# dakom/awsm-renderer

Measured on AMD Instinct MI355X. Metric: frames/sec + shaded Mpix/s, 4K Sponza glTF, 1/2/4/8 MI355X, higher is better.
Workload: dtype f32; 1 GPU; Sponza-class procedural atrium (configs[3]): 262144 triangles, 25 materials, 69 textures, 3840x2160, geometry pass + opaque pass, single-sample, MipmapMode::None; triangles=262144, width=3840, height=2160, draws=92, frame_overlap=True, stream_handoff=device flags (k_handoff_signal / k_handoff_wait), camera=orbit, one turn per 240 frames, environment=uniform cubes (builder default), opaque_route=lean (k_shade_lean + k_shade_todo), library=awsm-renderer_amd/libawsm_hip.so

## Files before the change

### awsm-renderer_amd/csrc/awsm_hip.cpp

```cpp
#include <hip/hip_runtime.h>
#include <algorithm>
#include <cmath>
#include <cstdarg>
#include <cstdio>
#include <cstdlib>
#include <cstring>
#include <ctime>
#include <string>
#include <vector>

#include "ctx.hpp"
#include "launch.hpp"

using namespace awsm;

namespace {

constexpr int kLeanWgsPerCu = 0;

inline FrameBufs* pass_slots(AwsmHipCtx* c, PassKind kind) {
    FrameBufs* const sets[kPassKinds] = {c->fb, c->tr, c->hud, c->htr, c->shadow};
    return sets[kind];
}
inline FrameBufs& pass_bufs(AwsmHipCtx* c, PassKind kind) { return pass_slots(c, kind)[c->slot]; }
inline FrameBufs& FB(AwsmHipCtx* c) { return c->fb[c->slot]; }
inline uint32_t samples_of(const AwsmHipCtx* c) { return c->msaa == 4 ? 4u : 1u; }
inline bool is_sharded(const AwsmHipCtx* c) { return c->band_n > 1 || (c->y1 != 0 && !(c->y0 == 0 && c->y1 >= c->height)); }
inline hipStream_t shade_stream_of(AwsmHipCtx* c) { return c->overlap ? c->shade_streams[c->slot] : c->stream; }
inline int n_slots(const AwsmHipCtx* c) { return c->overlap ? kSlots : 1; }
inline int prev_slot(const AwsmHipCtx* c) { return (c->slot + kSlots - 1) % kSlots; }
inline uint32_t* handoff_timeouts(AwsmHipCtx* c) { return c->counters_host + 16 + 2 * kSlots; }
inline unsigned long long* trace_slot(AwsmHipCtx* c, int which) { return c->trace_dev ? c->trace_dev + (size_t)which * c->trace_cap + c->frame_serial % c->trace_cap : nullptr; }
inline hipError_t mark_shade_done(AwsmHipCtx* c, hipStream_t ss) {
    if (c->handoff) awsm_launch_handoff_signal(c->handoff_flags + kSlots + c->slot, ++c->shade_sig[c->slot], trace_slot(c, 2), ss);
    else if (c->trace_dev) awsm_launch_handoff_signal(nullptr, 0u, trace_slot(c, 2), ss);
    const hipError_t e = hipEventRecord(c->ev_shade_done[c->slot], ss);
    c->shade_pending[c->slot] = true; c->shade_recorded[c->slot] = true;
    return e;
}
inline hipError_t wait_prev_slot(AwsmHipCtx* c, hipStream_t ss, bool main_kernel_only = false) {
    const int p = prev_slot(c);
    if (c->handoff && c->shade_sig[p]) {
        const bool lean = main_kernel_only && c->lean_flagged[p];
        awsm_launch_handoff_wait(c->handoff_flags + (lean ? 2 * kSlots : kSlots) + p, lean ? c->lean_sig[p] : c->shade_sig[p], c->handoff_budget_ticks, handoff_timeouts(c), c->handoff_timeouts_seen,
                                 c->handoff_poison + c->slot, c->frame_serial, ss);
        return hipSuccess;
    }
    return hipStreamWaitEvent(ss, c->ev_shade_done[p], 0);
}
inline hipError_t wait_slot_free(AwsmHipCtx* c) {
    if (c->handoff) { awsm_launch_handoff_wait(c->handoff_flags + kSlots + c->slot, c->shade_sig[c->slot], c->handoff_budget_ticks, handoff_timeouts(c), c->handoff_timeouts_seen,
                                               c->handoff_poison + c->slot, c->frame_serial, c->stream); return hipSuccess; }
    return hipStreamWaitEvent(c->stream, c->ev_shade_done[c->slot], 0);
}

struct HostTrace {
    static long threshold() { static long t = [] { const char* e = getenv("AWSM_HOST_TRACE"); return e ? atol(e) : 0L; }(); return t; }
    timespec last{};
    uint32_t serial;
    explicit HostTrace(uint32_t frame_serial) : serial(frame_serial) { if (threshold()) clock_gettime(CLOCK_MONOTONIC, &last); }
    void mark(const char* what) {
        if (!threshold()) return;
        timespec now; clock_gettime(CLOCK_MONOTONIC, &now);
        const long us = (now.tv_sec - last.tv_sec) * 1000000L + (now.tv_nsec - last.tv_nsec) / 1000L;
        if (us >= threshold()) fprintf(stderr, "awsm_hip host trace: frame %u: %s took %ld us\n", serial, what, us);
        last = now;
    }
};

int handoff_check(AwsmHipCtx* c) {
    if (!c->overlap) return AWSM_OK;
    const uint32_t now = *(volatile uint32_t*)handoff_timeouts(c);
    if (now != c->handoff_timeouts_seen) {
        c->handoff_dropped_frames += now - c->handoff_timeouts_seen;
        c->handoff_timeouts_seen = now;
        c->handoff = false;
        c->handoff_error_pending = true;
        for (FrameBufs& b : c->fb) b.cache_valid = false;
        c->taa_have = false; c->taa_serial = 0;
    }
    if (!c->handoff_error_pending) return AWSM_OK;
    c->handoff_error_pending = false;
    return fail(c, AWSM_ERR_DEVICE, "a device-side stream hand-off timed out (kernels serialised by a profiler, the streams folded onto one hardware queue, or a stall longer than "
                                    "AWSM_HANDOFF_TIMEOUT_MS): %u gate(s) so far, each dropped the frame it guarded whole — that frame's image was not written; this context orders "
                                    "its streams with events from here on (AWSM_DEVICE_HANDOFF=0 selects them from the start)", c->handoff_dropped_frames);
}

}

namespace awsm {

int fail(AwsmHipCtx* c, int code, const char* fmt, ...) {
    char buf[512];
    va_list ap;
    va_start(ap, fmt);
    vsnprintf(buf, sizeof buf, fmt, ap);
    va_end(ap);
    if (c) c->last_error = buf;
    return code;
}

hipError_t sync_shade_streams(AwsmHipCtx* c) {
    for (hipStream_t s : c->shade_streams) if (s) { const hipError_t e = hipStreamSynchronize(s); if (e != hipSuccess) return e; }
    for (bool& b : c->shade_recorded) b = false;
    return hipSuccess;
}

int dev_realloc(AwsmHipCtx* c, DevBuf& b, size_t bytes, bool zero) {
    if (b.ptr && b.size == bytes) {
        if (zero) HIPCHK(c, hipMemsetAsync(b.ptr, 0, bytes, c->stream));
        return AWSM_OK;
    }
    if (b.ptr) {
        HIPCHK(c, hipStreamSynchronize(c->stream));
        HIPCHK(c, sync_shade_streams(c));
        HIPCHK(c, hipFree(b.ptr));
        b.ptr = nullptr; b.size = 0;
    }
    if (bytes == 0) return AWSM_OK;
    HIPCHK(c, hipMalloc(&b.ptr, bytes));
    b.size = bytes;
    if (zero) HIPCHK(c, hipMemsetAsync(b.ptr, 0, bytes, c->stream));
    return AWSM_OK;
}

int dev_reserve(AwsmHipCtx* c, DevBuf& b, size_t bytes) {
    if (b.size >= bytes && b.ptr) return AWSM_OK;
    size_t want = std::max(bytes, b.size + b.size / 2);
    return dev_realloc(c, b, want, false);
}

constexpr size_t kKernelUploadMax = 256u << 10;

int stage_alloc(AwsmHipCtx* c, size_t len, uint8_t** out) {
    len = (len + 255) & ~size_t(255);
    if (len > c->stage_cap) {
        HIPCHK(c, hipStreamSynchronize(c->stream));
        if (c->stage) HIPCHK(c, hipHostFree(c->stage));
        c->stage = nullptr;
        size_t cap = std::max<size_t>(len * 2, 8u << 20);
        HIPCHK(c, hipHostMalloc((void**)&c->stage, cap, hipHostMallocDefault));
        c->stage_cap = cap; c->stage_head = 0;
    }
    if (c->stage_head + len > c->stage_cap) {
        HIPCHK(c, hipStreamSynchronize(c->stream));
        c->stage_head = 0;
    }
    *out = c->stage + c->stage_head;
    c->stage_head += len;
    return AWSM_OK;
}

int upload_small(AwsmHipCtx* c, void* dst, const void* src, size_t len) {
    uint8_t* st;
    int rc = stage_alloc(c, len, &st);
    if (rc) return rc;
    memcpy(st, src, len);
    if (len <= kKernelUploadMax && (len & 3u) == 0 && ((uintptr_t)dst & 3u) == 0 && ((uintptr_t)st & 3u) == 0) {
        awsm_launch_upload_words(dst, st, (uint32_t)(len >> 2), c->stream);
        HIPCHK(c, hipGetLastError());
    } else {
        HIPCHK(c, hipMemcpyAsync(dst, st, len, hipMemcpyHostToDevice, c->stream));
    }
    return AWSM_OK;
// ... 55 lines not shown
    f.tile_count = (uint32_t*)b.tile_count.ptr; f.tile_offset = (uint32_t*)b.tile_offset.ptr;
    f.tile_cursor = (uint32_t*)b.tile_cursor.ptr; f.bin_list = (uint32_t*)b.bin_list.ptr;
    f.tile_order = (uint32_t*)b.tile_order.ptr;
    f.scan_tmp = (uint32_t*)b.scan_tmp.ptr;
    f.tile_split = (uint32_t*)b.tile_split.ptr; f.raster_scratch = (unsigned long long*)b.raster_scratch.ptr;
    f.raster_extra_cap = b.raster_extra_cap; f.raster_slot_cap = b.raster_slot_cap;
    f.big_list = (uint32_t*)b.big_list.ptr;
    f.counters = (uint32_t*)b.counters.ptr;
    f.vis = (unsigned long long*)b.vis.ptr;
}

struct FrameView { bool hud_keys, merged; };
inline FrameView world_view() { return {false, false}; }
inline FrameView frame_view(const AwsmHipCtx* c) { return {c->hud_geometry_done, c->hud_merged}; }

void fill_frame(AwsmHipCtx* c, FrameDev* f, FrameView view) {
    memset(f, 0, sizeof *f);
    const PassList& world = c->lists[kPassWorld];
    const PassList& hud = c->lists[kPassHud];
    uint32_t y0, y1;
    shard(c, &y0, &y1);
    f->width = c->width; f->height = c->height; f->y0 = y0; f->y1 = y1; f->sy0 = y0; f->sy1 = y1;
    if (c->msaa && (y0 > 0 || y1 < c->height)) {
        f->y0 = y0 > 0 ? y0 - 1 : 0; f->y1 = std::min(c->height, y1 + 1);
    }
    f->tiles_x = (c->width + kTile - 1) / kTile;
    f->band_n = 1; f->band_r = 0; f->out_compact = 0;
    f->tile_row0 = f->y0 >> kTileShift;
    f->tiles_y = (f->y1 > f->y0) ? ((f->y1 + kTile - 1) / kTile - f->tile_row0) : 0;
    if (c->band_n > 1) {
        const uint32_t rows_full = (c->height + kTile - 1) / kTile;
        f->band_n = c->band_n; f->band_r = c->band_r; f->out_compact = c->band_compact;
        f->tile_row0 = c->band_r;
        f->tiles_y = c->band_r < rows_full ? (rows_full - c->band_r + c->band_n - 1) / c->band_n : 0;
    }
    f->n_draws = (uint32_t)world.draws.size();
    f->total_tris = world.total_tris; f->total_verts = 3u * world.total_tris;
    bind_pass(*f, FB(c));
    f->draw_shade = (DrawShadeDev*)FB(c).draw_shade.ptr;
    f->tex_slots = (TexSlotDev*)FB(c).tex_slots.ptr;
    f->draw_mat = (DrawMatDev*)FB(c).draw_mat.ptr;
    const bool lean_ok = !(c->flags & AWSM_CFG_GENERAL_SHADE_ONLY) && (uint64_t)c->width * c->height * (c->msaa == 4 ? 32u : 8u) < (1ull << 32) && (c->msaa == 0 || (c->msaa_edge_bits[c->slot].ptr && c->msaa_cells[c->slot].ptr)) && FB(c).tri_shade.ptr && FB(c).draw_lean.ptr && c->shade_todo[c->slot].ptr && ((uint64_t)world.total_tris + (view.merged ? hud.total_tris : 0u)) * kTriRecBytes < (1ull << 32) &&
                         c->bufs[AWSM_BUF_ATTR_DATA].size < (1ull << 32) - 64;
    f->tri_shade = lean_ok ? (uint4*)FB(c).tri_shade.ptr : nullptr;
    f->attr_data_bytes = (uint32_t)std::min<size_t>(c->bufs[AWSM_BUF_ATTR_DATA].size, 0xFFFFFFFFu);
    f->draw_lean = lean_ok ? (LeanDrawDev*)FB(c).draw_lean.ptr : nullptr;
    f->shade_todo = (uint32_t*)c->shade_todo[c->slot].ptr;
    f->shade_todo_cap = f->shade_todo ? (uint32_t)(c->shade_todo[c->slot].size / 4 - 4 - 1024) : 0u;
    f->lean_next = f->shade_todo ? f->shade_todo + 4 + f->shade_todo_cap : nullptr;
    f->lean_grid = c->lean_grid;
#ifdef AWSM_STAMP
    {
        static unsigned long long* stamps = nullptr;
        if (!stamps && hipMalloc((void**)&stamps, 4ull * 16384 * 8 * 8) == hipSuccess) (void)hipMemset(stamps, 0, 4ull * 16384 * 8 * 8);
        f->stamps = stamps;
        static bool told = false;
        if (!told) { told = true; FILE* fp = fopen("/tmp/awsm_stamps_ptr", "w"); if (fp) { fprintf(fp, "%llu\n", (unsigned long long)(uintptr_t)stamps); fclose(fp); } }
    }
#endif
    f->poison = c->handoff_poison ? c->handoff_poison + c->slot : nullptr;
    f->host_bin_status = c->counters_host + 16 + 2 * c->slot;
    f->frame_serial = c->frame_serial;
    f->camera = (const uint8_t*)FB(c).camera.ptr;
    f->camera_snap = nullptr; f->camera_snap_words = 0;
    memcpy(f->pix2view, FB(c).pix2view, sizeof f->pix2view); memcpy(f->view_rot, FB(c).view_rot, sizeof f->view_rot); memcpy(f->cam_pos, FB(c).cam_pos, sizeof f->cam_pos);
    memcpy(f->ortho_view_dir, FB(c).ortho_view_dir, sizeof f->ortho_view_dir); f->cam_ortho = FB(c).cam_ortho;
    f->msaa = c->msaa;
    f->msaa_color0 = (float4*)c->msaa_color0[c->slot].ptr;
    f->msaa_edges = (uint32_t*)c->msaa_edges[c->slot].ptr;
    f->msaa_edge_bits = (lean_ok && c->msaa == 4) ? (unsigned long long*)c->msaa_edge_bits[c->slot].ptr : nullptr;
    f->msaa_cells = (uint2*)c->msaa_cells[c->slot].ptr;
    f->hud_vis = view.hud_keys ? (const unsigned long long*)c->hud[c->slot].vis.ptr : nullptr;
    f->hud_draws = (const DrawDev*)c->hud[c->slot].draws_dev.ptr; f->hud_tri_info = (const uint32_t*)c->hud[c->slot].tri_flags.ptr;
    if (view.hud_keys && view.merged) {
        f->n_draws = (uint32_t)c->hud_combined.size();
        f->total_tris = world.total_tris + hud.total_tris; f->total_verts = 3u * f->total_tris;
        f->vis = (unsigned long long*)c->merged_vis[c->slot].ptr;
        f->hud_draws = f->draws; f->hud_tri_info = f->tri_info;
    }
    f->hud_pass = 0;
    f->msaa_halo = (const unsigned long long*)c->msaa_halo;
    f->halo_bands = c->band_n > 1 ? ((c->height + kTile - 1) / kTile + c->band_n - 1) / c->band_n : 0u;
    f->out_rgba16f = (uint16_t*)(c->bound_out ? (uint8_t*)c->bound_out - (size_t)c->out_first_row * c->width * 8 : c->out16[c->slot].ptr);
    f->out_rgba32f = (float*)c->out32[c->slot].ptr;
    f->lights_pre = (float4*)c->lights_pre[c->slot].ptr;
    f->lights_cap = (uint32_t)(c->lights_pre[c->slot].size / 32);
}

void compose_pixel_to_view(AwsmHipCtx* c, FrameBufs& b) {
    float cam[128];
    memcpy(cam, c->camera_host, 512);
    const float* proj = cam + 16; const float* inv_proj = cam + 64; const float* inv_view = cam + 80;
    const double W = (double)c->width, H = (double)c->height;
    const double A[16] = {2.0 / W, 0, 0, 0,   0, -2.0 / H, 0, 0,   0, 0, 1, 0,   1.0 / W - 1.0, 1.0 - 1.0 / H, 0, 1};
    for (int col = 0; col < 4; col++) for (int row = 0; row < 4; row++) {
        double s = 0.0;
        for (int k = 0; k < 4; k++) s += (double)inv_proj[k * 4 + row] * A[col * 4 + k];
        b.pix2view[col * 4 + row] = (float)s;
    }
    for (int col = 0; col < 3; col++) for (int row = 0; row < 3; row++) b.view_rot[col * 3 + row] = inv_view[col * 4 + row];
    for (int i = 0; i < 3; i++) b.cam_pos[i] = cam[96 + i];
    b.cam_ortho = proj[15] > 0.9f ? 1u : 0u;
    const double vx = inv_view[8], vy = inv_view[9], vz = inv_view[10], l = std::sqrt(vx * vx + vy * vy + vz * vz);
    b.ortho_view_dir[0] = l > 0.0 ? (float)(vx / l) : 0.0f; b.ortho_view_dir[1] = l > 0.0 ? (float)(vy / l) : 0.0f; b.ortho_view_dir[2] = l > 0.0 ? (float)(vz / l) : 1.0f;
}

int record(AwsmHipCtx* c, int which, hipStream_t s = nullptr) {
    if (!c->stage_timers) { c->ev_valid[which] = false; return AWSM_OK; }
    HIPCHK(c, hipEventRecord(c->ev[which], s ? s : c->stream));
    c->ev_valid[which] = true;
    return AWSM_OK;
}

AwsmHipCtx::ResolveKey resolve_key(AwsmHipCtx* c, const FrameDev& f) {
    AwsmHipCtx::ResolveKey k;
    memset(&k, 0, sizeof k);
    k.write_seq = c->write_seq + (c->scene_dirty ? 1u : 0u); k.draws_version = FB(c).draws_version;
    k.ptrs[0] = f.draw_shade; k.ptrs[1] = f.draw_mat; k.ptrs[2] = f.tex_slots; k.ptrs[3] = f.draw_lean; k.ptrs[4] = f.lights_pre;
    k.n_draws = f.n_draws; k.mipmap = c->last_opaque.mipmap; k.has_opaque = c->last_opaque.has_opaque; k.lights_cap = f.lights_cap;
    return k;
}
bool resolve_stale(AwsmHipCtx* c, const FrameDev& f) {
    const AwsmHipCtx::ResolveKey k = resolve_key(c, f);
    return memcmp(&k, &c->resolved[c->slot], sizeof k) != 0;
}

void fill_geometry_cache(AwsmHipCtx* c, FrameDev* f, bool replay) {
    FrameBufs& b = FB(c);
    f->wcache = (float4*)b.wcache.ptr;
    f->cache_on = 0; f->prev_draws = nullptr; f->prev_n_draws = 0; f->n_dirty = 0; f->cache_serial = b.cache_serial;
    if (!c->geometry_cache || replay || !b.cache_valid || !b.wcache.ptr || b.cache_had_tri_shade != (f->tri_shade != nullptr)) return;
    std::vector<DirtyRange> r;
    if (!c->dirty_log.ranges_since(b.cache_seq, kMaxDirtyRanges, r)) return;
    for (size_t i = 0; i < r.size(); i++) { f->dirty[i][0] = r[i].buf; f->dirty[i][1] = r[i].lo; f->dirty[i][2] = r[i].hi; }
    f->n_dirty = (uint32_t)r.size();
    f->prev_draws = (const DrawDev*)(b.cached_is_prev ? b.draws_prev.ptr : b.draws_dev.ptr);
    f->prev_n_draws = b.cached_n_draws;
    f->cache_on = f->prev_draws ? 1u : 0u;
}


inline void enqueue_binning(const FrameDev& f, bool has_tris, hipStream_t s) {
    if (has_tris) { awsm_launch_bin_count(&f, s); awsm_launch_bin_big(&f, 0, s); }
    awsm_launch_bin_scan(&f, s);
    if (has_tris) { awsm_launch_bin_fill(&f, s); awsm_launch_bin_big(&f, 1, s); }
}
int clear_empty_pass(AwsmHipCtx* c, const FrameBufs& b, uint32_t* counters, uint32_t n_tiles, hipStream_t s) {
    HIPCHK(c, hipMemsetAsync(counters, 0, kCtrWords * sizeof(uint32_t), s));
    HIPCHK(c, hipMemsetAsync(counters + 12, 0, 2 * sizeof(uint32_t), s));
    if (n_tiles) HIPCHK(c, hipMemsetAsync(b.tile_count.ptr, 0, n_tiles * sizeof(uint32_t), s));
    return AWSM_OK;
}

int enqueue_geometry(AwsmHipCtx* c, bool replay = false) {
    HostTrace ht(c->frame_serial);
    const PassList& world = c->lists[kPassWorld];
    FrameDev f;
    fill_frame(c, &f, world_view());
    fill_geometry_cache(c, &f, replay);
    f.block_draw = FB(c).block_map_valid ? (const uint32_t*)FB(c).block_map.ptr : nullptr;
    f.cache_mark = (c->stage_timers && FB(c).cache_mark.size >= (size_t)world.n_blocks * 4) ? (uint32_t*)FB(c).cache_mark.ptr : nullptr;
    const uint32_t n_tiles = f.tiles_x * f.tiles_y;
    int rc = sync_scene(c);
    if (rc) return rc;
    ht.mark("geometry: sync_scene");
    if (c->overlap && c->shade_pending[c->slot]) { HIPCHK(c, wait_slot_free(c)); c->shade_pending[c->slot] = false; }
    if (c->bufs[AWSM_BUF_CAMERA].ptr && !replay) {
        const size_t cam_bytes = std::min<size_t>(512, c->bufs[AWSM_BUF_CAMERA].size);
        if (world.total_tris && n_tiles) { f.camera_snap = (uint32_t*)FB(c).camera.ptr; f.camera_snap_words = (uint32_t)(cam_bytes / 4); }
        else HIPCHK(c, hipMemcpyAsync(FB(c).camera.ptr, c->bufs[AWSM_BUF_CAMERA].ptr, cam_bytes, hipMemcpyDeviceToDevice, c->stream));
    }
    if (c->overlap) {
        c->uploads_recorded[c->slot] = false;
        if (resolve_stale(c, f)) { HIPCHK(c, hipEventRecord(c->ev_uploads[c->slot], c->stream)); c->uploads_recorded[c->slot] = true; }
        c->geom_write_seq[c->slot] = c->write_seq;
    }
    ht.mark("geometry: slot wait + upload event");
    const bool has_geometry = world.total_tris && n_tiles;
    if (!has_geometry && (rc = clear_empty_pass(c, FB(c), (uint32_t*)FB(c).counters.ptr, n_tiles, c->stream))) return rc;
    if (c->trace_dev) awsm_launch_handoff_signal(nullptr, 0u, trace_slot(c, 0), c->stream);
    if ((rc = record(c, EV_START))) return rc;
#ifdef AWSM_DEBUG_SWITCHES
    static const int knockout_env = getenv("AWSM_DEBUG_KNOCKOUT") ? atoi(getenv("AWSM_DEBUG_KNOCKOUT")) : 0;
    const int knockout = c->frame_serial > 8 ? knockout_env : 0;
#else
    const int knockout = 0;
#endif
    if (has_geometry && !(knockout & 1)) awsm_launch_transform(c->scene_dev, &f, world.n_blocks, c->stream);
    if ((rc = record(c, EV_TRANSFORM))) return rc;
    ht.mark("geometry: transform launch");
    if (n_tiles && !(knockout & 2)) enqueue_binning(f, world.total_tris != 0, c->stream);
    if ((rc = record(c, EV_BIN))) return rc;
    ht.mark("geometry: bin launches");
    if (n_tiles && !(knockout & 4)) awsm_launch_raster(&f, c->stream);
    if ((rc = record(c, EV_RASTER))) return rc;
    ht.mark("geometry: raster launch");
    HIPCHK(c, hipGetLastError());
    {
        FrameBufs& b = FB(c);
        b.cache_valid = has_geometry && !(knockout & 1) && b.wcache.ptr != nullptr;
        b.cached_n_draws = (uint32_t)world.draws.size(); b.cached_is_prev = false;
        b.cache_had_tri_shade = f.tri_shade != nullptr;
        b.cache_seq = c->write_seq; b.cache_serial = c->frame_serial;
        uint64_t oldest = ~0ull;
        for (int sl = 0; sl < n_slots(c); sl++) oldest = std::min(oldest, c->fb[sl].cache_valid ? c->fb[sl].cache_seq : c->write_seq);
        c->dirty_log.prune(oldest);
    }
    return AWSM_OK;
}

int enqueue_opaque(AwsmHipCtx* c) {
    HostTrace ht(c->frame_serial);
    FrameDev f;
    fill_frame(c, &f, frame_view(c));
    f.has_opaque = c->last_opaque.has_opaque;
    f.mipmap = c->last_opaque.mipmap;
    f.aniso = (c->flags & AWSM_CFG_ANISOTROPIC) ? 1u : 0u;
    if (c->bound_out) {
        if (c->out_rows_mode) {
            if (f.out_compact || f.sy0 < c->out_first_row || (size_t)(f.sy1 - c->out_first_row) * c->width * 8 > c->bound_out_bytes)
                return fail(c, AWSM_ERR_INVALID_ARGUMENT, "opaque_pass: bound output starts at row %u and holds %zu bytes, the shard shades rows [%u, %u)", c->out_first_row, c->bound_out_bytes, f.sy0, f.sy1);
        } else {
            const size_t need = (f.out_compact ? (size_t)f.tiles_y * kTile : (size_t)c->height) * c->width * 8;
            if (c->bound_out_bytes < need) return fail(c, AWSM_ERR_INVALID_ARGUMENT, "opaque_pass: bound output holds %zu bytes, this shard layout writes %zu", c->bound_out_bytes, need);
        }
    }
    int rc = sync_scene(c);
    if (rc) return rc;
    hipStream_t ss = shade_stream_of(c);
    const bool want_resolve = f.sy1 > f.sy0 && f.has_opaque && (resolve_stale(c, f) || c->stage_timers);
    if (want_resolve) c->resolved[c->slot] = resolve_key(c, f);
    const bool early = c->uploads_recorded[c->slot] && c->overlap && !c->stage_timers && want_resolve && c->geometry_done && c->geom_write_seq[c->slot] == c->write_seq;
    if (early) {
        HIPCHK(c, hipStreamWaitEvent(ss, c->ev_uploads[c->slot], 0));
        awsm_launch_resolve_draws(c->scene_dev, &f, ss);
    }
    ht.mark("opaque: sync_scene + early resolve");
    if (c->overlap) {
        if (c->handoff) {
            ++c->geom_sig[c->slot];
            if (c->handoff_test_drop) c->handoff_test_drop--;
            else awsm_launch_handoff_signal(c->handoff_flags + c->slot, c->geom_sig[c->slot], trace_slot(c, 1), c->stream);
            awsm_launch_handoff_wait(c->handoff_flags + c->slot, c->geom_sig[c->slot], c->handoff_budget_ticks, handoff_timeouts(c), c->handoff_timeouts_seen, c->handoff_poison + c->slot, c->frame_serial, ss);
        } else {
            if (c->trace_dev) awsm_launch_handoff_signal(nullptr, 0u, trace_slot(c, 1), c->stream);
            HIPCHK(c, hipEventRecord(c->ev_geom_done[c->slot], c->stream));
            HIPCHK(c, hipStreamWaitEvent(ss, c->ev_geom_done[c->slot], 0));
        }
        const uint8_t* lo = (const uint8_t*)c->bound_out; const uint8_t* hi = lo ? lo + c->bound_out_bytes : nullptr;
        const int p = prev_slot(c);
        const bool same_image = lo && c->slot_out_lo[p] && lo < c->slot_out_hi[p] && c->slot_out_lo[p] < hi;
        if (c->shade_recorded[p]) HIPCHK(c, wait_prev_slot(c, ss, !(same_image || (c->msaa != 0 && c->msaa_halo))));
        c->slot_out_lo[c->slot] = lo; c->slot_out_hi[c->slot] = hi;
    }
    ht.mark("opaque: hand-off launches");
    if (want_resolve && !early) awsm_launch_resolve_draws(c->scene_dev, &f, ss);
    if ((rc = record(c, EV_SHADE_BEGIN, ss))) return rc;
    c->ev_valid[EV_SHADE_LEAN] = false;
    c->lean_flagged[c->slot] = false;
    if (c->overlap && c->handoff && f.sy1 > f.sy0 && awsm_shade_is_lean(&f)) {
        f.lean_done_flag = c->handoff_flags + 2 * kSlots + c->slot; f.lean_done_serial = ++c->lean_sig[c->slot];
        c->lean_flagged[c->slot] = true;
    }
    if (f.sy1 > f.sy0) {
        awsm_launch_shade(c->scene_dev, &f, ss);
        if (c->stage_timers && awsm_shade_is_lean(&f) && (rc = record(c, EV_SHADE_LEAN, ss))) return rc;
        (void)awsm_launch_shade_todo(c->scene_dev, &f, ss);
    }
    const AwsmHipCtx::ShadowState& sh = c->shadow_pass[c->slot];
    if (sh.on && c->shadow_px[c->slot] && f.has_opaque && f.sy1 > f.sy0) {
        const size_t px = (size_t)c->width * c->height;
        ShadowViewsArgs av{};
        ShadowArgs& a = av.base;
        const AwsmHipCtx::ShadowViews& views = c->shadow_views[c->slot];
        av.n_views = views.n; av.view = (unsigned char*)c->shadow_view_layers[c->slot].ptr;
        memcpy(av.view_proj, views.view_proj, sizeof av.view_proj);
        a.width = c->width; a.height = c->height;
        a.vis = (const unsigned long long*)FB(c).vis.ptr;
        a.camera = (const float*)f.camera;
        a.map = (const uint32_t*)c->shadow[c->slot].vis.ptr; a.map_size = sh.p.map_size; a.pcf_radius = (int32_t)sh.p.pcf_radius;
        memcpy(a.light_view_proj, sh.light_view_proj, sizeof a.light_view_proj); memcpy(a.light, sh.p.light, sizeof a.light);
        a.bias = sh.p.bias; a.slope_bias = sh.p.slope_bias; a.max_slope = sh.p.max_slope; a.strength = sh.p.strength; a.facing_fade = sh.p.facing_fade;
        a.visibility = (float*)c->shadow_layers[c->slot].ptr; a.multiplier = a.visibility + px;
        a.out16 = (uint2*)f.out_rgba16f; a.out32 = (float4*)f.out_rgba32f;
        a.poison = f.poison; a.frame_serial = f.frame_serial;
        awsm_launch_shadow_resolve(&a, samples_of(c), ss);
    }
    const AwsmHipCtx::SsaoState& so = c->ssao_pass[c->slot];
    if (so.on && f.has_opaque && f.sy1 > f.sy0) {
        const size_t px = (size_t)c->width * c->height;
        SsaoArgs sa{};
        sa.width = c->width; sa.height = c->height;
        sa.vis = (const unsigned long long*)FB(c).vis.ptr;
        sa.camera = (const float*)f.camera;
        sa.radius = so.p[0]; sa.intensity = so.p[1]; sa.bias = so.p[2]; sa.strength = so.p[3];
        sa.ao_raw = (float*)c->ssao_layers[c->slot].ptr; sa.ao_smoothed = sa.ao_raw + px; sa.view_z = sa.ao_raw + 2 * px;
        sa.out16 = (uint2*)f.out_rgba16f; sa.out32 = (float4*)f.out_rgba32f;
        sa.poison = f.poison; sa.frame_serial = f.frame_serial;
        awsm_launch_ssao(&sa, samples_of(c), ss);
    }
    if ((rc = record(c, EV_SHADE, ss))) return rc;
    ht.mark("opaque: shade launches");
    if (c->overlap) HIPCHK(c, mark_shade_done(c, ss));
    else if (c->trace_dev) awsm_launch_handoff_signal(nullptr, 0u, trace_slot(c, 2), ss);
    ht.mark("opaque: shade-done signal + event");
    HIPCHK(c, hipGetLastError());
    return AWSM_OK;
}

void fill_frame_forward(AwsmHipCtx* c, FrameDev* f, PassKind kind) {
    fill_frame(c, f, frame_view(c));
    const FrameBufs& t = pass_bufs(c, kind);
    const PassList& list = c->lists[kind];
    bind_pass(*f, t);
    f->vis = (unsigned long long*)FB(c).vis.ptr;
    f->n_draws = (uint32_t)list.draws.size();
    f->total_tris = list.total_tris; f->total_verts = 3u * list.total_tris;
    f->draw_shade = (DrawShadeDev*)t.draw_shade.ptr;
    f->tex_slots = (TexSlotDev*)t.tex_slots.ptr;
    f->draw_mat = (DrawMatDev*)t.draw_mat.ptr;
    f->wpos = (float4*)t.wpos.ptr;
    f->tri_shade = nullptr; f->draw_lean = nullptr; f->shade_todo = nullptr; f->shade_todo_cap = 0; f->lean_next = nullptr; f->lean_grid = 0;
    f->raster_scratch = nullptr;
    f->raster_extra_cap = 0; f->raster_slot_cap = 0;
    f->opaque_rgba16f = c->opaque_src ? (const uint16_t*)c->opaque_src : f->out_rgba16f;
    f->out_compact = 0;
    f->frag_rec = (uint4*)t.frag_rec.ptr; f->frag_color = (float4*)t.frag_color.ptr; f->frag_first = (uint32_t*)t.frag_first.ptr; f->frag_cap = t.frag_cap;
    f->out_rgba16f = (uint16_t*)(c->bound_comp ? c->bound_comp : c->comp16.ptr);
    f->out_rgba32f = (float*)c->comp32.ptr;
    f->has_opaque = c->last_opaque.has_opaque;
    f->mipmap = c->last_opaque.mipmap;
    f->aniso = (c->flags & AWSM_CFG_ANISOTROPIC) ? 1u : 0u;
    if (kind == kPassHudTransparent) {
        f->hud_pass = 1;
        f->opaque_rgba16f = f->out_rgba16f;
    }
}

void fill_selection(AwsmHipCtx* c, const AwsmHipCtx::SelectionState& st, SelectionDev* a) {
    memset(a, 0, sizeof *a);
    a->width = c->width; a->height = c->height; a->msaa = samples_of(c);
    a->n_draws = (uint32_t)c->lists[kPassWorld].draws.size(); a->total_tris = c->lists[kPassWorld].total_tris;
    a->n_keys = (uint32_t)(st.keys.size() / 2); a->n_boxes = (uint32_t)(st.boxes.size() / 6);
    a->flags = st.flags; a->radius = st.radius;
    memcpy(a->outline_color, st.outline_color, sizeof a->outline_color); memcpy(a->box_color, st.box_color, sizeof a->box_color);
    a->half_width = st.half_width; a->hidden_alpha = st.hidden_alpha; a->depth_epsilon = st.depth_epsilon;
    a->scene = c->scene_dev;
    a->material_meta_bytes = (uint32_t)std::min<size_t>(c->bufs[AWSM_BUF_MATERIAL_META].size, 0xFFFFFFFFu);
    a->draws = (const DrawDev*)FB(c).draws_dev.ptr;
    a->tri_info = (const uint32_t*)FB(c).tri_flags.ptr;
    a->vis = (const unsigned long long*)FB(c).vis.ptr;
    a->camera = (const uint8_t*)FB(c).camera.ptr;
    a->edges = (float*)c->sel_tables[c->slot].ptr;
    a->draw_selected = (uint8_t*)c->sel_tables[c->slot].ptr + (size_t)selection::kMaxEdges * selection::kEdgeFloats * 4;
    if (a->n_keys) memcpy(a->keys, st.keys.data(), st.keys.size() * 4);
    if (a->n_boxes) memcpy(a->boxes, st.boxes.data(), st.boxes.size() * 4);
}

int enqueue_transparent(AwsmHipCtx* c, PassKind kind) {
    const bool hud = kind == kPassHudTransparent;
    FrameDev f;
    fill_frame_forward(c, &f, kind);
    const uint32_t n_tiles = f.tiles_x * f.tiles_y;
    int rc = sync_scene(c);
    if (rc) return rc;
    hipStream_t ss = shade_stream_of(c);
    if (c->overlap && c->shade_recorded[prev_slot(c)]) HIPCHK(c, wait_prev_slot(c, ss));
    if ((rc = record(c, EV_FWD_BEGIN, ss))) return rc;
    const bool has_geometry = f.total_tris && n_tiles;
    if (!has_geometry) {
        if ((rc = clear_empty_pass(c, pass_bufs(c, kind), (uint32_t*)pass_bufs(c, kind).counters.ptr, n_tiles, ss))) return rc;
    } else {
        awsm_launch_resolve_draws(c->scene_dev, &f, ss);
        awsm_launch_transform_forward(c->scene_dev, &f, c->lists[kind].n_blocks, ss);
    }
    if (n_tiles) {
        enqueue_binning(f, f.total_tris != 0, ss);
        EditorGridDev grid;
        const AwsmHipCtx::GridState& gs = c->grid_pass[c->slot];
        const bool with_grid = gs.on && !hud;
        if (with_grid) { grid.camera = f.camera; memcpy(grid.p, gs.p, sizeof grid.p); }
        awsm_launch_forward(c->scene_dev, &f, with_grid ? &grid : nullptr, ss);
        const AwsmHipCtx::SelectionState& sl = c->sel_pass[c->slot];
        if (sl.on && !hud) {
            SelectionDev sd;
            fill_selection(c, sl, &sd);
            sd.out16 = (uint2*)f.out_rgba16f; sd.out32 = (float4*)f.out_rgba32f;
            sd.poison = f.poison; sd.frame_serial = f.frame_serial;
            awsm_launch_selection(&sd, ss);
        }
    }
    if ((rc = record(c, EV_FWD, ss))) return rc;
    if (c->overlap) HIPCHK(c, mark_shade_done(c, ss));
    HIPCHK(c, hipGetLastError());
    return AWSM_OK;
}

int ensure_bin_capacity_of(AwsmHipCtx* c, FrameBufs& b, uint32_t entries) {
    if (entries <= b.bin_capacity && b.bin_list.ptr) return AWSM_OK;
    uint32_t cap = std::max(entries, b.bin_capacity + b.bin_capacity / 2);
    int rc = dev_realloc(c, b.bin_list, (size_t)cap * 4, false);
    if (rc) return rc;
    b.bin_capacity = cap;
    return AWSM_OK;
}

int ensure_fragment_capacity(AwsmHipCtx* c, FrameBufs& b, uint32_t fragments) {
    if (fragments <= b.frag_cap && b.frag_rec.ptr) return AWSM_OK;
    const uint32_t cap = std::max(fragments, b.frag_cap + b.frag_cap / 2);
    int rc = dev_realloc(c, b.frag_rec, (size_t)cap * 16, false);
    if (!rc) rc = dev_realloc(c, b.frag_color, (size_t)cap * 16, false);
    if (rc) return rc;
    b.frag_cap = cap;
    return AWSM_OK;
}

int build_draw_list(AwsmHipCtx* c, const char* pass, const AwsmDraw* draws, uint32_t n, AwsmBuf data, uint32_t bytes_per_tri,
                    std::vector<DrawDev>& out, uint64_t* tris_out, uint64_t* blocks_out) {
    out.clear();
    uint64_t tris = 0, blocks = 0;
    for (uint32_t i = 0; i < n; i++) {
        const AwsmDraw& d = draws[i];
        if (d.inst_count != 0) {
            const DevBuf& ib = c->bufs[AWSM_BUF_INSTANCES];
            if (!ib.ptr) return fail(c, AWSM_ERR_NOT_READY, "%s: draw %u: instanced, but the instance-transform buffer was never created", pass, i);
            if ((d.inst_off & 15u) || (uint64_t)d.inst_off + 64ull * d.inst_count > ib.size)
                return fail(c, AWSM_ERR_OUT_OF_RANGE, "%s: draw %u: %u instances at %u exceed the instance-transform buffer", pass, i, d.inst_count, d.inst_off);
        }
        if (d.vis_data_off & (bytes_per_tri ? 15u : 3u)) return fail(c, AWSM_ERR_INVALID_ARGUMENT, "%s: draw %u: vertex data offset %u misaligned", pass, i, d.vis_data_off);
        if ((uint64_t)d.vis_data_off + (uint64_t)bytes_per_tri * d.tri_count > c->bufs[data].size || (!bytes_per_tri && d.tri_count && (uint64_t)d.vis_data_off + 40 > c->bufs[data].size))
            return fail(c, AWSM_ERR_OUT_OF_RANGE, "%s: draw %u: %u triangles at %u exceed the vertex buffer", pass, i, d.tri_count, d.vis_data_off);
        if ((uint64_t)d.geom_meta_off + 40 > c->bufs[AWSM_BUF_GEOM_META].size || (d.geom_meta_off & 3u))
            return fail(c, AWSM_ERR_OUT_OF_RANGE, "%s: draw %u: geometry meta offset %u out of range", pass, i, d.geom_meta_off);
        if (d.tri_count == 0) continue;
        const uint32_t copies = d.inst_count ? d.inst_count : 1u;
        for (uint32_t k = 0; k < copies; k++) {
            DrawDev dd{};
            dd.geom_meta_off = d.geom_meta_off; dd.vis_data_off = d.vis_data_off; dd.tri_count = d.tri_count; dd.flags = d.flags & 0x7Fu;
            if (d.inst_count) { dd.flags |= kDrawInstanced; dd.inst_off = d.inst_off + 64u * k; }
            dd.first_tri = (uint32_t)tris; dd.first_block = (uint32_t)blocks;
            out.push_back(dd);
            tris += d.tri_count;
            blocks += (3ull * d.tri_count + 255) / 256;
            if (tris > 0x55555555ull) return fail(c, AWSM_ERR_UNSUPPORTED, "%s: more than 2^32/3 triangles in one pass", pass);
            if (out.size() >= (1u << 24)) return fail(c, AWSM_ERR_UNSUPPORTED, "%s: more than 2^24 non-empty draws (instances included) in one pass", pass);
        }
    }
    *tris_out = tris; *blocks_out = blocks;
    return AWSM_OK;
}

struct PassDims { uint32_t w, h, samples; };
inline PassDims dims_of(const AwsmHipCtx* c, const FrameBufs& b) {
    if (b.kind == kPassShadow) { const uint32_t S = c->shadow_pass[b.slot].p.map_size; return {S, S, 1u}; }
    return {c->width, c->height, samples_of(c)};
}

int reserve_raster_items(AwsmHipCtx* c, FrameBufs& b, bool forward, PassDims dm) {
    const uint32_t tiles_x = (dm.w + kTile - 1) / kTile, tiles_y_full = (dm.h + kTile - 1) / kTile;
    const size_t n_tiles_full = (size_t)tiles_x * tiles_y_full;
    const uint32_t extra_cap = forward ? 0u : b.bin_capacity / 256u + 1u, slot_cap = forward ? 0u : b.bin_capacity / 128u + 2u;
    int rc;
    if ((rc = dev_reserve(c, b.tile_order, (n_tiles_full + extra_cap) * 4))) return rc;
    if (!forward && (rc = dev_reserve(c, b.raster_scratch, (size_t)slot_cap * kTile * kTile * 8 * dm.samples))) return rc;
    b.raster_extra_cap = extra_cap; b.raster_slot_cap = slot_cap;
    return AWSM_OK;
}

int size_pass_buffers(AwsmHipCtx* c, FrameBufs& b, size_t tri_cap, size_t draw_cap, bool forward, PassDims dm) {
    int rc;
    const size_t nd = std::max<size_t>(draw_cap, 1), nv = std::max<size_t>(3 * tri_cap, 1), nt = std::max<size_t>(tri_cap, 1);
    if ((rc = dev_reserve(c, b.draws_dev, nd * sizeof(DrawDev)))) return rc;
    const bool world_pass = b.kind == kPassWorld, shadow = b.kind == kPassShadow;
    if (world_pass && c->geometry_cache) {
        if ((rc = dev_reserve(c, b.draws_prev, nd * sizeof(DrawDev)))) return rc;
        if ((rc = dev_reserve(c, b.wcache, nv * 16))) return rc;
        const size_t blocks_bound = nv / 256 + nd + 1;
        if ((rc = dev_reserve(c, b.block_map, blocks_bound * 4))) return rc;
        b.block_map_valid = false;
        if (b.cache_mark.size < blocks_bound * 4) { if ((rc = dev_realloc(c, b.cache_mark, (blocks_bound + blocks_bound / 2) * 4, true))) return rc; }
    }
    b.cache_valid = false;
    if (!shadow && (rc = dev_reserve(c, b.draw_shade, nd * sizeof(DrawShadeDev)))) return rc;
    if (!shadow && (rc = dev_reserve(c, b.tex_slots, nd * kCoreTextures * sizeof(TexSlotDev)))) return rc;
    if (!shadow && (rc = dev_reserve(c, b.draw_mat, nd * sizeof(DrawMatDev)))) return rc;
    if ((rc = dev_reserve(c, b.clip, nv * 16))) return rc;
    if ((rc = dev_reserve(c, b.nrm, nv * 16))) return rc;
    if ((rc = dev_reserve(c, b.tan, nv * 16))) return rc;
    if (forward && (rc = dev_reserve(c, b.wpos, nv * 16))) return rc;
    if ((rc = dev_reserve(c, b.tri_flags, nt * 4))) return rc;
    if (!forward && !shadow && (rc = dev_reserve(c, b.tri_shade, nt * 32))) return rc;
    if (!forward && !shadow && (rc = dev_reserve(c, b.draw_lean, nd * sizeof(LeanDrawDev)))) return rc;
    if ((rc = dev_reserve(c, b.big_list, nt * 4))) return rc;
    if ((rc = dev_reserve(c, b.tri_rec, nt * kTriRecBytes))) return rc;
    const uint32_t tiles_x = (dm.w + kTile - 1) / kTile, tiles_y_full = (dm.h + kTile - 1) / kTile;
    const size_t n_tiles_full = (size_t)tiles_x * tiles_y_full;
    if ((rc = dev_reserve(c, b.tile_count, n_tiles_full * 4))) return rc;
    if ((rc = dev_reserve(c, b.tile_offset, (n_tiles_full + 1) * 4))) return rc;
    if ((rc = dev_reserve(c, b.tile_cursor, n_tiles_full * 4))) return rc;
    if ((rc = dev_reserve(c, b.tile_split, n_tiles_full * 8))) return rc;
    if ((rc = dev_reserve(c, b.scan_tmp, (((n_tiles_full + 255) / 256) * 2 + 1) * 40 * 4))) return rc;
    if ((rc = ensure_bin_capacity_of(c, b, (c->flags & AWSM_CFG_SMALL_BIN_LIST) ? 4096u : (uint32_t)std::min<size_t>(std::max<size_t>(4 * tri_cap + 65536u, 1u << 18), 0xFFFFFFF0u)))) return rc;
    if ((rc = reserve_raster_items(c, b, forward, dm))) return rc;
    b.tri_cap = tri_cap; b.draw_cap = draw_cap; b.sized_w = dm.w; b.sized_h = dm.h;
    return AWSM_OK;
}

int ensure_pass_capacity(AwsmHipCtx* c, FrameBufs& b, const std::vector<DrawDev>& draws_host, uint32_t total_tris, bool forward) {
    int rc;
    const PassDims dm = dims_of(c, b);
    if (total_tris > b.tri_cap || draws_host.size() > b.draw_cap || b.sized_w != dm.w || b.sized_h != dm.h || !b.bin_list.ptr) {
        bool instanced = false;
        for (const DrawDev& d : draws_host) instanced |= (d.flags & kDrawInstanced) != 0;
        const size_t tri_bound = forward || instanced ? ~size_t(0) : c->bufs[AWSM_BUF_VIS_GEOM_DATA].size / 168u;
        const size_t tri_cap = std::max<size_t>(std::min<size_t>((size_t)total_tris + total_tris / 4 + 4096, std::max<size_t>(tri_bound, total_tris)), b.tri_cap);
        const size_t draw_cap = std::max<size_t>(draws_host.size() + draws_host.size() / 4 + 64, b.draw_cap);
        const bool shadow = b.kind == kPassShadow;
        FrameBufs* const set = pass_slots(c, b.kind);
        for (int sl = 0; sl < (shadow ? 1 : n_slots(c)); sl++) {
            FrameBufs& t = set[(c->slot + sl) % kSlots];
            if ((rc = size_pass_buffers(c, t, std::max(tri_cap, t.tri_cap), std::max(draw_cap, t.draw_cap), forward, dm))) return rc;
        }
    }
    return AWSM_OK;
}

int upload_draws_at(AwsmHipCtx* c, FrameBufs& b, size_t at, const std::vector<DrawDev>& list) {
    const size_t bytes = list.size() * sizeof(DrawDev);
    uint8_t* dst = (uint8_t*)b.draws_dev.ptr + at * sizeof(DrawDev);
    if (bytes <= (1u << 20)) return upload_small(c, dst, list.data(), bytes);
    HIPCHK(c, hipMemcpyAsync(dst, list.data(), bytes, hipMemcpyHostToDevice, c->stream));
    HIPCHK(c, hipStreamSynchronize(c->stream));
    return AWSM_OK;
}

int upload_draw_list(AwsmHipCtx* c, FrameBufs& b, const std::vector<DrawDev>& draws_host, bool keep_prev) {
    const bool same_draws = b.draws_uploaded_valid && b.draws_uploaded_ptr == b.draws_dev.ptr && b.draws_uploaded.size() == draws_host.size() &&
                            (draws_host.empty() || memcmp(b.draws_uploaded.data(), draws_host.data(), draws_host.size() * sizeof(DrawDev)) == 0);
    auto upload_block_map = [&]() -> int {
        b.block_map_valid = false;
        if (!keep_prev || !b.block_map.ptr) return AWSM_OK;
        std::vector<uint32_t> map;
        for (size_t i = 0; i < draws_host.size(); i++) map.insert(map.end(), (3ull * draws_host[i].tri_count + 255) / 256, (uint32_t)i);
        if (map.size() * 4 > b.block_map.size || map.size() * 4 > (1u << 20)) return AWSM_OK;
        const int rc = upload_small(c, b.block_map.ptr, map.data(), map.size() * 4);
        if (!rc) b.block_map_valid = true;
        return rc;
    };
    if (draws_host.empty()) return AWSM_OK;
    if (same_draws) return (keep_prev && !b.block_map_valid) ? upload_block_map() : AWSM_OK;
    if (keep_prev && b.cache_valid && !b.cached_is_prev && b.draws_prev.ptr && b.draws_prev.size == b.draws_dev.size) {
        std::swap(b.draws_dev, b.draws_prev);
        b.cached_is_prev = true;
    } else if (keep_prev && !b.cached_is_prev) b.cache_valid = false;
    b.draws_uploaded = draws_host; b.draws_uploaded_ptr = b.draws_dev.ptr; b.draws_uploaded_valid = true; b.draws_version++;
    b.tail_uploaded_valid = false;
    { const int rc = upload_block_map(); if (rc) return rc; }
    return upload_draws_at(c, b, 0, draws_host);
}

int reserve_pass_buffers(AwsmHipCtx* c, FrameBufs& b, const std::vector<DrawDev>& draws_host, uint32_t total_tris, bool forward) {
    int rc = ensure_pass_capacity(c, b, draws_host, total_tris, forward);
    if (rc) return rc;
    return upload_draw_list(c, b, draws_host, b.kind == kPassWorld);
}

inline uint32_t with_headroom(uint32_t need) { return need + need / 4 + 1024; }
int grow_after_overflow(AwsmHipCtx* c, FrameBufs& b, const uint32_t* counters) {
    const int rc = ensure_bin_capacity_of(c, b, with_headroom(counters[kCtrEntries]));
    return rc ? rc : reserve_raster_items(c, b, false, dims_of(c, b));
}

int merge_record(AwsmHipCtx* c, const char* entry, const char* type, const void* src, void* dst, size_t size) {
    const uint32_t given = *(const uint32_t*)src;
    if (given < 4u || given > 4096u) return fail(c, AWSM_ERR_INVALID_ARGUMENT, "%s: %s.struct_size = %u (set it to sizeof(%s))", entry, type, given, type);
    memcpy((uint8_t*)dst + 4, (const uint8_t*)src + 4, (std::min<size_t>(given, size) & ~(size_t)3) - 4);
    return AWSM_OK;
}
int check_finite(AwsmHipCtx* c, const char* entry, const float* p, size_t n) {
    for (size_t i = 0; i < n; i++)
        if (!std::isfinite(p[i])) return fail(c, AWSM_ERR_INVALID_ARGUMENT, "%s: value %zu of the record is not finite", entry, i);
    return AWSM_OK;
}

}

extern "C" {

uint32_t awsm_hip_abi_version(void) { return AWSM_HIP_ABI_VERSION; }

const char* awsm_hip_last_error(const AwsmHipCtx* ctx) { return ctx ? ctx->last_error.c_str() : "null context"; }

int awsm_hip_create(const AwsmConfig* cfg, AwsmHipCtx** out) {
    if (!cfg || !out || cfg->struct_size < sizeof(AwsmConfig) || cfg->abi_version != AWSM_HIP_ABI_VERSION)
        return AWSM_ERR_INVALID_ARGUMENT;
    *out = nullptr;
    int n_dev = 0;
    if (hipGetDeviceCount(&n_dev) != hipSuccess || n_dev <= 0 || cfg->device < 0 || cfg->device >= n_dev) return AWSM_ERR_NO_DEVICE;
    AwsmHipCtx* c = new (std::nothrow) AwsmHipCtx();
    if (!c) return AWSM_ERR_OUT_OF_MEMORY;
    c->device = cfg->device;
    c->flags = cfg->flags;
    for (int k = 0; k < kPassKinds; k++)
        for (int s = 0; s < kSlots; s++) { FrameBufs& b = pass_slots(c, (PassKind)k)[s]; b.kind = (PassKind)k; b.slot = (uint8_t)s; }
    auto bail = [&](int code) { awsm_hip_destroy(c); return code; };
    if (hipSetDevice(c->device) != hipSuccess) return bail(AWSM_ERR_DEVICE);
    hipDeviceProp_t prop;
    if (hipGetDeviceProperties(&prop, c->device) != hipSuccess) return bail(AWSM_ERR_DEVICE);
    if (strncmp(prop.gcnArchName, "gfx950", 6) != 0) {
        fprintf(stderr, "awsm_hip: device %d is %s; this library carries gfx950 code objects only\n", c->device, prop.gcnArchName);
        return bail(AWSM_ERR_NO_DEVICE);
    }
    if (cfg->stream) { c->stream = (hipStream_t)cfg->stream; c->own_stream = false; }
    else { if (hipStreamCreateWithFlags(&c->stream, hipStreamNonBlocking) != hipSuccess) return bail(AWSM_ERR_DEVICE); c->own_stream = true; }
    for (int i = 0; i < EV_COUNT; i++) if (hipEventCreate(&c->ev[i]) != hipSuccess) return bail(AWSM_ERR_DEVICE);
    if (hipMalloc((void**)&c->scene_dev, sizeof(DevScene)) != hipSuccess) return bail(AWSM_ERR_OUT_OF_MEMORY);
    c->overlap = (cfg->flags & AWSM_CFG_OVERLAP_FRAMES) != 0;
    { const char* e = getenv("AWSM_GEOMETRY_CACHE"); c->geometry_cache = !(e && e[0] == '0'); }
    {
        const char* e = getenv("AWSM_LEAN_WGS_PER_CU");
        const int per_cu = e ? atoi(e) : (c->overlap ? kLeanWgsPerCu : 0);
        c->lean_grid = per_cu > 0 ? (uint32_t)(per_cu * prop.multiProcessorCount) & ~7u : 0u;
    }
    for (int s = 0; s < n_slots(c); s++) {
        for (PassKind k : {kPassWorld, kPassTransparent, kPassHudTransparent, kPassHud}) {
            DevBuf& ctr = pass_slots(c, k)[s].counters;
            if (hipMalloc(&ctr.ptr, 16 * sizeof(uint32_t)) != hipSuccess || (k == kPassWorld && hipMemset(ctr.ptr, 0, 16 * sizeof(uint32_t)) != hipSuccess)) return bail(AWSM_ERR_OUT_OF_MEMORY);
            ctr.size = 16 * sizeof(uint32_t);
        }
        if (hipMalloc(&c->fb[s].camera.ptr, 512) != hipSuccess || hipMemset(c->fb[s].camera.ptr, 0, 512) != hipSuccess) return bail(AWSM_ERR_OUT_OF_MEMORY);
        c->fb[s].camera.size = 512;
    }

    if (c->overlap) {
        for (int s = 0; s < kSlots; s++) {
#ifdef AWSM_DEBUG_SWITCHES
            if (const char* m = getenv("AWSM_SHADE_CU_MASK")) {
                std::vector<uint32_t> words;
                for (const char* p = m; *p; ) { char* end = nullptr; words.push_back((uint32_t)strtoul(p, &end, 16)); p = (*end == ',') ? end + 1 : end; if (end == p && *p) break; }
                if (words.empty() || hipExtStreamCreateWithCUMask(&c->shade_streams[s], (uint32_t)words.size(), words.data()) != hipSuccess) return bail(AWSM_ERR_DEVICE);
            } else
#endif
            if (hipStreamCreateWithFlags(&c->shade_streams[s], hipStreamNonBlocking) != hipSuccess) return bail(AWSM_ERR_DEVICE);
            const unsigned ev_flags = hipEventDisableTiming | hipEventReleaseToDevice;
            if (hipEventCreateWithFlags(&c->ev_geom_done[s], ev_flags) != hipSuccess || hipEventCreateWithFlags(&c->ev_shade_done[s], ev_flags) != hipSuccess ||
                hipEventCreateWithFlags(&c->ev_uploads[s], ev_flags) != hipSuccess) return bail(AWSM_ERR_DEVICE);
            if (s == 0 && hipEventCreateWithFlags(&c->ev_flush, hipEventDisableTiming) != hipSuccess) return bail(AWSM_ERR_DEVICE);
        }
    }
    if (hipHostMalloc((void**)&c->counters_host, (16 + 2 * kSlots + 1) * sizeof(uint32_t), hipHostMallocDefault) != hipSuccess) return bail(AWSM_ERR_OUT_OF_MEMORY);
    memset(c->counters_host, 0, (16 + 2 * kSlots + 1) * sizeof(uint32_t));
    if (c->overlap) {
        const char* e = getenv("AWSM_DEVICE_HANDOFF");
        c->handoff = !(e && e[0] == '0');
        { int khz = 0; if (hipDeviceGetAttribute(&khz, hipDeviceAttributeWallClockRate, c->device) == hipSuccess && khz > 0) c->clock_khz = (uint32_t)khz; }
        double budget_ms = 4000.0;
        if (const char* p = getenv("AWSM_HANDOFF_TIMEOUT_MS")) { const double v = atof(p); if (v > 0.0) budget_ms = v; }
        c->handoff_budget_ticks = (unsigned long long)(budget_ms * (double)c->clock_khz) + 1ull;
        if (hipMalloc((void**)&c->handoff_flags, 3 * kSlots * sizeof(uint32_t)) != hipSuccess || hipMalloc((void**)&c->handoff_poison, kSlots * sizeof(uint32_t)) != hipSuccess) return bail(AWSM_ERR_OUT_OF_MEMORY);
        if (hipMemset(c->handoff_flags, 0, 3 * kSlots * sizeof(uint32_t)) != hipSuccess || hipMemset(c->handoff_poison, 0xFF, kSlots * sizeof(uint32_t)) != hipSuccess ||
            hipDeviceSynchronize() != hipSuccess) return bail(AWSM_ERR_DEVICE);
        if (const char* d = getenv("AWSM_TEST_HANDOFF_DROP")) c->handoff_test_drop = (uint32_t)atoi(d);
        for (int k = 0; c->handoff && k < 2 * kSlots; k++) {
            hipStream_t ss = c->shade_streams[k % kSlots], waiter = k < kSlots ? ss : c->stream, setter = k < kSlots ? c->stream : ss;
            const uint32_t serial = ++c->geom_sig[0];
            awsm_launch_handoff_wait(c->handoff_flags, serial, 10ull * c->clock_khz , handoff_timeouts(c), 0u, nullptr, 0u, waiter);
            awsm_launch_handoff_signal(c->handoff_flags, serial, nullptr, setter);
            if (hipStreamSynchronize(waiter) != hipSuccess || hipStreamSynchronize(setter) != hipSuccess) return bail(AWSM_ERR_DEVICE);
            if (*(volatile uint32_t*)handoff_timeouts(c) != 0u) { c->handoff = false; c->handoff_timeouts_seen = *(volatile uint32_t*)handoff_timeouts(c); }
        }
    }
    memset(&c->scene, 0, sizeof c->scene);
    c->scene.skybox_rgba[3] = 1.0f;
    for (int i = 0; i < 3; i++) { c->scene.prefiltered_rgb[i] = 1.0f; c->scene.irradiance_rgb[i] = 1.0f; }
    *out = c;
    return AWSM_OK;
}

int awsm_hip_destroy(AwsmHipCtx* c) {
    if (!c) return AWSM_ERR_INVALID_ARGUMENT;
    (void)hipSetDevice(c->device);
    if (c->stream) (void)hipStreamSynchronize(c->stream);
    (void)sync_shade_streams(c);
    auto fr = [](DevBuf& b) { if (b.ptr) (void)hipFree(b.ptr); b.ptr = nullptr; b.size = 0; };
    for (auto& b : c->bufs) fr(b);
    for (auto& b : c->tex) fr(b);
    for (auto& b : c->tex_kinds) fr(b);
    for (auto& b : c->merged_vis) fr(b);
    fr(c->pose_records);
    fr(c->env_stage); fr(c->env_tables); fr(c->env_rows); fr(c->env_filter_tab); if (c->ev_env_copy) (void)hipEventDestroy(c->ev_env_copy);
    fr(c->lut); for (auto& b : c->cube_tex) fr(b); for (auto& b : c->cube_bordered) fr(b); fr(c->digest); for (auto& b : c->shade_todo) fr(b); for (int sl = 0; sl < kSlots; sl++) { fr(c->msaa_color0[sl]); fr(c->msaa_edges[sl]); fr(c->msaa_edge_bits[sl]); fr(c->msaa_cells[sl]); } fr(c->mip_kinds); for (auto& b : c->out16) fr(b); for (auto& b : c->out32) fr(b); fr(c->comp16); fr(c->comp32); fr(c->grid_layer); for (auto& b : c->lights_pre) fr(b);
    for (auto& b : c->ssao_layers) fr(b);
    for (auto& b : c->taa_img) fr(b); fr(c->taa_layers);
    for (auto& b : c->sel_tables) fr(b);
    fr(c->sel_layers);
    for (auto& b : c->shadow_layers) fr(b); for (auto& b : c->shadow_cam) fr(b); for (auto& b : c->shadow_view_ctr) fr(b); for (auto& b : c->shadow_view_layers) fr(b); for (DevScene* sc : c->shadow_scene) if (sc) (void)hipFree(sc);
    for (auto& b : c->display8) fr(b); fr(c->effects16); fr(c->bloom_a); fr(c->bloom_b); fr(c->dof_lc); fr(c->dof_blur);
    for (int k = 0; k < kPassKinds * kSlots; k++) {
        FrameBufs& b = pass_slots(c, (PassKind)(k / kSlots))[k % kSlots];
        fr(b.vis); fr(b.wpos); fr(b.frag_rec); fr(b.frag_color); fr(b.frag_first); fr(b.tex_slots); fr(b.draw_mat); fr(b.clip); fr(b.nrm); fr(b.tan); fr(b.tri_rec); fr(b.tri_flags); fr(b.tri_shade); fr(b.draw_lean); fr(b.draws_dev); fr(b.draw_shade); fr(b.tile_count); fr(b.tile_offset);
        fr(b.wcache); fr(b.draws_prev); fr(b.cache_mark); fr(b.block_map); fr(b.tile_cursor); fr(b.tile_order); fr(b.scan_tmp); fr(b.tile_split); fr(b.raster_scratch); fr(b.bin_list); fr(b.big_list); fr(b.counters); fr(b.camera);
    }
    for (hipStream_t st : c->shade_streams) if (st) (void)hipStreamDestroy(st);
    for (int i = 0; i < kSlots; i++) { if (c->ev_geom_done[i]) (void)hipEventDestroy(c->ev_geom_done[i]); if (c->ev_shade_done[i]) (void)hipEventDestroy(c->ev_shade_done[i]); if (c->ev_uploads[i]) (void)hipEventDestroy(c->ev_uploads[i]); }
    if (c->ev_flush) (void)hipEventDestroy(c->ev_flush);
    if (c->scene_dev) (void)hipFree(c->scene_dev);
    if (c->stage) (void)hipHostFree(c->stage);
    if (c->counters_host) (void)hipHostFree(c->counters_host);
    if (c->handoff_flags) (void)hipFree(c->handoff_flags);
    if (c->handoff_poison) (void)hipFree(c->handoff_poison);
    if (c->trace_dev) (void)hipFree(c->trace_dev);
    for (int i = 0; i < EV_COUNT; i++) if (c->ev[i]) (void)hipEventDestroy(c->ev[i]);
    if (c->own_stream && c->stream) (void)hipStreamDestroy(c->stream);
    delete c;
    return AWSM_OK;
}

int awsm_hip_device_info(AwsmHipCtx* c, char* name_out, size_t name_cap, uint32_t* cu_count, uint64_t* hbm_bytes) {
    if (!c) return AWSM_ERR_INVALID_ARGUMENT;
    hipDeviceProp_t prop;
    HIPCHK(c, hipGetDeviceProperties(&prop, c->device));
    if (name_out && name_cap) snprintf(name_out, name_cap, "%s (%s)", prop.name, prop.gcnArchName);
    if (cu_count) *cu_count = (uint32_t)prop.multiProcessorCount;
    if (hbm_bytes) *hbm_bytes = (uint64_t)prop.totalGlobalMem;
    return AWSM_OK;
}

int awsm_hip_buffer_create(AwsmHipCtx* c, AwsmBuf which, size_t bytes) {
    if (!c || (int)which < 0 || which >= AWSM_BUF_COUNT) return fail(c, AWSM_ERR_INVALID_ARGUMENT, "buffer_create: bad buffer id %d", (int)which);
    HIPCHK(c, hipSetDevice(c->device));
    { int rcb = scene_write_barrier(c); if (rcb) return rcb; }
    log_dirty(c, which, 0, ~size_t(0));
    if (bytes && c->bufs[which].ptr && c->bufs[which].size == bytes) {
        if (which == AWSM_BUF_CAMERA) memset(c->camera_host, 0, sizeof c->camera_host);
        HIPCHK(c, hipMemsetAsync(c->bufs[which].ptr, 0, bytes + 16, c->stream));
        return AWSM_OK;
    }
    int rc = dev_realloc(c, c->bufs[which], bytes ? bytes + 16 : 0, true);
    if (rc) return rc;
    if (bytes) c->bufs[which].size = bytes;
    if (which == AWSM_BUF_CAMERA) memset(c->camera_host, 0, sizeof c->camera_host);
    if (which == AWSM_BUF_LIGHTS) for (int sl = 0; sl < n_slots(c); sl++) if ((rc = dev_realloc(c, c->lights_pre[sl], std::max<size_t>(bytes / 64, 1) * 32, true))) return rc;
    c->scene_dirty = true;
    return AWSM_OK;
}

int awsm_hip_buffer_write(AwsmHipCtx* c, AwsmBuf which, size_t dst_off, const void* src, size_t len) {
    if (!c || (int)which < 0 || which >= AWSM_BUF_COUNT || (!src && len)) return fail(c, AWSM_ERR_INVALID_ARGUMENT, "buffer_write: bad argument");
    if ((dst_off & 3) || (len & 3)) return fail(c, AWSM_ERR_INVALID_ARGUMENT, "buffer_write: offset %zu / size %zu not 4-byte aligned", dst_off, len);
    DevBuf& b = c->bufs[which];
    if (!b.ptr) return fail(c, AWSM_ERR_NOT_READY, "buffer_write: buffer %d was never created", (int)which);
    if (dst_off > b.size || len > b.size - dst_off) return fail(c, AWSM_ERR_OUT_OF_RANGE, "buffer_write: [%zu,+%zu) outside buffer %d of %zu bytes", dst_off, len, (int)which, b.size);
    if (len == 0) return AWSM_OK;
    HIPCHK(c, hipSetDevice(c->device));
    if (which != AWSM_BUF_CAMERA) { int rcb = scene_write_barrier(c); if (rcb) return rcb; log_dirty(c, which, dst_off, dst_off + len); }
    else { if (dst_off < 512) memcpy(c->camera_host + dst_off, src, std::min<size_t>(len, 512 - dst_off)); c->camera_written_since_snapshot = true; }
    uint8_t* dst = (uint8_t*)b.ptr + dst_off;
    if (len <= (1u << 20)) return upload_small(c, dst, src, len);
    HIPCHK(c, hipMemcpyAsync(dst, src, len, hipMemcpyHostToDevice, c->stream));
    HIPCHK(c, hipStreamSynchronize(c->stream));
    return AWSM_OK;
}

int awsm_hip_skin_pose_records_write(AwsmHipCtx* c, uint32_t first, uint32_t n, const AwsmSkinPoseRecord* records) {
    if (!c || (!records && n)) return fail(c, AWSM_ERR_INVALID_ARGUMENT, "skin_pose_records_write: bad argument");
    static_assert(sizeof(AwsmSkinPoseRecord) == 72, "k_skin_pose reads 72-byte records");
    std::vector<AwsmSkinPoseRecord>& host = c->pose_records_host;
    if (first > host.size() || n > 0x03000000u - first) return fail(c, AWSM_ERR_OUT_OF_RANGE, "skin_pose_records_write: [%u,+%u) with %zu records resident", first, n, host.size());
    if (n == 0) return AWSM_OK;
    for (uint32_t i = 0; i < n; i++)
        if ((records[i].transform_offset & 3u) || (records[i].matrix_offset & 3u)) return fail(c, AWSM_ERR_INVALID_ARGUMENT, "skin_pose_records_write: record %u has an offset that is not a multiple of 4", first + i);
// ... 405 lines not shown
    }
    if (!c->shadow_scene[c->slot]) { HIPCHK(c, hipMalloc((void**)&c->shadow_scene[c->slot], sizeof(DevScene))); c->shadow_scene_seq[c->slot] = 0; }
    return dev_reserve(c, c->shadow_cam[c->slot], (size_t)cam_blocks * 512);
}

int awsm_hip_shadow_pass(AwsmHipCtx* c, const AwsmShadow* s, const void* light_camera, size_t camera_bytes, const AwsmDraw* casters, uint32_t n) {
    if (!c || !s || (!casters && n)) return AWSM_ERR_INVALID_ARGUMENT;
    if (!c->geometry_done || c->opaque_done) return fail(c, AWSM_ERR_NOT_READY, "shadow_pass goes between the geometry pass and the opaque pass of a frame");
    if (is_sharded(c))
        return fail(c, AWSM_ERR_UNSUPPORTED, "shadow_pass on a sharded context: the resolve's neighbours need rows the shard never rasterised (no halo exchange)");
    AwsmShadow full;
    float lvp[16];
    int rc;
    if ((rc = check_shadow_record(c, "shadow_pass", "spot", s, full))) return rc;
    if ((rc = check_light_block(c, "shadow_pass", light_camera, camera_bytes, lvp))) return rc;
    if (n && (rc = check_caster_buffers(c, "shadow_pass"))) return rc;
    HIPCHK(c, hipSetDevice(c->device));
    std::vector<DrawDev> list;
    uint64_t tris = 0, blocks = 0;
    if ((rc = build_draw_list(c, "shadow_pass", casters, n, AWSM_BUF_VIS_GEOM_DATA, 168u, list, &tris, &blocks))) return rc;
    FrameBufs& sb = pass_bufs(c, kPassShadow);
    PassList& cast = c->lists[kPassShadow];
    AwsmHipCtx::ShadowState& st = c->shadow_pass[c->slot];
    c->shadow_done = false; st.on = false;
    st.p = full; memcpy(st.light_view_proj, lvp, sizeof lvp);
    cast.draws.swap(list);
    cast.total_tris = (uint32_t)tris; cast.n_blocks = (uint32_t)blocks;
    if ((rc = reserve_shadow_slot(c, 0u, 1u))) return rc;
    if ((rc = dev_reserve(c, sb.vis, (size_t)full.map_size * full.map_size * 8))) return rc;
    if ((rc = reserve_pass_buffers(c, sb, cast.draws, cast.total_tris, false))) return rc;
    if ((rc = upload_small(c, c->shadow_cam[c->slot].ptr, light_camera, 512))) return rc;
    c->shadow_views[c->slot].n = 0;
    if ((rc = enqueue_shadow(c))) return rc;
    st.on = true; c->shadow_done = true;
    return AWSM_OK;
}

int awsm_hip_shadow_pass_views(AwsmHipCtx* c, const AwsmShadow* s, const AwsmShadowView* views, uint32_t n_views) {
    if (!c || !s) return AWSM_ERR_INVALID_ARGUMENT;
    if (!views || n_views < 1u || n_views > (uint32_t)AWSM_SHADOW_MAX_VIEWS)
        return fail(c, AWSM_ERR_INVALID_ARGUMENT, "shadow_pass_views: %u views at %p (1 .. %d views)", n_views, (const void*)views, AWSM_SHADOW_MAX_VIEWS);
    if (!c->geometry_done || c->opaque_done) return fail(c, AWSM_ERR_NOT_READY, "shadow_pass_views goes between the geometry pass and the opaque pass of a frame");
    if (is_sharded(c))
        return fail(c, AWSM_ERR_UNSUPPORTED, "shadow_pass_views on a sharded context: the resolve's neighbours need rows the shard never rasterised (no halo exchange)");
    AwsmShadow full;
    int rc;
    if ((rc = check_shadow_record(c, "shadow_pass_views", "positional", s, full))) return rc;
    float lvp[AWSM_SHADOW_MAX_VIEWS][16];
    uint8_t blocks_host[AWSM_SHADOW_MAX_VIEWS * 512];
    char label[AWSM_SHADOW_MAX_VIEWS][40];
    bool any_casters = false;
    for (uint32_t i = 0; i < n_views; i++) {
        const AwsmShadowView& v = views[i];
        snprintf(label[i], sizeof label[i], "shadow_pass_views: view %u", i);
        if (!v.casters && v.n_casters) return fail(c, AWSM_ERR_INVALID_ARGUMENT, "shadow_pass_views: view %u has %u casters at a null pointer", i, v.n_casters);
        if ((rc = check_light_block(c, label[i], v.light_camera, v.camera_bytes, lvp[i]))) return rc;
        memcpy(blocks_host + (size_t)i * 512, v.light_camera, 512);
        any_casters |= v.n_casters != 0;
    }
    if (any_casters && (rc = check_caster_buffers(c, "shadow_pass_views"))) return rc;
    HIPCHK(c, hipSetDevice(c->device));
    PassList lists[AWSM_SHADOW_MAX_VIEWS];
    for (uint32_t i = 0; i < n_views; i++) {
        uint64_t tris = 0, blocks = 0;
        if ((rc = build_draw_list(c, label[i], views[i].casters, views[i].n_casters, AWSM_BUF_VIS_GEOM_DATA, 168u, lists[i].draws, &tris, &blocks))) return rc;
        lists[i].total_tris = (uint32_t)tris; lists[i].n_blocks = (uint32_t)blocks;
    }
    FrameBufs& sb = pass_bufs(c, kPassShadow);
    AwsmHipCtx::ShadowState& st = c->shadow_pass[c->slot];
    AwsmHipCtx::ShadowViews& vs = c->shadow_views[c->slot];
    c->shadow_done = false; st.on = false;
    st.p = full; memcpy(st.light_view_proj, lvp[0], sizeof st.light_view_proj);
    vs.n = n_views; memcpy(vs.view_proj, lvp, sizeof vs.view_proj);
    for (uint32_t i = 0; i < n_views; i++) { vs.lists[i].draws.swap(lists[i].draws); vs.lists[i].total_tris = lists[i].total_tris; vs.lists[i].n_blocks = lists[i].n_blocks; }
    c->lists[kPassShadow] = PassList();
    if ((rc = reserve_shadow_slot(c, AWSM_SHADOW_MAX_VIEWS, AWSM_SHADOW_MAX_VIEWS))) return rc;
    if ((rc = dev_reserve(c, sb.vis, (size_t)n_views * full.map_size * full.map_size * 8))) return rc;
    for (uint32_t i = 0; i < n_views; i++)
        if ((rc = ensure_pass_capacity(c, sb, vs.lists[i].draws, vs.lists[i].total_tris, false))) return rc;
    if ((rc = upload_small(c, c->shadow_cam[c->slot].ptr, blocks_host, (size_t)n_views * 512))) return rc;
    if ((rc = enqueue_shadow_views(c))) return rc;
    st.on = true; c->shadow_done = true;
    return AWSM_OK;
}

static int read_shadow_layer(AwsmHipCtx* c, const char* entry, uint32_t view, uint64_t* keys) {
    if (!c || !keys) return AWSM_ERR_INVALID_ARGUMENT;
    if (!c->shadow_done || !c->shadow[c->slot].vis.ptr) return fail(c, AWSM_ERR_NOT_READY, "%s: the last submitted frame had no shadow pass", entry);
    const uint32_t n = std::max(c->shadow_views[c->slot].n, 1u);
    if (view >= n) return fail(c, AWSM_ERR_INVALID_ARGUMENT, "%s: view %u of a pass with %u", entry, view, n);
    HIPCHK(c, hipSetDevice(c->device));
    { int rcs = sync_all(c); if (rcs) return rcs; }
    const size_t S = c->shadow_pass[c->slot].p.map_size;
    HIPCHK(c, hipMemcpy(keys, (const uint64_t*)c->shadow[c->slot].vis.ptr + (size_t)view * S * S, S * S * 8, hipMemcpyDeviceToHost));
    return AWSM_OK;
}
int awsm_hip_read_shadow_map(AwsmHipCtx* c, uint64_t* keys) { return read_shadow_layer(c, "read_shadow_map", 0u, keys); }
int awsm_hip_read_shadow_map_view(AwsmHipCtx* c, uint32_t view, uint64_t* keys) { return read_shadow_layer(c, "read_shadow_map_view", view, keys); }

int awsm_hip_read_shadow_view(AwsmHipCtx* c, uint8_t* view_out) {
    if (!c || !view_out) return AWSM_ERR_INVALID_ARGUMENT;
    const size_t px = (size_t)c->width * c->height;
    if (!px || !c->shadow_done || !c->opaque_done || c->shadow_px[c->slot] != px || !c->shadow_views[c->slot].n || c->shadow_view_layers[c->slot].size < px)
        return fail(c, AWSM_ERR_NOT_READY, "read_shadow_view: the last submitted frame had no shadow_pass_views with an opaque pass (has_opaque) behind it");
    HIPCHK(c, hipSetDevice(c->device));
    { int rcs = sync_all(c); if (rcs) return rcs; }
    HIPCHK(c, hipMemcpy(view_out, c->shadow_view_layers[c->slot].ptr, px, hipMemcpyDeviceToHost));
    return AWSM_OK;
}

int awsm_hip_read_shadow(AwsmHipCtx* c, float* visibility, float* multiplier) {
    if (!c) return AWSM_ERR_INVALID_ARGUMENT;
    const size_t px = (size_t)c->width * c->height;
    if (!px || !c->shadow_done || !c->opaque_done || c->shadow_px[c->slot] != px || !c->shadow_layers[c->slot].ptr)
        return fail(c, AWSM_ERR_NOT_READY, "read_shadow: the last submitted frame had no shadow pass with an opaque pass (has_opaque) behind it");
    HIPCHK(c, hipSetDevice(c->device));
    { int rcs = sync_all(c); if (rcs) return rcs; }
    const float* d = (const float*)c->shadow_layers[c->slot].ptr;
    if (visibility) HIPCHK(c, hipMemcpy(visibility, d, px * 4, hipMemcpyDeviceToHost));
    if (multiplier) HIPCHK(c, hipMemcpy(multiplier, d + px, px * 4, hipMemcpyDeviceToHost));
    return AWSM_OK;
}

int awsm_hip_opaque_pass(AwsmHipCtx* c, const AwsmOpaqueParams* p) {
    if (!c || !p) return AWSM_ERR_INVALID_ARGUMENT;
    if (p->mipmap > 1) return fail(c, AWSM_ERR_INVALID_ARGUMENT, "opaque_pass: mipmap must be 0 (MipmapMode::None) or 1 (MipmapMode::Gradient)");
    if (c->width == 0) return fail(c, AWSM_ERR_NOT_READY, "opaque_pass before resize");
    if (p->has_opaque) {
        if (!c->geometry_done) return fail(c, AWSM_ERR_NOT_READY, "opaque_pass before geometry_pass");
        static const AwsmBuf need[] = {AWSM_BUF_CAMERA, AWSM_BUF_GEOM_META, AWSM_BUF_MATERIAL_META, AWSM_BUF_MATERIALS, AWSM_BUF_ATTR_INDEX,
                                       AWSM_BUF_ATTR_DATA, AWSM_BUF_TEXTURE_TRANSFORMS, AWSM_BUF_LIGHTS_INFO, AWSM_BUF_LIGHTS};
        for (AwsmBuf b : need) if (!c->bufs[b].ptr) return fail(c, AWSM_ERR_NOT_READY, "opaque_pass: buffer %d missing", (int)b);
        if (!c->lut.ptr) return fail(c, AWSM_ERR_NOT_READY, "opaque_pass: no BRDF LUT (env_upload or brdf_lut_generate)");
    }
    if (c->msaa == 4 && c->band_n > 1 && p->has_opaque) {
        const size_t need = (size_t)c->band_n * awsm_hip_msaa_halo_bands(c) * 2 * c->width * 8;
        if (!c->msaa_halo || c->msaa_halo_bytes < need)
            return fail(c, AWSM_ERR_NOT_READY, "opaque_pass: MSAA with band sharding needs the gathered halo keys (awsm_hip_msaa_halo_export -> all-gather -> awsm_hip_msaa_halo_bind, %zu bytes)", need);
    }
    const bool ssao_on = c->ssao.on && p->has_opaque;
    if (ssao_on && is_sharded(c))
        return fail(c, AWSM_ERR_UNSUPPORTED, "opaque_pass with SSAO on a sharded context: its taps and its smoothing read depth in rows the shard never rasterised (no halo exchange)");
    HIPCHK(c, hipSetDevice(c->device));
    if (ssao_on) { const int rcs = dev_reserve(c, c->ssao_layers[c->slot], (size_t)c->width * c->height * 12); if (rcs) return rcs; }
    c->ssao_pass[c->slot] = c->ssao;
    c->ssao_pass[c->slot].on = ssao_on;
    c->ssao_px[c->slot] = ssao_on ? (size_t)c->width * c->height : 0;
    const bool shadow_on = c->shadow_done && c->shadow_pass[c->slot].on && p->has_opaque;
    if (shadow_on) { const int rcs = dev_reserve(c, c->shadow_layers[c->slot], (size_t)c->width * c->height * 8); if (rcs) return rcs; }
    if (shadow_on && c->shadow_views[c->slot].n) { const int rcs = dev_reserve(c, c->shadow_view_layers[c->slot], (size_t)c->width * c->height); if (rcs) return rcs; }
    c->shadow_px[c->slot] = shadow_on ? (size_t)c->width * c->height : 0;
    c->last_opaque = *p;
    if (!p->has_opaque && c->camera_written_since_snapshot && c->bufs[AWSM_BUF_CAMERA].ptr) {
        int rcs = sync_all(c);
        if (rcs) return rcs;
        compose_pixel_to_view(c, FB(c));
        HIPCHK(c, hipMemcpy(FB(c).camera.ptr, c->bufs[AWSM_BUF_CAMERA].ptr, std::min<size_t>(512, c->bufs[AWSM_BUF_CAMERA].size), hipMemcpyDeviceToDevice));
        c->camera_written_since_snapshot = false;
    }
    int rc = enqueue_opaque(c);
    if (rc) return rc;
    c->opaque_done = true; c->transparent_done = false; c->hud_transparent_done = false;
    return AWSM_OK;
}

static int transparent_pass_body(AwsmHipCtx* c, const AwsmDraw* draws, uint32_t n, PassKind kind) {
    const bool hud = kind == kPassHudTransparent;
    if (!c || (!draws && n)) return AWSM_ERR_INVALID_ARGUMENT;
    if (!c->geometry_done || !c->opaque_done) return fail(c, AWSM_ERR_NOT_READY, "transparent_pass needs the geometry and opaque passes of the same frame first");
    if (hud && !c->transparent_done) return fail(c, AWSM_ERR_NOT_READY, "hud_transparent_pass draws over the composite: call transparent_pass first (n_draws = 0 is valid)");
    const bool sharded = is_sharded(c);
    if (sharded && !c->opaque_src)
        return fail(c, AWSM_ERR_UNSUPPORTED, "transparent_pass on a sharded context: screen-space transmission reads the whole opaque image — gather it and bind it with awsm_hip_bind_opaque_source first");
    if (!hud && c->sel.on && sharded)
        return fail(c, AWSM_ERR_UNSUPPORTED, "transparent_pass with a selection on a sharded context: the outline's ring reads keys in rows the shard never rasterised (no halo exchange)");
    if (!hud && c->sel.on && !c->lists[kPassWorld].draws.empty() && (!c->bufs[AWSM_BUF_GEOM_META].ptr || !c->bufs[AWSM_BUF_MATERIAL_META].ptr))
        return fail(c, AWSM_ERR_NOT_READY, "transparent_pass with a selection: the geometry or material meta buffer is missing");
    if (c->opaque_src && c->opaque_src_bytes < (size_t)c->width * c->height * 8)
        return fail(c, AWSM_ERR_INVALID_ARGUMENT, "transparent_pass: the bound opaque source holds %zu bytes, the frame needs %zu", c->opaque_src_bytes, (size_t)c->width * c->height * 8);
    static const AwsmBuf need[] = {AWSM_BUF_TRANSFORMS, AWSM_BUF_CAMERA, AWSM_BUF_GEOM_META, AWSM_BUF_MATERIAL_META, AWSM_BUF_MATERIALS, AWSM_BUF_ATTR_INDEX,
                                   AWSM_BUF_ATTR_DATA, AWSM_BUF_TEXTURE_TRANSFORMS, AWSM_BUF_LIGHTS_INFO, AWSM_BUF_LIGHTS, AWSM_BUF_TRANSPARENCY_GEOM_DATA};
    if (n) {
        for (AwsmBuf b : need) if (!c->bufs[b].ptr) return fail(c, AWSM_ERR_NOT_READY, "transparent_pass: buffer %d missing", (int)b);
        if (!c->lut.ptr) return fail(c, AWSM_ERR_NOT_READY, "transparent_pass: no BRDF LUT (env_upload or brdf_lut_generate)");
    }
    HIPCHK(c, hipSetDevice(c->device));
    uint64_t tris = 0, blocks = 0;
    PassList& list = c->lists[kind];
    FrameBufs& t = pass_bufs(c, kind);
    int rc = build_draw_list(c, hud ? "hud_transparent_pass" : "transparent_pass", draws, n, AWSM_BUF_TRANSPARENCY_GEOM_DATA, 0u, list.draws, &tris, &blocks);
    if (rc) return rc;
    list.total_tris = (uint32_t)tris; list.n_blocks = (uint32_t)blocks;
    const size_t px = (size_t)c->width * c->height;
    if (!c->bound_comp && (rc = dev_reserve(c, c->comp16, px * 8))) return rc;
    if (c->bound_comp && c->bound_comp_bytes < px * 8) return fail(c, AWSM_ERR_INVALID_ARGUMENT, "transparent_pass: bound composite holds %zu bytes, the frame needs %zu", c->bound_comp_bytes, px * 8);
    if ((c->flags & AWSM_CFG_PARITY_TAP) && (rc = dev_reserve(c, c->comp32, px * 16))) return rc;
    if ((rc = reserve_pass_buffers(c, t, list.draws, list.total_tris, true))) return rc;
    if ((rc = dev_reserve(c, t.frag_first, px * 4))) return rc;
    if ((rc = ensure_fragment_capacity(c, t, (c->flags & AWSM_CFG_SMALL_BIN_LIST) ? 4096u : (uint32_t)std::max<size_t>(px / 2, 1u << 20)))) return rc;
    if (c->overlap) {
        HIPCHK(c, hipEventRecord(c->ev_geom_done[c->slot], c->stream));
        HIPCHK(c, hipStreamWaitEvent(shade_stream_of(c), c->ev_geom_done[c->slot], 0));
    }
    if (!hud) c->grid_pass[c->slot] = c->grid;
    if (!hud) {
        if (c->sel.on && (rc = dev_reserve(c, c->sel_tables[c->slot], (size_t)selection::kMaxEdges * selection::kEdgeFloats * 4 + std::max<size_t>(c->lists[kPassWorld].draws.size(), 1)))) return rc;
        c->sel_pass[c->slot] = c->sel;
    }
    if ((rc = enqueue_transparent(c, kind))) return rc;
    if (hud) c->hud_transparent_done = true; else { c->transparent_done = true; c->hud_transparent_done = false; }
    return AWSM_OK;
}
int awsm_hip_transparent_pass(AwsmHipCtx* c, const AwsmDraw* draws, uint32_t n) { return transparent_pass_body(c, draws, n, kPassTransparent); }
int awsm_hip_hud_transparent_pass(AwsmHipCtx* c, const AwsmDraw* draws, uint32_t n) { return transparent_pass_body(c, draws, n, kPassHudTransparent); }

int awsm_hip_set_stage_timers(AwsmHipCtx* c, int enabled) {
    if (!c) return AWSM_ERR_INVALID_ARGUMENT;
    c->stage_timers = enabled != 0;
    return AWSM_OK;
}

int awsm_hip_frame_trace(AwsmHipCtx* c, uint32_t capacity) {
    if (!c || capacity > (1u << 20)) return AWSM_ERR_INVALID_ARGUMENT;
    HIPCHK(c, hipSetDevice(c->device));
    { int rcs = sync_all(c); if (rcs) return rcs; }
    if (c->trace_dev) { HIPCHK(c, hipFree(c->trace_dev)); c->trace_dev = nullptr; c->trace_cap = 0; }
    if (!capacity) return AWSM_OK;
    HIPCHK(c, hipMalloc((void**)&c->trace_dev, (size_t)3 * capacity * 8));
    HIPCHK(c, hipMemset(c->trace_dev, 0, (size_t)3 * capacity * 8));
    c->trace_cap = capacity;
    return AWSM_OK;
}

int awsm_hip_read_frame_trace(AwsmHipCtx* c, uint64_t* ticks_out, uint32_t n_frames, uint32_t* last_serial_out, uint32_t* ticks_per_ms_out) {
    if (!c || !ticks_out) return AWSM_ERR_INVALID_ARGUMENT;
    if (!c->trace_dev) return fail(c, AWSM_ERR_NOT_READY, "read_frame_trace: tracing is off (awsm_hip_frame_trace)");
    if (n_frames == 0 || n_frames > c->trace_cap) return fail(c, AWSM_ERR_OUT_OF_RANGE, "read_frame_trace: %u frames asked, the ring holds %u", n_frames, c->trace_cap);
    HIPCHK(c, hipSetDevice(c->device));
    { int rcs = sync_all(c); if (rcs) return rcs; }
    std::vector<uint64_t> ring((size_t)3 * c->trace_cap);
    HIPCHK(c, hipMemcpy(ring.data(), c->trace_dev, ring.size() * 8, hipMemcpyDeviceToHost));
    for (uint32_t i = 0; i < n_frames; i++) {
        const uint32_t serial = c->frame_serial - (n_frames - 1u - i);
        for (int w = 0; w < 3; w++) ticks_out[(size_t)i * 3 + w] = ring[(size_t)w * c->trace_cap + serial % c->trace_cap];
    }
    if (last_serial_out) *last_serial_out = c->frame_serial;
    if (ticks_per_ms_out) { int khz = 0; *ticks_per_ms_out = hipDeviceGetAttribute(&khz, hipDeviceAttributeWallClockRate, c->device) == hipSuccess && khz > 0 ? (uint32_t)khz : 100000u; }
    return AWSM_OK;
}

int awsm_hip_frame_flush(AwsmHipCtx* c) {
    if (!c) return AWSM_ERR_INVALID_ARGUMENT;
    { int rch = handoff_check(c); if (rch) return rch; }
    int rc = scene_write_barrier(c, false);
    if (rc || !c->overlap) return rc;
    HIPCHK(c, hipEventRecord(c->ev_flush, c->stream));
    return AWSM_OK;
}

static int enqueue_post(AwsmHipCtx* c, const AwsmPostParams& p);
int awsm_hip_frame_end(AwsmHipCtx* c, AwsmFrameStats* out) {
    if (!c) return AWSM_ERR_INVALID_ARGUMENT;
    HIPCHK(c, hipSetDevice(c->device));
    const PassList& world_list = c->lists[kPassWorld];
    const uint32_t* const world = c->counters_host;
    const uint32_t* const fwd = c->counters_host + 8;
    bool still_over = false;
    for (int attempt = 0;; attempt++) {
        if (out && c->geometry_done && c->has_opaque_for_stats()) {
            FrameDev f;
            fill_frame(c, &f, frame_view(c));
            HIPCHK(c, hipMemsetAsync((uint32_t*)FB(c).counters.ptr + kCtrCovered, 0, sizeof(uint32_t), c->stream));
            awsm_launch_count_covered(&f, c->stream);
        }
        HIPCHK(c, hipMemcpyAsync(c->counters_host, FB(c).counters.ptr, 8 * sizeof(uint32_t), hipMemcpyDeviceToHost, c->stream));
        HIPCHK(c, hipStreamSynchronize(c->stream));
        c->cache_blocks_last = 0;
        if (out && c->geometry_done && c->stage_timers && world_list.n_blocks && FB(c).cache_mark.size >= (size_t)world_list.n_blocks * 4) {
            std::vector<uint32_t> marks(world_list.n_blocks);
            HIPCHK(c, hipMemcpy(marks.data(), FB(c).cache_mark.ptr, marks.size() * 4, hipMemcpyDeviceToHost));
            for (uint32_t m : marks) c->cache_blocks_last += m == c->frame_serial ? 1u : 0u;
        }
        if (c->overlap) { HIPCHK(c, sync_shade_streams(c)); for (bool& b : c->shade_pending) b = false; }
        { int rch = handoff_check(c); if (rch) return rch; }
        memset(c->counters_host + 8, 0, 8 * sizeof(uint32_t));
        uint32_t hud_fwd[kCtrWords] = {}, hud_geo[kCtrWords] = {}, shadow_geo[kCtrWords] = {};
        if (c->shadow_done) { const int rcs = read_shadow_counters(c, shadow_geo); if (rcs) return rcs; }
        if (c->transparent_done) HIPCHK(c, hipMemcpy(c->counters_host + 8, pass_bufs(c, kPassTransparent).counters.ptr, kCtrWords * sizeof(uint32_t), hipMemcpyDeviceToHost));
        if (c->hud_transparent_done) HIPCHK(c, hipMemcpy(hud_fwd, pass_bufs(c, kPassHudTransparent).counters.ptr, sizeof hud_fwd, hipMemcpyDeviceToHost));
        if (c->hud_geometry_done) HIPCHK(c, hipMemcpy(hud_geo, pass_bufs(c, kPassHud).counters.ptr, sizeof hud_geo, hipMemcpyDeviceToHost));
        const bool geom_over = c->geometry_done && world[kCtrOverflow] != 0, fwd_over = c->transparent_done && fwd[kCtrOverflow] != 0;
        const bool frag_over = c->transparent_done && fwd[kCtrFragOverflow] != 0;
        const bool hud_geo_over = c->hud_geometry_done && hud_geo[kCtrOverflow] != 0, hud_fwd_over = c->hud_transparent_done && hud_fwd[kCtrOverflow] != 0, hud_frag_over = c->hud_transparent_done && hud_fwd[kCtrFragOverflow] != 0;
        const bool shadow_over = c->shadow_done && shadow_geo[kCtrOverflow] != 0;
        still_over = geom_over || fwd_over || frag_over || hud_geo_over || hud_fwd_over || hud_frag_over || shadow_over;
        if (!still_over || attempt >= 4) break;
        int rc;
        c->overflow_retries++;
        if (geom_over) {
            if ((rc = grow_after_overflow(c, FB(c), world))) return rc;
            if ((rc = enqueue_geometry(c, true))) return rc;
        }
        if (hud_geo_over || (geom_over && c->hud_geometry_done && c->hud_merged)) {
            if (hud_geo_over && (rc = grow_after_overflow(c, pass_bufs(c, kPassHud), hud_geo))) return rc;
            if ((rc = enqueue_hud_geometry(c))) return rc;
        }
        if (shadow_over) {
            if ((rc = grow_after_overflow(c, pass_bufs(c, kPassShadow), shadow_geo))) return rc;
// ... 380 lines not shown
    if (full.flags & ~AWSM_TAA_RESET) return fail(c, AWSM_ERR_INVALID_ARGUMENT, "set_taa: unknown flags 0x%x", full.flags);
    for (int i = 0; i < 2; i++) if (!std::isfinite(full.jitter_ndc[i])) return fail(c, AWSM_ERR_INVALID_ARGUMENT, "set_taa: jitter_ndc[%d] is not finite", i);
    for (int i = 0; i < 16; i++) if (!std::isfinite(full.reproject[i])) return fail(c, AWSM_ERR_INVALID_ARGUMENT, "set_taa: reproject[%d] is not finite", i);
    AwsmHipCtx::TaaState& st = c->taa;
    st.on = true;
    st.feedback = full.feedback;
    st.flags |= full.flags;
    memcpy(st.jitter, full.jitter_ndc, sizeof st.jitter); memcpy(st.reproject, full.reproject, sizeof st.reproject);
    return AWSM_OK;
}
int awsm_hip_read_taa(AwsmHipCtx* c, uint16_t* resolved, float* lookup_xy, uint8_t* used) {
    if (!c) return AWSM_ERR_INVALID_ARGUMENT;
    const size_t px = (size_t)c->width * c->height;
    if (!px || !c->taa_resolved || !c->post_done || c->taa_serial != c->frame_serial) return fail(c, AWSM_ERR_NOT_READY, "read_taa: the last post pass did not resolve (awsm_hip_set_taa, then awsm_hip_post_pass)");
    HIPCHK(c, hipSetDevice(c->device));
    { int rcs = sync_all(c); if (rcs) return rcs; }
    if (resolved) HIPCHK(c, hipMemcpy(resolved, c->taa_args.out, px * 8, hipMemcpyDeviceToHost));
    if (lookup_xy || used) {
        const int rc = dev_reserve(c, c->taa_layers, px * 9);
        if (rc) return rc;
        TaaArgs t = c->taa_args;
        t.layer_xy = (float*)c->taa_layers.ptr; t.layer_used = (uint8_t*)(t.layer_xy + 2 * px);
        t.poison = nullptr;
        awsm_launch_taa_layers(&t, samples_of(c), c->stream);
        HIPCHK(c, hipGetLastError());
        HIPCHK(c, hipStreamSynchronize(c->stream));
        if (lookup_xy) HIPCHK(c, hipMemcpy(lookup_xy, t.layer_xy, px * 8, hipMemcpyDeviceToHost));
        if (used) HIPCHK(c, hipMemcpy(used, t.layer_used, px, hipMemcpyDeviceToHost));
    }
    return AWSM_OK;
}

int awsm_hip_post_pass(AwsmHipCtx* c, const AwsmPostParams* p) {
    if (!c || !p) return AWSM_ERR_INVALID_ARGUMENT;
    if (p->struct_size != sizeof(AwsmPostParams)) return fail(c, AWSM_ERR_INVALID_ARGUMENT, "post_pass: struct_size %u, this library's AwsmPostParams is %zu bytes", p->struct_size, sizeof(AwsmPostParams));
    if (p->tonemapping > 2u) return fail(c, AWSM_ERR_INVALID_ARGUMENT, "post_pass: tonemapping %u (0 None, 1 KhronosNeutralPbr, 2 Aces)", p->tonemapping);
    if (p->flags & ~(AWSM_POST_SMAA | AWSM_POST_BLOOM | AWSM_POST_DOF)) return fail(c, AWSM_ERR_INVALID_ARGUMENT, "post_pass: unknown flags 0x%x", p->flags);
    if (is_sharded(c)) return fail(c, AWSM_ERR_UNSUPPORTED, "post_pass on a sharded context: the SMAA / bloom / DoF stencils read neighbouring rows (no halo exchange)");
    if (c->width == 0 || !c->geometry_done || !c->opaque_done) return fail(c, AWSM_ERR_NOT_READY, "post_pass needs the frame's opaque pass first");
    if (c->taa.on && (c->taa.flags & AWSM_TAA_RESET)) { c->taa_have = false; c->taa_serial = 0; c->taa.flags &= ~AWSM_TAA_RESET; }
    c->taa_pass = c->taa;
    if (!c->taa.on) c->taa_resolved = false;
    return enqueue_post(c, *p);
}

static int enqueue_post(AwsmHipCtx* c, const AwsmPostParams& pp) {
    const AwsmPostParams* p = &pp;
    const size_t px = (size_t)c->width * c->height;
    if (c->bound_display && c->bound_display_bytes < px * 4) return fail(c, AWSM_ERR_INVALID_ARGUMENT, "post_pass: bound display image holds %zu bytes, the frame needs %zu", c->bound_display_bytes, px * 4);
    HIPCHK(c, hipSetDevice(c->device));
    int rc = AWSM_OK;
    if (!c->bound_display && (rc = dev_reserve(c, c->display8[c->slot], px * 4))) return rc;
    const bool bloom = p->flags & AWSM_POST_BLOOM, dof = p->flags & AWSM_POST_DOF, tap = c->flags & AWSM_CFG_PARITY_TAP;
    if (tap && (rc = dev_reserve(c, c->effects16, px * 8))) return rc;
    if (bloom && ((rc = dev_reserve(c, c->bloom_a, px * 8)) || (rc = dev_reserve(c, c->bloom_b, px * 8)))) return rc;
    if (dof && ((rc = dev_reserve(c, c->dof_lc, px * 8)) || (rc = dev_reserve(c, c->dof_blur, px * 16)))) return rc;
    PostArgs a{};
    a.width = c->width; a.height = c->height;
    if (c->transparent_done) a.src = (const uint2*)(c->bound_comp ? c->bound_comp : c->comp16.ptr);
    else a.src = (const uint2*)(c->bound_out ? (const uint8_t*)c->bound_out - (size_t)c->out_first_row * c->width * 8 : (const uint8_t*)c->out16[c->slot].ptr);
    a.vis = (const unsigned long long*)FB(c).vis.ptr;
    const FrameBufs& t = pass_bufs(c, kPassTransparent);
    if (dof && c->transparent_done && c->lists[kPassTransparent].total_tris && t.frag_first.ptr) {
        a.frag_first = (const uint32_t*)t.frag_first.ptr; a.frag_rec = (const uint4*)t.frag_rec.ptr; a.frag_cap = t.frag_cap; a.tri_rec = (const TriRec*)t.tri_rec.ptr;
    }
    a.camera = (const float*)FB(c).camera.ptr;
    a.dof_lc = (float2*)c->dof_lc.ptr; a.dof_blur = (float4*)c->dof_blur.ptr;
    a.effects = tap ? (uint2*)c->effects16.ptr : nullptr;
    a.display = (uint32_t*)(c->bound_display ? c->bound_display : c->display8[c->slot].ptr);
    a.tonemap = p->tonemapping; a.dof = dof ? 1u : 0u;
    a.poison = c->handoff_poison ? c->handoff_poison + c->slot : nullptr; a.frame_serial = c->frame_serial;
    if (!a.src || !a.vis || !a.camera) return fail(c, AWSM_ERR_NOT_READY, "post_pass: the frame's images are missing");
    hipStream_t ss = shade_stream_of(c);
    if (c->overlap && c->shade_recorded[prev_slot(c)]) HIPCHK(c, wait_prev_slot(c, ss));
    if (c->taa_pass.on) {
        if ((rc = dev_reserve(c, c->taa_img[0], px * 8)) || (rc = dev_reserve(c, c->taa_img[1], px * 8))) return rc;
        if (c->taa_serial != c->frame_serial) {
            c->taa_frame_hist = c->taa_have;
            c->taa_cur ^= 1;
            c->taa_serial = c->frame_serial;
        }
        const AwsmHipCtx::TaaState& ts = c->taa_pass;
        TaaArgs t{};
        t.width = c->width; t.height = c->height;
        t.cur = a.src; t.vis = a.vis;
        t.history = c->taa_frame_hist ? (const uint2*)c->taa_img[c->taa_cur ^ 1].ptr : nullptr;
        t.out = (uint2*)c->taa_img[c->taa_cur].ptr;
        memcpy(t.reproject, ts.reproject, sizeof t.reproject); t.jitter[0] = ts.jitter[0]; t.jitter[1] = ts.jitter[1]; t.feedback = ts.feedback;
        t.poison = a.poison; t.frame_serial = a.frame_serial;
        awsm_launch_taa(&t, samples_of(c), ss);
        a.src = t.out;
        c->taa_args = t; c->taa_have = true; c->taa_resolved = true;
    }
    awsm_launch_post(&a, p->flags, samples_of(c), c->bloom_a.ptr, c->bloom_b.ptr, ss);
    HIPCHK(c, hipGetLastError());
    if (c->overlap) HIPCHK(c, mark_shade_done(c, ss));
    c->last_display = a.display;
    c->post_params = pp;
    c->post_done = true;
    return AWSM_OK;
}

int awsm_hip_read_display(AwsmHipCtx* c, uint8_t* out) {
    if (!c || !out) return AWSM_ERR_INVALID_ARGUMENT;
    if (!c->last_display) return fail(c, AWSM_ERR_NOT_READY, "read_display before post_pass");
    HIPCHK(c, hipSetDevice(c->device));
    { int rcs = sync_all(c); if (rcs) return rcs; }
    HIPCHK(c, hipMemcpy(out, c->last_display, (size_t)c->width * c->height * 4, hipMemcpyDeviceToHost));
    return AWSM_OK;
}

int awsm_hip_read_effects(AwsmHipCtx* c, uint16_t* out) {
    if (!c || !out) return AWSM_ERR_INVALID_ARGUMENT;
    if (!(c->flags & AWSM_CFG_PARITY_TAP) || !c->effects16.ptr || !c->last_display) return fail(c, AWSM_ERR_NOT_READY, "read_effects needs AWSM_CFG_PARITY_TAP and a post_pass");
    HIPCHK(c, hipSetDevice(c->device));
    { int rcs = sync_all(c); if (rcs) return rcs; }
    HIPCHK(c, hipMemcpy(out, c->effects16.ptr, (size_t)c->width * c->height * 8, hipMemcpyDeviceToHost));
    return AWSM_OK;
}

int awsm_hip_bind_display(AwsmHipCtx* c, void* device_ptr, size_t bytes) {
    if (!c) return AWSM_ERR_INVALID_ARGUMENT;
    if (device_ptr && bytes == 0) return fail(c, AWSM_ERR_INVALID_ARGUMENT, "bind_display: zero-sized image");
    c->bound_display = device_ptr; c->bound_display_bytes = bytes;
    return AWSM_OK;
}

void* awsm_hip_display_device_ptr(AwsmHipCtx* c) { return c ? c->last_display : nullptr; }

static int read_pass_vertices(AwsmHipCtx* c, const FrameBufs& b, uint32_t n, float* clip_out, float* nt_out, float* wpos_out) {
    HIPCHK(c, hipSetDevice(c->device));
    { int rcs = sync_all(c); if (rcs) return rcs; }
    if (n == 0) return AWSM_OK;
    if (clip_out) HIPCHK(c, hipMemcpy(clip_out, b.clip.ptr, (size_t)n * 16, hipMemcpyDeviceToHost));
    if (wpos_out) HIPCHK(c, hipMemcpy(wpos_out, b.wpos.ptr, (size_t)n * 16, hipMemcpyDeviceToHost));
    if (nt_out) {
        std::vector<float> nn((size_t)n * 4), tt((size_t)n * 4);
        HIPCHK(c, hipMemcpy(nn.data(), b.nrm.ptr, (size_t)n * 16, hipMemcpyDeviceToHost));
        HIPCHK(c, hipMemcpy(tt.data(), b.tan.ptr, (size_t)n * 16, hipMemcpyDeviceToHost));
        for (size_t i = 0; i < n; i++) { memcpy(nt_out + i * 8, &nn[i * 4], 16); memcpy(nt_out + i * 8 + 4, &tt[i * 4], 16); }
    }
    return AWSM_OK;
}

int awsm_hip_read_transformed_forward(AwsmHipCtx* c, float* clip_out, float* nt_out, float* wpos_out, uint32_t max_vertices) {
    if (!c) return AWSM_ERR_INVALID_ARGUMENT;
    if (!c->transparent_done) return fail(c, AWSM_ERR_NOT_READY, "read_transformed_forward before transparent_pass");
    return read_pass_vertices(c, pass_bufs(c, kPassTransparent), std::min(max_vertices, 3u * c->lists[kPassTransparent].total_tris), clip_out, nt_out, wpos_out);
}

int awsm_hip_read_transformed(AwsmHipCtx* c, float* clip_out, float* nt_out, uint32_t max_vertices) {
    if (!c) return AWSM_ERR_INVALID_ARGUMENT;
    if (!c->geometry_done) return fail(c, AWSM_ERR_NOT_READY, "read_transformed before geometry_pass");
    return read_pass_vertices(c, FB(c), std::min(max_vertices, 3u * c->lists[kPassWorld].total_tris), clip_out, nt_out, nullptr);
}

}
```

### awsm-renderer_amd/csrc/ctx.hpp

```cpp
#pragma once
#include <hip/hip_runtime.h>
#include <stddef.h>
#include <stdint.h>
#include <string>
#include <vector>

#include "frame_params.hpp"
#include "dirty_log.hpp"

namespace awsm {

#ifndef AWSM_SLOTS
#define AWSM_SLOTS 2
#endif
constexpr int kSlots = AWSM_SLOTS;
struct DevBuf {
    void* ptr = nullptr;
    size_t size = 0;
};

enum { EV_START = 0, EV_TRANSFORM, EV_BIN, EV_RASTER, EV_SHADE_BEGIN, EV_SHADE_LEAN, EV_SHADE, EV_FWD_BEGIN, EV_FWD, EV_COUNT };

enum PassKind : uint8_t { kPassWorld = 0, kPassTransparent, kPassHud, kPassHudTransparent, kPassShadow };
constexpr int kPassKinds = 5;

struct PassList {
    std::vector<DrawDev> draws;
    uint32_t total_tris = 0, n_blocks = 0;
};

struct FrameBufs {
    DevBuf wpos;
    DevBuf frag_rec, frag_color, frag_first;
    uint32_t frag_cap = 0;
    DevBuf tex_slots;
    DevBuf draw_mat;
    DevBuf tri_shade, draw_lean;
    DevBuf clip, nrm, tan, tri_rec, tri_flags, draws_dev, draw_shade, tile_count, tile_offset, tile_cursor, tile_order, bin_list, big_list, counters, vis;
    DevBuf camera;
    DevBuf scan_tmp;
    DevBuf tile_split, raster_scratch;
    uint32_t raster_extra_cap = 0, raster_slot_cap = 0;
    uint32_t bin_capacity = 0;
    float pix2view[16] = {}, view_rot[9] = {}, cam_pos[3] = {}, ortho_view_dir[3] = {};
    uint32_t cam_ortho = 0;
    size_t tri_cap = 0, draw_cap = 0;
    uint32_t sized_w = 0, sized_h = 0;
    std::vector<DrawDev> draws_uploaded;
    void* draws_uploaded_ptr = nullptr;
    bool draws_uploaded_valid = false;
    uint64_t draws_version = 0;
    std::vector<DrawDev> tail_uploaded;
    void* tail_uploaded_ptr = nullptr;
    size_t tail_uploaded_at = 0;
    bool tail_uploaded_valid = false;
    DevBuf wcache, draws_prev;
    DevBuf block_map;
    bool block_map_valid = false;
    DevBuf cache_mark;
    uint32_t cached_n_draws = 0;
    bool cache_valid = false;
    bool cached_is_prev = false;
    bool cache_had_tri_shade = false;
    uint64_t cache_seq = 0;
    uint32_t cache_serial = 0;
    PassKind kind = kPassWorld;
    uint8_t slot = 0;
};

}

using namespace awsm;

struct AwsmHipCtx {
    int device = 0;
    uint32_t flags = 0;
    hipStream_t stream = nullptr;
    bool own_stream = false;
    bool stage_timers = true;
    std::string last_error;

    DevBuf bufs[AWSM_BUF_COUNT];
    bool camera_written_since_snapshot = false;
    uint8_t camera_host[512] = {};
    DevScene scene{};
    DevScene* scene_dev = nullptr;
    bool scene_dirty = true;
    DevBuf tex[kMaxTexArrays];
    DevBuf lut;
    DevBuf cube_tex[3], cube_bordered[3];
    DevBuf env_stage, env_tables, env_rows, env_filter_tab;
    hipEvent_t ev_env_copy = nullptr;
    DevBuf tex_kinds[kMaxTexArrays];
    uint32_t tex_srgb[64] = {};
    bool tex_srgb_made = false;

    DevBuf pose_records;
    std::vector<AwsmSkinPoseRecord> pose_records_host;

    uint32_t width = 0, height = 0;
    uint32_t y0 = 0, y1 = 0;
    uint32_t band_n = 1, band_r = 0, band_compact = 0;
    uint32_t msaa = 0;
    DevBuf mip_kinds;
    DevBuf msaa_color0[kSlots], msaa_edges[kSlots];
    DevBuf msaa_edge_bits[kSlots];
    DevBuf msaa_cells[kSlots];
    DevBuf out16[kSlots], out32[kSlots];
    DevBuf digest;
    uint32_t lean_grid = 0;
    DevBuf shade_todo[kSlots];
    void* bound_out = nullptr;
    size_t bound_out_bytes = 0;
    const uint8_t* slot_out_lo[kSlots] = {}; const uint8_t* slot_out_hi[kSlots] = {};

    bool overlap = false;
    hipStream_t shade_streams[kSlots] = {};
    bool shade_recorded[kSlots] = {};
    bool uploads_recorded[kSlots] = {};
    struct ResolveKey { uint64_t write_seq, draws_version; const void* ptrs[5]; uint32_t n_draws, mipmap, has_opaque, lights_cap; } resolved[kSlots] = {};
    hipEvent_t ev_geom_done[kSlots] = {}, ev_shade_done[kSlots] = {}, ev_uploads[kSlots] = {} ;
    hipEvent_t ev_flush = nullptr;
    uint64_t write_seq = 0, geom_write_seq[kSlots] = {};
    DirtyLog dirty_log;
    bool geometry_cache = true;
    uint32_t cache_blocks_last = 0;
    bool shade_pending[kSlots] = {};
    bool handoff = false;
    uint32_t* handoff_flags = nullptr;
    uint32_t geom_sig[kSlots] = {}, shade_sig[kSlots] = {}, lean_sig[kSlots] = {};
    bool lean_flagged[kSlots] = {};
    unsigned long long handoff_budget_ticks = 400000000ull;
    uint32_t clock_khz = 100000;
    uint32_t* handoff_poison = nullptr;
    uint32_t handoff_timeouts_seen = 0;
    uint32_t handoff_dropped_frames = 0;
    bool handoff_error_pending = false;
    uint32_t handoff_test_drop = 0;
    FrameBufs fb[kSlots];
    FrameBufs tr[kSlots];
    FrameBufs hud[kSlots];
    bool hud_geometry_done = false;
    bool hud_merged = false;
    DevBuf merged_vis[kSlots];
    std::vector<DrawDev> hud_combined;
    bool transparent_done = false, hud_transparent_done = false;
    FrameBufs htr[kSlots];
    struct GridState { bool on = false; float p[20] = {}; } grid, grid_pass[kSlots];
    DevBuf grid_layer;
    struct SelectionState {
        bool on = false;
        uint32_t flags = 0, radius = 0;
        float outline_color[4] = {}, box_color[4] = {}, half_width = 0, hidden_alpha = 0, depth_epsilon = 0;
        std::vector<uint32_t> keys;
        std::vector<float> boxes;
    } sel, sel_pass[kSlots];
    DevBuf sel_tables[kSlots], sel_layers;
    DevBuf comp16, comp32;
    DevBuf display8[kSlots], effects16, bloom_a, bloom_b, dof_lc, dof_blur;
    void* bound_display = nullptr;
    size_t bound_display_bytes = 0;
    void* last_display = nullptr;
    bool post_done = false;
    AwsmPostParams post_params{};
    DevBuf lights_pre[kSlots];
    void* bound_comp = nullptr;
    size_t bound_comp_bytes = 0;
    const void* msaa_halo = nullptr;
    size_t msaa_halo_bytes = 0;
    const void* opaque_src = nullptr;
    size_t opaque_src_bytes = 0;
    int slot = 0;
    PassList lists[kPassKinds];
    std::vector<AwsmDraw> draws_api;
    bool geometry_done = false, opaque_done = false;
    AwsmOpaqueParams last_opaque{};
    uint32_t overflow_retries = 0;
    bool has_opaque_for_stats() const { return !opaque_done || last_opaque.has_opaque != 0; }

    uint8_t* stage = nullptr;
    size_t stage_cap = 0, stage_head = 0;
    uint32_t* counters_host = nullptr;
    uint32_t frame_serial = 0, status_seen[kSlots] = {};
    uint32_t dropped_frames = 0;
    uint32_t out_first_row = 0;
    bool out_rows_mode = false;

    hipEvent_t ev[EV_COUNT] = {};
    bool ev_valid[EV_COUNT] = {};

    unsigned long long* trace_dev = nullptr;
    uint32_t trace_cap = 0;

    struct SsaoState { bool on = false; float p[4] = {}; } ssao, ssao_pass[kSlots];
    DevBuf ssao_layers[kSlots];
    size_t ssao_px[kSlots] = {};

    FrameBufs shadow[kSlots];
    DevScene* shadow_scene[kSlots] = {};
    uint64_t shadow_scene_seq[kSlots] = {}, scene_uploads = 0;
    DevBuf shadow_cam[kSlots];
    bool shadow_done = false;
    struct ShadowState { bool on = false; AwsmShadow p{}; float light_view_proj[16] = {}; } shadow_pass[kSlots];
    DevBuf shadow_layers[kSlots];
    size_t shadow_px[kSlots] = {};

    struct TaaState {
        bool on = false;
        float feedback = 0.1f;
        uint32_t flags = 0;
        float jitter[2] = {};
        float reproject[16] = {1, 0, 0, 0, 0, 1, 0, 0, 0, 0, 1, 0, 0, 0, 0, 1};
    } taa, taa_pass;
    DevBuf taa_img[2], taa_layers;
    int taa_cur = 0;
    bool taa_have = false;
    bool taa_frame_hist = false;
    uint32_t taa_serial = 0;
    bool taa_resolved = false;
    TaaArgs taa_args{};

    struct ShadowViews {
        uint32_t n = 0;
        float view_proj[AWSM_SHADOW_MAX_VIEWS][16] = {};
        PassList lists[AWSM_SHADOW_MAX_VIEWS];
    } shadow_views[kSlots];
    DevBuf shadow_view_ctr[kSlots], shadow_view_layers[kSlots];
};

#define HIPCHK(c, call)                                                                            \
    do {                                                                                           \
        hipError_t e_ = (call);                                                                    \
        if (e_ != hipSuccess)                                                                      \
            return fail((c), e_ == hipErrorOutOfMemory ? AWSM_ERR_OUT_OF_MEMORY : AWSM_ERR_DEVICE, \
                        "%s failed: %s (%s:%d)", #call, hipGetErrorString(e_), __FILE__, __LINE__); \
    } while (0)

#define AWSM_HIDDEN __attribute__((visibility("hidden")))

namespace awsm {

AWSM_HIDDEN int fail(AwsmHipCtx* c, int code, const char* fmt, ...);
AWSM_HIDDEN hipError_t sync_shade_streams(AwsmHipCtx* c);
AWSM_HIDDEN int dev_realloc(AwsmHipCtx* c, DevBuf& b, size_t bytes, bool zero);
AWSM_HIDDEN int dev_reserve(AwsmHipCtx* c, DevBuf& b, size_t bytes);
AWSM_HIDDEN int stage_alloc(AwsmHipCtx* c, size_t len, uint8_t** out);
AWSM_HIDDEN int upload_small(AwsmHipCtx* c, void* dst, const void* src, size_t len);
AWSM_HIDDEN int scene_write_barrier(AwsmHipCtx* c, bool is_write = true);
AWSM_HIDDEN int sync_all(AwsmHipCtx* c);
AWSM_HIDDEN uint32_t mip_levels_full(uint32_t w, uint32_t h);

}
```

### awsm-renderer_amd/csrc/frame_params.hpp

```cpp
#pragma once
#include <hip/hip_runtime.h>
#include <stdint.h>
#include "../../include/awsm_hip.h"

namespace awsm {

constexpr int kTile = 32;
constexpr int kTileShift = 5;
constexpr int kMaxTexArrays = 64;
constexpr int kMaxSamplers = 32;

constexpr uint32_t kDrawInstanced = 0x80u;

struct DrawDev {
    uint32_t geom_meta_off;
    uint32_t vis_data_off;
    uint32_t tri_count;
    uint32_t flags;
    uint32_t first_tri;
    uint32_t first_block;
    uint32_t inst_off;
    uint32_t pad1;
};

struct DrawShadeDev {
    uint32_t first_tri;
    uint32_t material_word;
    uint32_t attr_indices_word;
    uint32_t attr_data_word;
    uint32_t stride_words;
    uint32_t uv_sets_index;
    uint32_t flags;
    uint32_t color_sets;
};

struct TexSlotDev {
    const uint32_t* base;
    uint32_t width, height;
    uint32_t flags;
    float tt[6];
    uint32_t layer_levels;
    const uint32_t* level_off;
    const uint32_t* array_base;
};
static_assert(sizeof(TexSlotDev) == 64, "TexSlotDev must be 64 bytes");
constexpr int kCoreTextures = 5;

struct DrawMatDev {
    float base_color[4];
    float metallic, roughness, normal_scale, occlusion_strength;
    float emissive[3];
    float ior;
    uint32_t shader_alpha;
    uint32_t debug_bitmask;
    uint32_t ext_mask;
    float alpha_cutoff;
};
static_assert(sizeof(DrawMatDev) == 64, "DrawMatDev must be 64 bytes");

struct LeanDrawDev {
    uint32_t flags;
    float metallic, roughness, normal_scale;
    float base_color[3]; float occlusion_strength;
    float emissive[3];
    float normal_bias;
    uint32_t tex[kCoreTextures][2];
    float occlusion_bias;
    uint32_t pad1;
    uint32_t gtex[kCoreTextures][4];
    float tt[6];
    uint32_t pad2[2];
};
static_assert(sizeof(LeanDrawDev) == 208, "LeanDrawDev must be 208 bytes");

constexpr int kMaxMipLevels = 16;
struct TexArrayDev {
    const uint8_t* texels;
    uint32_t width, height, layers;
    uint32_t mips;
    uint32_t level_off[kMaxMipLevels];
};

struct CubeDev {
    const uint2* texels;
    uint32_t size, mips;
    uint32_t level_off[kMaxMipLevels];
    const uint2* bordered;
    uint32_t b_level_off[kMaxMipLevels];
};
enum { kCubeSkybox = 0, kCubePrefiltered = 1, kCubeIrradiance = 2 };

struct DevScene {
    const uint8_t* buf[AWSM_BUF_COUNT];
    TexArrayDev tex[kMaxTexArrays];
    AwsmSampler samplers[kMaxSamplers];
    uint32_t n_tex, n_samplers;
    float skybox_rgba[4];
    float prefiltered_rgb[4];
    float irradiance_rgb[4];
    const uint16_t* lut_rg16f;
    uint32_t lut_w, lut_h;
    CubeDev cube[3];
};

struct TriRec;
constexpr size_t kTriRecBytes = 80;
constexpr uint32_t kMaxDirtyRanges = 12;

enum CounterWord : uint32_t { kCtrBinned = 0, kCtrEntries, kCtrOverflow, kCtrCovered, kCtrBig, kCtrFragments, kCtrFragOverflow, kCtrExtraItems, kCtrWords };

struct FrameDev {
    uint32_t width, height;
    uint32_t y0, y1;
    uint32_t sy0, sy1;
    uint32_t tiles_x, tiles_y;
    uint32_t tile_row0;
    uint32_t band_n, band_r;
    uint32_t out_compact;
    uint32_t n_draws;
    uint32_t total_tris;
    uint32_t total_verts;
    uint32_t rank0, block0;
    uint32_t bin_capacity;
    uint32_t has_opaque;
    uint32_t mipmap;
    uint32_t aniso;
    uint32_t msaa;
    const uint8_t* camera;
    float pix2view[16];
    float view_rot[9];
    float cam_pos[3];
    float ortho_view_dir[3];
    uint32_t cam_ortho;
    const DrawDev* draws;
    DrawShadeDev* draw_shade;
    TexSlotDev* tex_slots;
    DrawMatDev* draw_mat;
    float4* lights_pre;
    uint32_t lights_cap;
    float4* clip;
    float4* nrm;
    float4* tan;
    float4* wpos;
    const uint32_t* block_draw;
    float4* wcache;
    const DrawDev* prev_draws;
    uint32_t prev_n_draws;
    uint32_t cache_on;
    uint32_t cache_serial;
    uint32_t* cache_mark;
    uint32_t n_dirty;
    uint32_t dirty[12][3];
    TriRec* tri_rec;
    uint32_t* tri_info;
    uint4* tri_shade;
    uint32_t attr_data_bytes;
    LeanDrawDev* draw_lean;
    uint32_t* shade_todo;
    uint32_t shade_todo_cap;
    uint32_t* lean_done_flag;
    uint32_t lean_done_serial;
    uint32_t* camera_snap;
    uint32_t camera_snap_words;
    uint32_t* lean_next;
    uint32_t lean_grid;
    uint32_t* tile_count;
    uint32_t* tile_offset;
    uint32_t* tile_cursor;
    uint32_t* scan_tmp;
    uint32_t* tile_order;
    uint32_t* tile_split;
    unsigned long long* raster_scratch;
    uint32_t raster_extra_cap, raster_slot_cap;
    uint32_t* bin_list;
    uint32_t* big_list;
#ifdef AWSM_STAMP
    unsigned long long* stamps;
#endif
    const uint32_t* poison;
    uint32_t* host_bin_status;
    uint32_t frame_serial;
    uint32_t* counters;
    unsigned long long* vis;
    uint16_t* out_rgba16f;
    float* out_rgba32f;
    float4* msaa_color0;
    uint32_t* msaa_edges;
    unsigned long long* msaa_edge_bits;
    uint2* msaa_cells;
    const unsigned long long* hud_vis;
    const DrawDev* hud_draws;
    const uint32_t* hud_tri_info;
    uint32_t hud_pass;
    const unsigned long long* msaa_halo;
    uint32_t halo_bands;
    const uint16_t* opaque_rgba16f;
    uint4* frag_rec;
    float4* frag_color;
    uint32_t* frag_first;
    uint32_t frag_cap;
};

struct PostArgs {
    uint32_t width, height;
    const uint2* src;
    const unsigned long long* vis;
    const uint32_t* frag_first;
    const uint4* frag_rec;
    uint32_t frag_cap;
    const TriRec* tri_rec;
    const float* camera;
    float2* dof_lc;
    float4* dof_blur;
    const uint2* stage_in;
    uint2* stage_out;
    uint2* effects;
    uint32_t* display;
    uint32_t tonemap;
    uint32_t dof;
    const uint32_t* poison;
    uint32_t frame_serial;
};

struct EditorGridDev {
    const uint8_t* camera;
    float p[20];
};

struct SsaoArgs {
    uint32_t width, height;
    const unsigned long long* vis;
    const float* camera;
    float radius, intensity, bias, strength;
    float* ao_raw;
    float* ao_smoothed;
    float* view_z;
    uint2* out16;
    float4* out32;
    const uint32_t* poison;
    uint32_t frame_serial;
};

struct ShadowArgs {
    uint32_t width, height;
    const unsigned long long* vis;
    const float* camera;
    const uint32_t* map;
    uint32_t map_size;
    int32_t pcf_radius;
    float light_view_proj[16];
    float light[4];
    float bias, slope_bias, max_slope, strength, facing_fade;
    float* visibility;
    float* multiplier;
    uint2* out16;
    float4* out32;
    const uint32_t* poison;
    uint32_t frame_serial;
};

struct ShadowViewsArgs {
    ShadowArgs base;
    uint32_t n_views;
    unsigned char* view;
    float view_proj[AWSM_SHADOW_MAX_VIEWS][16];
};

struct TaaArgs {
    uint32_t width, height;
    const uint2* cur;
    const unsigned long long* vis;
    const uint2* history;
    uint2* out;
    float reproject[16];
    float jitter[2];
    float feedback;
    float* layer_xy;
    uint8_t* layer_used;
    const uint32_t* poison;
    uint32_t frame_serial;
};

#ifdef __HIPCC__
__device__ __forceinline__ bool frame_poisoned(const FrameDev& f) {
    return f.poison != nullptr && *(const __attribute__((address_space(4))) uint32_t*)f.poison == f.frame_serial;
}
#endif

}
```

### awsm-renderer_amd/csrc/kernels_geometry.hip

```cpp
#include "frame_params.hpp"
#include "raster_setup.hpp"
#include "launch.hpp"

#ifndef AWSM_GEOM_PRIO
#define AWSM_GEOM_PRIO 3
#endif

namespace awsm {

#ifdef AWSM_STAMP
#define AWSM_STAMP_AT(f, kernel, slot) do { if (threadIdx.x == 0 && (f).stamps && blockIdx.x < 16384u) (f).stamps[((size_t)(kernel) * 16384u + blockIdx.x) * 8u + (slot)] = __builtin_amdgcn_s_memrealtime(); } while (0)
#else
#define AWSM_STAMP_AT(f, kernel, slot) do { } while (0)
#endif

struct GeomMetaDev {
    uint32_t mesh_key_high, mesh_key_low;
    uint32_t morph_len, morph_weights_off, morph_values_off;
    uint32_t skin_sets, skin_matrices_off, skin_index_weights_off;
    uint32_t transform_off, material_meta_off;
};

AWSM_DI bool draw_unchanged(const DevScene* __restrict__ sc, const FrameDev& f, const DrawDev& d, const DrawDev& p, const uint32_t* __restrict__ gmp) {
    if (d.geom_meta_off != p.geom_meta_off || d.vis_data_off != p.vis_data_off || d.tri_count != p.tri_count || d.flags != p.flags || d.first_tri != p.first_tri ||
        d.first_block != p.first_block || d.inst_off != p.inst_off) return false;
    if (f.poison != nullptr && *(const __attribute__((address_space(4))) uint32_t*)f.poison == f.cache_serial) return false;
    if (f.n_dirty == 0u) return true;
    auto hit = [&](uint32_t buf, uint32_t lo, uint32_t hi) {
        for (uint32_t i = 0; i < f.n_dirty; i++) if (f.dirty[i][0] == buf && f.dirty[i][1] < hi && lo < f.dirty[i][2]) return true;
        return false;
    };
    if (hit(AWSM_BUF_GEOM_META, d.geom_meta_off, d.geom_meta_off + 40u)) return false;
    if (hit(AWSM_BUF_VIS_GEOM_DATA, d.vis_data_off, (uint32_t)min((unsigned long long)d.vis_data_off + 168ull * d.tri_count, 0xFFFFFFFFull))) return false;
    if ((d.flags & kDrawInstanced) && hit(AWSM_BUF_INSTANCES, d.inst_off, d.inst_off + 64u)) return false;
    const uint32_t toff = (gmp[8] / 64u) * 64u, mmoff = (gmp[9] / 256u) * 256u;
    if (hit(AWSM_BUF_TRANSFORMS, toff, toff + 64u)) return false;
    if (hit(AWSM_BUF_MATERIAL_META, mmoff, mmoff + 68u)) return false;
    if (gmp[2] != 0u && hit(AWSM_BUF_MORPH_WEIGHTS, gmp[3], gmp[3] + 4u + 4u * gmp[2])) return false;
    if (gmp[5] != 0u && hit(AWSM_BUF_SKIN_MATRICES, gmp[6], 0xFFFFFFFFu)) return false;
    return true;
}

#ifndef AWSM_TRANSFORM_WAVES
#define AWSM_TRANSFORM_WAVES 6
#endif
template <bool FWD>
__global__ __launch_bounds__(256) __attribute__((amdgpu_waves_per_eu(FWD ? 4 : AWSM_TRANSFORM_WAVES))) void k_deform_transform(const DevScene* __restrict__ sc, FrameDev f) {
    __shared__ __attribute__((aligned(16))) uint32_t lds_vtx[FWD ? 4 : 256 * 14];
    if (frame_poisoned(f)) return;
#if AWSM_GEOM_PRIO
    __builtin_amdgcn_s_setprio(AWSM_GEOM_PRIO);
#endif
    const uint32_t tid = threadIdx.x;
    const uint32_t b = blockIdx.x + f.block0;
    {
        const uint32_t n_tiles = f.tiles_x * f.tiles_y, gsz = gridDim.x * 256u, g0 = blockIdx.x * 256u + tid;
        for (uint32_t i = g0; i < n_tiles; i += gsz) f.tile_count[i] = 0u;
        if (g0 < 8u) f.counters[g0] = 0u;
        if (g0 == 12u || g0 == 13u) f.counters[g0] = 0u;
        if (!FWD && f.shade_todo && g0 == 14u) f.shade_todo[0] = 0u;
        if (!FWD && f.lean_next && g0 >= 64u && g0 < 128u) f.lean_next[(g0 - 64u) * 16u] = 0u;
        if (!FWD && g0 < f.camera_snap_words) f.camera_snap[g0] = reinterpret_cast<const uint32_t*>(sc->buf[AWSM_BUF_CAMERA])[g0];
    }
    uint32_t lo = 0, hi = f.n_draws;
    if (!FWD && f.block_draw) lo = f.block_draw[blockIdx.x];
    else while (hi - lo > 1) {
        uint32_t mid = (lo + hi) >> 1;
        if (f.draws[mid].first_block <= b) lo = mid; else hi = mid;
    }
    const DrawDev d = f.draws[lo];
    const uint32_t nverts = 3u * d.tri_count;
    const uint32_t local0 = (b - d.first_block) * 256u;
    const uint32_t count = min(256u, nverts - local0);

    const uint32_t* gmp = reinterpret_cast<const uint32_t*>(sc->buf[AWSM_BUF_GEOM_META] + d.geom_meta_off);
    if (!FWD && f.cache_on && lo < f.prev_n_draws && draw_unchanged(sc, f, d, f.prev_draws[lo], gmp)) {
        if (f.cache_mark && tid == 0u) f.cache_mark[blockIdx.x] = f.frame_serial;
        if (tid < count) {
            const size_t gv = (size_t)3u * d.first_tri + local0 + tid;
            const float4 w = f.wcache[gv];
            const m4 view_proj = load_m4(reinterpret_cast<const float*>(sc->buf[AWSM_BUF_CAMERA] + 128));
            const f4 clip = mul(view_proj, {w.x, w.y, w.z, w.w});
            f.clip[gv] = make_float4(clip.x, clip.y, clip.z, clip.w);
        }
        return;
    }
    GeomMetaDev gm;
    gm.morph_len = gmp[2]; gm.morph_weights_off = gmp[3]; gm.morph_values_off = gmp[4];
    gm.skin_sets = gmp[5]; gm.skin_matrices_off = gmp[6]; gm.skin_index_weights_off = gmp[7];
    gm.transform_off = gmp[8];

    f3 pos, normal; f4 tangent; uint32_t vertex_index;
    if (!FWD) {
        const uint8_t* src = sc->buf[AWSM_BUF_VIS_GEOM_DATA] + (size_t)d.vis_data_off + (size_t)local0 * 56u;
        const uint32_t bytes = count * 56u;
        const uint32_t n16 = bytes >> 4;
        const uint4* src16 = reinterpret_cast<const uint4*>(src);
        uint4* lds16 = reinterpret_cast<uint4*>(lds_vtx);
        for (uint32_t i = tid; i < n16; i += 256u) lds16[i] = src16[i];
        const uint32_t tail0 = n16 << 2;
        if (tid < (bytes >> 2) - tail0) lds_vtx[tail0 + tid] = reinterpret_cast<const uint32_t*>(src)[tail0 + tid];
        __syncthreads();
        if (tid >= count) return;
        const uint32_t* v = lds_vtx + tid * 14u;
        pos = {__uint_as_float(v[0]), __uint_as_float(v[1]), __uint_as_float(v[2])};
        normal = {__uint_as_float(v[6]), __uint_as_float(v[7]), __uint_as_float(v[8])};
        tangent = {__uint_as_float(v[9]), __uint_as_float(v[10]), __uint_as_float(v[11]), __uint_as_float(v[12])};
        vertex_index = v[13];
    } else {
        if (tid >= count) return;
        const uint32_t* mm = reinterpret_cast<const uint32_t*>(sc->buf[AWSM_BUF_MATERIAL_META] + (size_t)(gmp[9] / 256u) * 256u);
        vertex_index = reinterpret_cast<const uint32_t*>(sc->buf[AWSM_BUF_ATTR_INDEX])[mm[9] / 4u + local0 + tid];
        const float* v = reinterpret_cast<const float*>(sc->buf[AWSM_BUF_TRANSPARENCY_GEOM_DATA] + (size_t)d.vis_data_off + (size_t)vertex_index * 40u);
        pos = {v[0], v[1], v[2]};
        normal = {v[3], v[4], v[5]};
        tangent = {v[6], v[7], v[8], v[9]};
    }

    if (gm.morph_len != 0u) {
        const float* mw = reinterpret_cast<const float*>(sc->buf[AWSM_BUF_MORPH_WEIGHTS]);
        const float* mv = reinterpret_cast<const float*>(sc->buf[AWSM_BUF_MORPH_VALUES]);
        const uint32_t wbase = gm.morph_weights_off / 4u + 1u;
        const uint32_t vbase = gm.morph_values_off / 4u + vertex_index * (gm.morph_len * 10u);
        f3 txyz = {tangent.x, tangent.y, tangent.z};
        for (uint32_t i = 0; i < gm.morph_len; i++) {
            const float w = mw[wbase + i];
            const float* dlt = mv + vbase + i * 10u;
            pos = {pos.x + w * dlt[0], pos.y + w * dlt[1], pos.z + w * dlt[2]};
            normal = {normal.x + w * dlt[3], normal.y + w * dlt[4], normal.z + w * dlt[5]};
            txyz = {txyz.x + w * dlt[6], txyz.y + w * dlt[7], txyz.z + w * dlt[8]};
        }
        tangent = {txyz.x, txyz.y, txyz.z, tangent.w};
    }
    if (gm.skin_sets != 0u) {
        const float* iw = reinterpret_cast<const float*>(sc->buf[AWSM_BUF_SKIN_INDEX_WEIGHTS]);
        const float* jm = reinterpret_cast<const float*>(sc->buf[AWSM_BUF_SKIN_MATRICES]);
        const uint32_t base = gm.skin_index_weights_off / 4u + vertex_index * gm.skin_sets * 8u;
        const uint32_t moff = gm.skin_matrices_off / 64u;
        f3 op = {0.0f, 0.0f, 0.0f}, on = op, ot = op;
#pragma unroll
        for (int c = 0; c < 4; c++) {
            float e0 = 0.0f, e1 = 0.0f, e2 = 0.0f;
            for (uint32_t set = 0; set < gm.skin_sets; set++) {
                const float4* p = reinterpret_cast<const float4*>(iw + base + set * 8u);
                const float4 q0 = p[0], q1 = p[1];
                const uint32_t j0 = __float_as_uint(q0.x), j1 = __float_as_uint(q0.z), j2 = __float_as_uint(q1.x), j3 = __float_as_uint(q1.z);
                const float w0 = q0.y, w1 = q0.w, w2 = q1.y, w3 = q1.w;
                const float4 a = reinterpret_cast<const float4*>(jm + (size_t)(j0 + moff) * 16u)[c], bq = reinterpret_cast<const float4*>(jm + (size_t)(j1 + moff) * 16u)[c];
                const float4 cq = reinterpret_cast<const float4*>(jm + (size_t)(j2 + moff) * 16u)[c], dq = reinterpret_cast<const float4*>(jm + (size_t)(j3 + moff) * 16u)[c];
                const float s0 = ((w0 * a.x + w1 * bq.x) + w2 * cq.x) + w3 * dq.x;
                const float s1 = ((w0 * a.y + w1 * bq.y) + w2 * cq.y) + w3 * dq.y;
                const float s2 = ((w0 * a.z + w1 * bq.z) + w2 * cq.z) + w3 * dq.z;
                if (set == 0) { e0 = s0; e1 = s1; e2 = s2; } else { e0 += s0; e1 += s1; e2 += s2; }
            }
            const float px = c == 0 ? pos.x : (c == 1 ? pos.y : (c == 2 ? pos.z : 1.0f));
            if (c == 0) op = {e0 * px, e1 * px, e2 * px}; else op = {op.x + e0 * px, op.y + e1 * px, op.z + e2 * px};
            if (c < 3) {
                const float nx = c == 0 ? normal.x : (c == 1 ? normal.y : normal.z), tx = c == 0 ? tangent.x : (c == 1 ? tangent.y : tangent.z);
                if (c == 0) { on = {e0 * nx, e1 * nx, e2 * nx}; ot = {e0 * tx, e1 * tx, e2 * tx}; }
                else { on = {on.x + e0 * nx, on.y + e1 * nx, on.z + e2 * nx}; ot = {ot.x + e0 * tx, ot.y + e1 * tx, ot.z + e2 * tx}; }
            }
        }
        pos = op; normal = on;
        tangent = {ot.x, ot.y, ot.z, tangent.w};
    }

    m4 model = load_m4(reinterpret_cast<const float*>(sc->buf[AWSM_BUF_TRANSFORMS] + (size_t)(gm.transform_off / 64u) * 64u));
    if (d.flags & kDrawInstanced) {
        const m4 inst = load_m4(reinterpret_cast<const float*>(sc->buf[AWSM_BUF_INSTANCES] + d.inst_off));
        m4 mi;
#pragma unroll
        for (int j = 0; j < 4; j++) mi.c[j] = mul(model, inst.c[j]);
        model = mi;
    }
    const m4 view_proj = load_m4(reinterpret_cast<const float*>(sc->buf[AWSM_BUF_CAMERA] + 128));
    const f4 world_pos = mul(model, {pos.x, pos.y, pos.z, 1.0f});
    const f4 clip = mul(view_proj, world_pos);

    const m3 mm = upper3(model);
    const f3 c0 = mm.c[0], c1 = mm.c[1], c2 = mm.c[2];
    const f3 r0 = {c0.x, c1.x, c2.x}, r1 = {c0.y, c1.y, c2.y}, r2 = {c0.z, c1.z, c2.z};
    const f3 cof0 = cross(r1, r2), cof1 = cross(r2, r0), cof2 = cross(r0, r1);
    const float det_model = dot(r0, cof0);
    f3 wn_un;
    if (fabsf(det_model) > 1e-8f) wn_un = {dot(cof0, normal) / det_model, dot(cof1, normal) / det_model, dot(cof2, normal) / det_model};
    else wn_un = mul(mm, normal);
    const f3 world_normal = normalize(wn_un);

    const f3 tangent_raw = mul(mm, {tangent.x, tangent.y, tangent.z});
    f3 tangent_ortho = tangent_raw - world_normal * dot(tangent_raw, world_normal);
    const float tlen_sq = dot(tangent_ortho, tangent_ortho);
    if (tlen_sq > 1e-8f) {
        tangent_ortho = tangent_ortho * inverse_sqrt(tlen_sq);
    } else {
        const f3 axis = (fabsf(world_normal.z) > 0.999f) ? mk3(0.0f, 1.0f, 0.0f) : mk3(0.0f, 0.0f, 1.0f);
        tangent_ortho = normalize(cross(axis, world_normal));
    }

    const uint32_t lv = local0 + tid;
    const size_t gv = (size_t)3u * d.first_tri + lv;
    f.clip[gv] = make_float4(clip.x, clip.y, clip.z, clip.w);
    if (!FWD && f.wcache) f.wcache[gv] = make_float4(world_pos.x, world_pos.y, world_pos.z, world_pos.w);
    f.nrm[gv] = make_float4(world_normal.x, world_normal.y, world_normal.z, 0.0f);
    f.tan[gv] = make_float4(tangent_ortho.x, tangent_ortho.y, tangent_ortho.z, tangent.w);
    if (FWD) f.wpos[gv] = make_float4(world_pos.x, world_pos.y, world_pos.z, 1.0f);
    if (lv % 3u == 0u) {
        const uint32_t info = lo | ((d.flags & 0x7Fu) << 24)  | ((FWD && (f.draw_shade[lo].flags & 2u)) ? 0x80000000u : 0u);
        f.tri_info[d.first_tri + lv / 3u] = info;
        if (!FWD && f.tri_shade) {
            uint4 ts0 = make_uint4(info, 0u, 0u, 0u), ts1 = make_uint4(0u, 0u, 0u, 0u);
            if (sc->buf[AWSM_BUF_MATERIAL_META] && sc->buf[AWSM_BUF_ATTR_INDEX] && sc->buf[AWSM_BUF_ATTR_DATA]) {
                const uint32_t* mm = reinterpret_cast<const uint32_t*>(sc->buf[AWSM_BUF_MATERIAL_META] + (size_t)(gmp[9] / 256u) * 256u);
                const uint32_t* ai = reinterpret_cast<const uint32_t*>(sc->buf[AWSM_BUF_ATTR_INDEX]) + mm[9] / 4u + lv;
                const uint32_t data_word = mm[10] / 4u, stride_words = mm[11] / 4u, uv0 = mm[12];
                const uint32_t* ad = reinterpret_cast<const uint32_t*>(sc->buf[AWSM_BUF_ATTR_DATA]);
                const uint32_t w0 = data_word + ai[0] * stride_words + uv0, w1 = data_word + ai[1] * stride_words + uv0, w2 = data_word + ai[2] * stride_words + uv0;
                const uint32_t n_words = f.attr_data_bytes >> 2;
                if (w0 < n_words && w0 + 1u < n_words) { ts0.z = ad[w0]; ts0.w = ad[w0 + 1u]; }
                if (w1 < n_words && w1 + 1u < n_words) { ts1.x = ad[w1]; ts1.y = ad[w1 + 1u]; }
                if (w2 < n_words && w2 + 1u < n_words) { ts1.z = ad[w2]; ts1.w = ad[w2 + 1u]; }
            }
            f.tri_shade[2u * (d.first_tri + lv / 3u)] = ts0;
            f.tri_shade[2u * (d.first_tri + lv / 3u) + 1u] = ts1;
        }
    }
}

constexpr uint32_t kBinWindow = 2048;

template <bool FILL>
AWSM_DI void bin_emit(const FrameDev& f, int tx, int l, uint32_t rank) {
    const uint32_t idx = (uint32_t)l * f.tiles_x + (uint32_t)tx;
    if (!FILL) {
        atomicAdd(&f.tile_count[idx], 1u);
    } else {
        const uint32_t slot = atomicAdd(&f.tile_cursor[idx], 1u);
        const uint32_t pos = f.tile_offset[idx] + slot;
        if (pos < f.bin_capacity) f.bin_list[pos] = rank;
    }
}

struct BinTri {
    TriSetup t;
    int tx0, tx1, ty0, ty1, wdt, ntiles;
    bool ok, big, small;
};
template <bool SETUP>
AWSM_DI void bin_tri_load(const FrameDev& f, uint32_t r, BinTri& b) {
    b.ok = false;
    if (r < f.total_tris) {
        if (SETUP) {
            const float4 v0 = f.clip[(size_t)r * 3], v1 = f.clip[(size_t)r * 3 + 1], v2 = f.clip[(size_t)r * 3 + 2];
            bool outside = false;
            if ((f.band_n > 1u || f.y0 > 0u || f.y1 < f.height) && v0.w > 0.0f && v1.w > 0.0f && v2.w > 0.0f) {
                const float hh = 0.5f * (float)f.height;
                const float ya = (1.0f - v0.y / v0.w) * hh, yb = (1.0f - v1.y / v1.w) * hh, yc = (1.0f - v2.y / v2.w) * hh;
                const float lo = fminf(fminf(ya, yb), yc) - 1.0f, hi = fmaxf(fmaxf(ya, yb), yc) + 1.0f;
                if (hi < (float)f.y0 || lo >= (float)f.y1) outside = true;
                else if (f.band_n > 1u && lo >= (float)f.y0 && hi < (float)f.y1) {
                    const int bn = (int)f.band_n, row0 = (int)f.tile_row0;
                    const int a0 = ((int)floorf(lo) >> kTileShift) - row0, a1 = ((int)floorf(hi) >> kTileShift) - row0;
                    const int t0 = (max(a0, 0) + bn - 1) / bn, t1 = a1 >= 0 ? a1 / bn : -1;
                    outside = t0 > t1;
                }
            }
            if (outside) { tri_rec_store_invalid(f.tri_rec + r); b.ok = false; }
            else {
                const bool cull_back = ((f.tri_info[r] >> 24) & AWSM_DRAW_CULL_BACK) != 0;
                b.ok = tri_setup(v0, v1, v2, cull_back, f.width, f.height, f.y0, f.y1, b.t);
                if (!b.ok) { b.t.minx = 0; b.t.maxx = 0; b.t.miny = 0; b.t.maxy = 0; }
                tri_rec_store(f.tri_rec + r, b.t, b.ok);
            }
        } else {
            b.ok = tri_rec_load(f.tri_rec + r, b.t);
        }
    }
    b.tx0 = 0; b.tx1 = -1; b.ty0 = 0; b.ty1 = -1;
    const int bn = (int)f.band_n, row0 = (int)f.tile_row0;
    if (b.ok) {
        b.tx0 = b.t.minx >> kTileShift; b.tx1 = b.t.maxx >> kTileShift;
        const int a0 = (b.t.miny >> kTileShift) - row0, a1 = (b.t.maxy >> kTileShift) - row0;
        b.ty0 = (a0 + bn - 1) / bn; b.ty1 = a1 >= 0 ? a1 / bn : -1;
        b.ok = b.ty0 <= b.ty1;
    }
    b.wdt = b.tx1 - b.tx0 + 1;
    b.ntiles = b.ok ? b.wdt * (b.ty1 - b.ty0 + 1) : 0;
    b.big = b.ntiles > 16;
    b.small = b.ok && !b.big;
}
AWSM_DI bool bin_tile_hit(const FrameDev& f, const TriSetup& t, int ntiles, int tx, int l) {
    const int ty = (int)f.tile_row0 + l * (int)f.band_n;
    return ntiles == 1 || tile_may_overlap(t, tx << kTileShift, ty << kTileShift, (tx + 1) << kTileShift, (ty + 1) << kTileShift);
}

constexpr uint32_t kBinBatches = 1;
static_assert(kBinBatches == 1, "k_bin keeps its triangle in registers across the phases");

template <bool FILL>
AWSM_DI void bin_big_walk(const FrameDev& f, uint32_t block, uint32_t n_blocks) {
    const uint32_t n_big = f.counters[4];
    const int lane = threadIdx.x & 63;
    const uint32_t wave = block * 4u + (threadIdx.x >> 6), n_waves = n_blocks * 4u;
    for (uint32_t i = wave; i < n_big; i += n_waves) {
        const uint32_t r = f.big_list[i];
        BinTri b;
        bin_tri_load<false>(f, r, b);
        for (int k = lane; k < b.ntiles; k += 64) {
            const int l = b.ty0 + k / b.wdt, tx = b.tx0 + k % b.wdt;
            if (bin_tile_hit(f, b.t, b.ntiles, tx, l)) bin_emit<FILL>(f, tx, l, r);
        }
    }
}
constexpr uint32_t kBinBigBlocks = 64;

template <bool FILL>
__global__ __launch_bounds__(256) void k_bin(FrameDev f) {
#if AWSM_GEOM_PRIO
    __builtin_amdgcn_s_setprio(AWSM_GEOM_PRIO);
#endif
    __shared__ int win[4];
    __shared__ uint32_t n_ok, n_big_wg, big_base;
    __shared__ uint32_t lcount[kBinWindow];
    __shared__ uint32_t lbase[FILL ? kBinWindow : 1];

    const uint32_t tid = threadIdx.x;
    if (frame_poisoned(f)) return;
    AWSM_STAMP_AT(f, FILL ? 2 : 0, 0);
    if (FILL && blockIdx.x < kBinBigBlocks) { bin_big_walk<true>(f, blockIdx.x, kBinBigBlocks); AWSM_STAMP_AT(f, 2, 7); return; }
    const uint32_t r0 = f.rank0 + (blockIdx.x - (FILL ? kBinBigBlocks : 0u)) * (256u * kBinBatches) + tid;
    const int lane = tid & 63;
    if (tid == 0) { win[0] = 0x7fffffff; win[1] = 0x7fffffff; win[2] = -1; win[3] = -1; n_ok = 0; n_big_wg = 0; }
    __syncthreads();

    uint32_t my_ok = 0;
    BinTri keep;
    for (uint32_t j = 0; j < kBinBatches; j++) {
        const uint32_t r = r0 + j * 256u;
        BinTri& b = keep;
        bin_tri_load<!FILL>(f, r, b);
        AWSM_STAMP_AT(f, FILL ? 2 : 0, 7);
        my_ok += b.ok ? 1u : 0u;
        {
            int wx0 = b.small ? b.tx0 : 0x7fffffff, wy0 = b.small ? b.ty0 : 0x7fffffff, wx1 = b.small ? b.tx1 : -1, wy1 = b.small ? b.ty1 : -1;
#pragma unroll
            for (int off = 32; off > 0; off >>= 1) {
                wx0 = min(wx0, __shfl_xor(wx0, off)); wy0 = min(wy0, __shfl_xor(wy0, off));
                wx1 = max(wx1, __shfl_xor(wx1, off)); wy1 = max(wy1, __shfl_xor(wy1, off));
            }
            if (lane == 0 && wx1 >= 0) { atomicMin(&win[0], wx0); atomicMin(&win[1], wy0); atomicMax(&win[2], wx1); atomicMax(&win[3], wy1); }
        }
    }
    uint32_t big_slot = 0;
    if (!FILL) {
        const unsigned long long mask = __ballot(keep.big);
        if (mask) {
            uint32_t base = 0;
            if (lane == __ffsll((long long)mask) - 1) base = atomicAdd(&n_big_wg, (uint32_t)__popcll(mask));
            big_slot = (uint32_t)__shfl((int)base, __ffsll((long long)mask) - 1) + (uint32_t)__popcll(mask & ((1ull << lane) - 1ull));
        }
    }
    if (!FILL) {
        for (int off = 32; off > 0; off >>= 1) my_ok += __shfl_down(my_ok, off);
        if (lane == 0 && my_ok) atomicAdd(&n_ok, my_ok);
    }
    AWSM_STAMP_AT(f, FILL ? 2 : 0, 1);
    __syncthreads();
    AWSM_STAMP_AT(f, FILL ? 2 : 0, 2);
    if (!FILL && n_big_wg) {
        if (tid == 0) big_base = atomicAdd(&f.counters[4], n_big_wg);
        __syncthreads();
        if (keep.big) f.big_list[big_base + big_slot] = r0;
    }
    const int wx0 = win[0], wy0 = win[1], ww = win[2] - wx0 + 1, wh = win[3] - wy0 + 1;
    const uint32_t nwin = (ww > 0 && wh > 0) ? (uint32_t)ww * (uint32_t)wh : 0u;
    const bool use_lds = nwin <= kBinWindow;
    if (!FILL && tid == 0 && n_ok) atomicAdd(&f.counters[0], n_ok);
    if (use_lds) for (uint32_t i = tid; i < nwin; i += 256u) lcount[i] = 0u;
    __syncthreads();

    for (uint32_t j = 0; j < kBinBatches; j++) {
        const uint32_t r = r0 + j * 256u;
        BinTri reload;
        if (kBinBatches > 1) bin_tri_load<false>(f, r, reload);
        const BinTri& b = kBinBatches > 1 ? reload : keep;
        if (b.small)
            for (int l = b.ty0; l <= b.ty1; l++)
                for (int tx = b.tx0; tx <= b.tx1; tx++)
                    if (bin_tile_hit(f, b.t, b.ntiles, tx, l)) {
                        if (use_lds) atomicAdd(&lcount[(l - wy0) * ww + (tx - wx0)], 1u);
                        else bin_emit<FILL>(f, tx, l, r);
                    }
    }
    if (!use_lds) return;
    __syncthreads();
    AWSM_STAMP_AT(f, FILL ? 2 : 0, 3);
    for (uint32_t i = tid; i < nwin; i += 256u) {
        const uint32_t c = lcount[i];
        if (c) {
            const uint32_t gidx = (uint32_t)(wy0 + (int)(i / (uint32_t)ww)) * f.tiles_x + (uint32_t)(wx0 + (int)(i % (uint32_t)ww));
            if (!FILL) atomicAdd(&f.tile_count[gidx], c);
            else { lbase[i] = f.tile_offset[gidx] + atomicAdd(&f.tile_cursor[gidx], c); lcount[i] = 0u; }
        }
    }
    AWSM_STAMP_AT(f, FILL ? 2 : 0, 4);
    if (!FILL) return;
    __syncthreads();
    AWSM_STAMP_AT(f, 2, 5);
    for (uint32_t j = 0; j < kBinBatches; j++) {
        const uint32_t r = r0 + j * 256u;
        BinTri reload;
        if (kBinBatches > 1) bin_tri_load<false>(f, r, reload);
        const BinTri& b = kBinBatches > 1 ? reload : keep;
        if (b.small)
            for (int l = b.ty0; l <= b.ty1; l++)
                for (int tx = b.tx0; tx <= b.tx1; tx++)
                    if (bin_tile_hit(f, b.t, b.ntiles, tx, l)) {
                        const uint32_t li = (uint32_t)((l - wy0) * ww + (tx - wx0));
                        const uint32_t pos = lbase[li] + atomicAdd(&lcount[li], 1u);
                        if (pos < f.bin_capacity) f.bin_list[pos] = r;
                    }
    }
    AWSM_STAMP_AT(f, 2, 6);
}

template <bool FILL>
__global__ __launch_bounds__(256) void k_bin_big(FrameDev f) { if (frame_poisoned(f)) return; bin_big_walk<FILL>(f, blockIdx.x, gridDim.x); }

constexpr uint32_t kRasterSlice = 256;
constexpr uint32_t kScanThreads = 256, kScanWords = 40;
AWSM_DI uint32_t ld_sc1(const uint32_t* p) { return __hip_atomic_load(p, __ATOMIC_RELAXED, __HIP_MEMORY_SCOPE_AGENT); }
AWSM_DI void st_sc1(uint32_t* p, uint32_t v) { __hip_atomic_store(p, v, __ATOMIC_RELAXED, __HIP_MEMORY_SCOPE_AGENT); }
__global__ __launch_bounds__(kScanThreads) void k_bin_scan(FrameDev f, uint32_t n_tiles) {
#if AWSM_GEOM_PRIO
    __builtin_amdgcn_s_setprio(AWSM_GEOM_PRIO);
#endif
    __shared__ uint32_t hist[36], part[3][4], base[kScanWords], last_flag;
    const uint32_t tid = threadIdx.x, lane = tid & 63u, wave = tid >> 6, k = blockIdx.x, G = gridDim.x;
    const uint32_t i = k * kScanThreads + tid;
    const bool live = i < n_tiles;
    if (frame_poisoned(f)) return;
    AWSM_STAMP_AT(f, 1, 0);
    if (tid < 36u) hist[tid] = 0u;
    const uint32_t c = live ? f.tile_count[i] : 0u;
    const uint32_t b = 32u - (uint32_t)__clz(c);
    const uint32_t ns = (live && c > kRasterSlice && f.raster_scratch) ? (c + kRasterSlice - 1u) / kRasterSlice : 0u;
    const uint32_t v[3] = {c, ns ? ns - 1u : 0u, ns};
    __syncthreads();
    const uint32_t rank = live ? atomicAdd(&hist[b], 1u) : 0u;
    uint32_t incl[3] = {v[0], v[1], v[2]};
#pragma unroll
    for (int d = 1; d < 64; d <<= 1)
#pragma unroll
        for (int q = 0; q < 3; q++) { const uint32_t o = (uint32_t)__shfl_up((int)incl[q], d); if ((int)lane >= d) incl[q] += o; }
    if (lane == 63u) { part[0][wave] = incl[0]; part[1][wave] = incl[1]; part[2][wave] = incl[2]; }
    __syncthreads();
    uint32_t excl[3], total[3];
#pragma unroll
    for (int q = 0; q < 3; q++) {
        uint32_t before = 0u, all = 0u;
#pragma unroll
        for (uint32_t w = 0; w < 4u; w++) { const uint32_t p = part[q][w]; all += p; if (w < wave) before += p; }
        excl[q] = before + incl[q] - v[q]; total[q] = all;
    }
    uint32_t* agg = f.scan_tmp + (size_t)k * kScanWords;
    uint32_t* bases = f.scan_tmp + (size_t)(G + k) * kScanWords;
    if (tid < 3u) st_sc1(agg + tid, total[tid]);
    else if (tid < 36u) st_sc1(agg + tid, hist[tid - 3u]);
    asm volatile("s_waitcnt vmcnt(0)" ::: "memory");
    __syncthreads();
    if (tid == 0u) last_flag = atomicAdd(&f.counters[12], 1u) == G - 1u ? 1u : 0u;
    __syncthreads();
    AWSM_STAMP_AT(f, 1, 1);
    if (last_flag) {
        __shared__ uint32_t q_total[36];
        for (uint32_t q = wave; q < 36u; q += 4u) {
            uint32_t carry = 0u;
            for (uint32_t k0 = 0; k0 < G; k0 += 64u) {
                const uint32_t kk = k0 + lane;
                const uint32_t a = kk < G ? ld_sc1(f.scan_tmp + (size_t)kk * kScanWords + q) : 0u;
                uint32_t in = a;
#pragma unroll
                for (int d = 1; d < 64; d <<= 1) { const uint32_t o = (uint32_t)__shfl_up((int)in, d); if ((int)lane >= d) in += o; }
                if (kk < G) st_sc1(f.scan_tmp + (size_t)(G + kk) * kScanWords + q, carry + in - a);
                carry += (uint32_t)__shfl((int)in, 63);
            }
            if (lane == 0u) q_total[q] = carry;
        }
        __syncthreads();
        if (tid < 33u) {
            uint32_t heavier = 0u;
            for (uint32_t bb = tid + 1u; bb < 33u; bb++) heavier += q_total[3u + bb];
            st_sc1(f.scan_tmp + (size_t)2u * G * kScanWords + tid, heavier);
        }
        if (tid == 0u) {
            const uint32_t total_entries = q_total[0];
            f.tile_offset[n_tiles] = total_entries;
            f.counters[1] = total_entries;
            if (total_entries > f.bin_capacity) f.counters[2] = 1u;
            f.counters[7] = min(q_total[1], f.raster_extra_cap);
            if (f.host_bin_status) {
                __hip_atomic_store(f.host_bin_status, total_entries, __ATOMIC_RELAXED, __HIP_MEMORY_SCOPE_SYSTEM);
                __hip_atomic_store(f.host_bin_status + 1, (f.frame_serial & 0x7FFFFFFFu) | (total_entries > f.bin_capacity ? 0x80000000u : 0u), __ATOMIC_RELAXED, __HIP_MEMORY_SCOPE_SYSTEM);
            }
        }
        asm volatile("s_waitcnt vmcnt(0)" ::: "memory");
        __syncthreads();
        if (tid == 0u) st_sc1(&f.counters[13], 1u);
    } else {
        if (tid == 0u) {
            uint32_t spins = 0u;
            while (ld_sc1(&f.counters[13]) == 0u && ++spins < (1u << 22)) __builtin_amdgcn_s_sleep(8);
            if (spins >= (1u << 22)) f.counters[2] = 1u;
        }
        __syncthreads();
    }
    AWSM_STAMP_AT(f, 1, 2);
    if (tid < 36u) base[tid] = ld_sc1(bases + tid) + (tid >= 3u ? ld_sc1(f.scan_tmp + (size_t)2u * G * kScanWords + tid - 3u) : 0u);
    __syncthreads();
    if (live) {
        f.tile_offset[i] = base[0] + excl[0];
        f.tile_cursor[i] = 0u;
        f.tile_order[base[3u + b] + rank] = i;
        if (ns) {
            const uint32_t eb = base[1] + excl[1], sb = base[2] + excl[2];
            const bool fits = eb + ns - 1u <= f.raster_extra_cap && sb + ns <= f.raster_slot_cap && ns <= 4095u;
            for (uint32_t s = 1; s < ns; s++) if (eb + s - 1u < f.raster_extra_cap) f.tile_order[n_tiles + eb + s - 1u] = fits ? (i | (s << 20)) : 0xFFFFFFFFu;
            reinterpret_cast<uint2*>(f.tile_split)[i] = make_uint2(fits ? sb : 0xFFFFFFFFu, 0u);
        }
    }
    AWSM_STAMP_AT(f, 1, 4);
}

struct WorkTri {
    double c[3];
    float a[3], b[3];
    float zq[3];
    uint32_t rank;
    uint32_t bbox;
    uint32_t exact;
};
static_assert(sizeof(WorkTri) == 72, "WorkTri");
struct WorkSmall {
    int e[3], a[3], b[3];
    float zq[3];
    uint32_t bias;
    uint32_t pad[2];
    uint32_t rank, bbox, exact;
};
static_assert(sizeof(WorkSmall) == sizeof(WorkTri) && offsetof(WorkSmall, rank) == offsetof(WorkTri, rank) && offsetof(WorkSmall, exact) == offsetof(WorkTri, exact), "WorkSmall");

AWSM_DI void load_work_tri(const WorkTri& g, TriSetup& t) {
#pragma unroll
    for (int i = 0; i < 3; i++) { t.a[i] = g.a[i]; t.b[i] = g.b[i]; t.c[i] = g.c[i]; t.zq[i] = g.zq[i]; }
    t.exact = g.exact != 0u; t.small = g.exact == 2u;
}

template <int S>
AWSM_DI void raster_pixel(unsigned long long* keys, const TriSetup& t, int tpx, int tpy, int px, int py, uint32_t r) {
    if (S == 1) {
        const int sx = (tpx + px) << 8, sy = (tpy + py) << 8;
        const unsigned long long k = tri_sample_key_at(t, sample_coord(sx + 128), sample_coord(sy + 128), r);
        if (k != ~0ull) atomicMin(&keys[py * kTile + px], k);
    } else {
        const float zc = tri_plane_depth(t, tri_edges_d(t, (double)(tpx + px), (double)(tpy + py))) + 0.0f;
        float dz[4];
        msaa_depth_steps(t.a, t.b, t.zq, dz);
#pragma unroll
        for (int s = 0; s < S; s++) {
            const unsigned long long k = tri_msaa_sample_key(t, tpx + px, tpy + py, s, zc, dz, r);
            if (k != ~0ull) atomicMin(&keys[(py * kTile + px) * S + s], k);
        }
    }
}
// ... 206 lines not shown
    const uint32_t tile = item & 0xFFFFFu, slice = item >> 20;
    const uint32_t tid = threadIdx.x;
    const int tpx = (int)(tile % f.tiles_x) << kTileShift;
    const int tpy = (int)(f.tile_row0 + (tile / f.tiles_x) * f.band_n) << kTileShift;

#pragma unroll
    for (int i = 0; i < 4 * S; i++) keys[tid + i * 256] = ~0ull;
    const uint32_t off = f.tile_offset[tile];
    const uint32_t count_all = f.tile_count[tile];
    const uint32_t slot0 = (count_all > kRasterSlice && f.raster_scratch) ? f.tile_split[2u * tile] : 0xFFFFFFFFu;
    const bool split = slot0 != 0xFFFFFFFFu;
    const uint32_t n_slices = split ? (count_all + kRasterSlice - 1u) / kRasterSlice : 1u;
    const uint32_t count_fit = min(count_all, f.bin_capacity - min(f.bin_capacity, off));
    const uint32_t first = split ? min(slice * kRasterSlice, count_fit) : 0u;
    const uint32_t count = split ? min((slice + 1u) * kRasterSlice, count_fit) : count_fit;
    const int lane = tid & 63, wave = tid >> 6;

    for (uint32_t base = first; base < count; base += kBatch) {
        if (tid == 0) { n_mid = 0; n_big = 0; next_mid = 16u; next_big = 4u; }
        __syncthreads();
        const uint32_t idx = base + tid;
        if (base == first) AWSM_STAMP_AT(f, 3, 1);
        if (idx < count && tid < kBatch) {
            const uint32_t r = f.bin_list[off + idx];
            TriSetup t;
            if (tri_rec_load(f.tri_rec + r, t)) {
                const int x0 = max(t.minx, tpx), x1 = min(t.maxx, tpx + kTile - 1);
                const int y0 = max(t.miny, tpy), y1 = min(t.maxy, tpy + kTile - 1);
                if (x0 <= x1 && y0 <= y1) {
                    const int area = (x1 - x0 + 1) * (y1 - y0 + 1);
                    if (area <= 4) {
                        for (int py = y0; py <= y1; py++)
                            for (int px = x0; px <= x1; px++) raster_pixel<S>(keys, t, tpx, tpy, px - tpx, py - tpy, r);
                    } else {
                        const uint32_t slot = (area <= 256) ? atomicAdd(&n_mid, 1u) : (kBatch - 1u) - atomicAdd(&n_big, 1u);
                        const uint32_t bbox = (uint32_t)(x0 - tpx) | ((uint32_t)(x1 - tpx) << 8) | ((uint32_t)(y0 - tpy) << 16) | ((uint32_t)(y1 - tpy) << 24);
                        if (area <= 256 && t.small) {
                            WorkSmall& g = reinterpret_cast<WorkSmall&>(work[slot]);
                            const double half = S == 1 ? 0.5 : 0.0;
                            const double X = (double)x0 + half, Y = (double)y0 + half;
                            uint32_t bw = 0u;
#pragma unroll
                            for (int i = 0; i < 3; i++) {
                                const int bias = (t.a[i] > 0.0f || (t.a[i] == 0.0f && t.b[i] > 0.0f)) ? 0 : 1;
                                g.e[i] = (int)fma((double)t.a[i], X, fma((double)t.b[i], Y, t.c[i])) - bias;
                                g.a[i] = (int)t.a[i]; g.b[i] = (int)t.b[i]; g.zq[i] = t.zq[i];
                                bw |= (uint32_t)bias << i;
                            }
                            g.bias = bw; g.rank = r; g.bbox = bbox; g.exact = 2u;
                        } else {
                            WorkTri& g = work[slot];
#pragma unroll
                            for (int i = 0; i < 3; i++) { g.a[i] = t.a[i]; g.b[i] = t.b[i]; g.c[i] = t.c[i]; g.zq[i] = t.zq[i]; }
                            g.rank = r; g.exact = (t.small && !(area <= 256)) ? 2u : (t.exact ? 1u : 0u);
                            g.bbox = bbox;
                        }
                    }
                }
            }
        }
        __syncthreads();
        if (base == first) AWSM_STAMP_AT(f, 3, 2);
        const uint32_t nm = n_mid, nb = n_big;
        {
            const uint32_t group = tid >> 4;
            const int lx = (int)(tid & 3u), ly = (int)((tid >> 2) & 3u);
            for (uint32_t j = group; j < nm; ) {
                const WorkTri& g = work[j];
                if (g.exact == 2u) { if (S == 1) raster_walk_small(keys, reinterpret_cast<const WorkSmall&>(g), lx, ly); else raster_walk_small4(keys, reinterpret_cast<const WorkSmall&>(g), lx, ly); }
                else {
                TriSetup t;
                load_work_tri(g, t);
                const uint32_t bb = g.bbox, r = g.rank;
                const int x0 = (int)(bb & 255u), x1 = (int)((bb >> 8) & 255u), y0 = (int)((bb >> 16) & 255u), y1 = (int)(bb >> 24);
                raster_walk<S, 4>(keys, t, tpx, tpy, x0, x1, y0, y1, lx, ly, r);
                }
                uint32_t nx = 0u;
                if ((tid & 15u) == 0u) nx = atomicAdd(&next_mid, 1u);
                j = (uint32_t)__shfl((int)nx, 0, 16);
            }
        }
        for (uint32_t j = wave; j < nb; ) {
            const WorkTri& g = work[(kBatch - 1u) - j];
            TriSetup t;
            load_work_tri(g, t);
            const uint32_t bb = g.bbox, r = g.rank;
            const int x0 = (int)(bb & 255u), x1 = (int)((bb >> 8) & 255u), y0 = (int)((bb >> 16) & 255u), y1 = (int)(bb >> 24);
            const int lx = lane & 7, ly = lane >> 3;
            raster_walk<S, 8>(keys, t, tpx, tpy, x0, x1, y0, y1, lx, ly, r);
            uint32_t nx = 0u;
            if (lane == 0) nx = atomicAdd(&next_big, 1u);
            j = (uint32_t)__shfl((int)nx, 0, 64);
        }
        __syncthreads();
    }
    __syncthreads();
    AWSM_STAMP_AT(f, 3, 3);
    if (split) {
        __shared__ uint32_t arrived;
        unsigned long long* mine = f.raster_scratch + (size_t)(slot0 + slice) * (kTile * kTile * S);
#pragma unroll
        for (int i = 0; i < 4 * S; i++) __hip_atomic_store(mine + tid + i * 256, keys[tid + i * 256], __ATOMIC_RELAXED, __HIP_MEMORY_SCOPE_AGENT);
        asm volatile("s_waitcnt vmcnt(0)" ::: "memory");
        __syncthreads();
        if (tid == 0) arrived = __hip_atomic_fetch_add(&f.tile_split[2u * tile + 1u], 1u, __ATOMIC_RELAXED, __HIP_MEMORY_SCOPE_AGENT);
        __syncthreads();
        if (arrived != n_slices - 1u) return;
        for (uint32_t k = 0; k < n_slices; k++) {
            if (k == slice) continue;
            const unsigned long long* other = f.raster_scratch + (size_t)(slot0 + k) * (kTile * kTile * S);
            unsigned long long v[4 * S];
#pragma unroll
            for (int i = 0; i < 4 * S; i++) v[i] = __hip_atomic_load(other + tid + i * 256, __ATOMIC_RELAXED, __HIP_MEMORY_SCOPE_AGENT);
#pragma unroll
            for (int i = 0; i < 4 * S; i++) if (v[i] < keys[tid + i * 256]) keys[tid + i * 256] = v[i];
        }
        __syncthreads();
    }
#pragma unroll
    for (int i = 0; i < 4 * S; i++) {
        const int e = (int)tid + i * 256;
        const int p = e / S, s = e % S;
        const int px = tpx + (p & (kTile - 1)), py = tpy + (p >> kTileShift);
        if (px < (int)f.width && py >= (int)f.y0 && py < (int)f.y1) __builtin_nontemporal_store(keys[e], &f.vis[((size_t)py * f.width + px) * S + s]);
    }
    AWSM_STAMP_AT(f, 3, 4);
}
template <int S> __global__ void k_raster_tile(FrameDev f);
template <> __global__ __launch_bounds__(256) __attribute__((amdgpu_waves_per_eu(AWSM_RASTER_WAVES1))) void k_raster_tile<1>(FrameDev f) {
    __shared__ unsigned long long keys[kTile * kTile];
    raster_tile_body<1>(f, keys);
}
#ifndef AWSM_RASTER_VGPRS4
#define AWSM_RASTER_VGPRS4 0
#endif
#if AWSM_RASTER_VGPRS4
template <> __global__ __launch_bounds__(256) __attribute__((amdgpu_num_vgpr(AWSM_RASTER_VGPRS4))) void k_raster_tile<4>(FrameDev f) {
#else
template <> __global__ __launch_bounds__(256) __attribute__((amdgpu_waves_per_eu(AWSM_RASTER_WAVES4))) void k_raster_tile<4>(FrameDev f) {
#endif
    extern __shared__ unsigned long long keys_dynamic[];
    raster_tile_body<4>(f, keys_dynamic);
}

__global__ __launch_bounds__(256) void k_hud_merge(const unsigned long long* __restrict__ world, const unsigned long long* __restrict__ hud, unsigned long long* __restrict__ out,
                                                   size_t first, size_t n) {
    const size_t i = first + (size_t)blockIdx.x * 256u + threadIdx.x;
    if (i >= first + n) return;
    const unsigned long long w = world[i], h = hud[i];
    const unsigned long long depth = w == ~0ull ? 0x3F800000ull : (w >> 32);
    out[i] = h == ~0ull ? w : ((depth << 32) | (h & 0xFFFFFFFFull));
}

__global__ __launch_bounds__(256) void k_upload_words(uint32_t* __restrict__ dst, const uint32_t* __restrict__ src_pinned, uint32_t n_words) {
    for (uint32_t i = blockIdx.x * 256u + threadIdx.x; i < n_words; i += gridDim.x * 256u) dst[i] = __builtin_nontemporal_load(src_pinned + i);
}

__global__ __launch_bounds__(64) void k_handoff_signal(uint32_t* flag, uint32_t serial, unsigned long long* stamp) {
    if (threadIdx.x != 0) return;
    if (stamp) *stamp = wall_clock64();
    if (flag) st_sc1(flag, serial);
}
__global__ __launch_bounds__(64) void k_handoff_wait(const uint32_t* flag, uint32_t serial, unsigned long long budget_ticks, uint32_t* timeouts_host, uint32_t timeouts_known,
                                                     uint32_t* poison, uint32_t poison_serial) {
    if (threadIdx.x != 0) return;
    if (__hip_atomic_load(timeouts_host, __ATOMIC_RELAXED, __HIP_MEMORY_SCOPE_SYSTEM) != timeouts_known) budget_ticks = min(budget_ticks, 2000ull);
    const unsigned long long t0 = wall_clock64();
    while ((int32_t)(ld_sc1(flag) - serial) < 0) {
        if (wall_clock64() - t0 >= budget_ticks) {
            if (poison) st_sc1(poison, poison_serial);
            __hip_atomic_fetch_add(timeouts_host, 1u, __ATOMIC_RELAXED, __HIP_MEMORY_SCOPE_SYSTEM);
            break;
        }
        __builtin_amdgcn_s_sleep(8);
    }
}

}

extern "C" void awsm_launch_upload_words(void* dst, const void* src_pinned, uint32_t n_words, hipStream_t s) {
    const uint32_t nb = (n_words + 255u) / 256u;
    if (nb) hipLaunchKernelGGL(awsm::k_upload_words, dim3(nb < 64u ? nb : 64u), dim3(256), 0, s, (uint32_t*)dst, (const uint32_t*)src_pinned, n_words);
}

extern "C" void awsm_launch_handoff_signal(uint32_t* flag, uint32_t serial, unsigned long long* stamp, hipStream_t s) {
    hipLaunchKernelGGL(awsm::k_handoff_signal, dim3(1), dim3(64), 0, s, flag, serial, stamp);
}
extern "C" void awsm_launch_handoff_wait(const uint32_t* flag, uint32_t serial, unsigned long long budget_ticks, uint32_t* timeouts_host, uint32_t timeouts_known,
                                         uint32_t* poison, uint32_t poison_serial, hipStream_t s) {
    hipLaunchKernelGGL(awsm::k_handoff_wait, dim3(1), dim3(64), 0, s, flag, serial, budget_ticks, timeouts_host, timeouts_known, poison, poison_serial);
}
extern "C" void awsm_launch_hud_merge(const unsigned long long* world, const unsigned long long* hud, unsigned long long* out, size_t first, size_t n, hipStream_t s) {
    if (n) hipLaunchKernelGGL(awsm::k_hud_merge, dim3((unsigned)((n + 255u) / 256u)), dim3(256), 0, s, world, hud, out, first, n);
}
extern "C" void awsm_launch_transform(const awsm::DevScene* sc, const awsm::FrameDev* f, uint32_t n_blocks, hipStream_t s) {
    if (n_blocks) hipLaunchKernelGGL(awsm::k_deform_transform<false>, dim3(n_blocks), dim3(256), 0, s, sc, *f);
}
extern "C" void awsm_launch_transform_forward(const awsm::DevScene* sc, const awsm::FrameDev* f, uint32_t n_blocks, hipStream_t s) {
    if (n_blocks) hipLaunchKernelGGL(awsm::k_deform_transform<true>, dim3(n_blocks), dim3(256), 0, s, sc, *f);
}
extern "C" void awsm_launch_bin_count(const awsm::FrameDev* f, hipStream_t s) {
    const uint32_t per = 256u * awsm::kBinBatches, nb = (f->total_tris - f->rank0 + per - 1u) / per;
    if (nb) hipLaunchKernelGGL(awsm::k_bin<false>, dim3(nb), dim3(256), 0, s, *f);
}
extern "C" void awsm_launch_bin_big(const awsm::FrameDev* f, int fill, hipStream_t s) {
    if (f->total_tris <= f->rank0) return;
    if (fill) return;
    hipLaunchKernelGGL(awsm::k_bin_big<false>, dim3(512), dim3(256), 0, s, *f);
}
__global__ void k_debug_pad(unsigned long long ticks) {
    const unsigned long long t0 = wall_clock64();
    while (wall_clock64() - t0 < ticks) __builtin_amdgcn_s_sleep(32);
}
extern "C" void awsm_launch_bin_scan(const awsm::FrameDev* f, hipStream_t s) {
#ifdef AWSM_DEBUG_SWITCHES
    static const long pad_us = getenv("AWSM_DEBUG_CHAIN_PAD_US") ? atol(getenv("AWSM_DEBUG_CHAIN_PAD_US")) : 0;
    if (pad_us > 0) hipLaunchKernelGGL(k_debug_pad, dim3(1), dim3(64), 0, s, (unsigned long long)pad_us * 100ull);
#endif
    const uint32_t n_tiles = f->tiles_x * f->tiles_y;
    if (n_tiles) hipLaunchKernelGGL(awsm::k_bin_scan, dim3((n_tiles + awsm::kScanThreads - 1u) / awsm::kScanThreads), dim3(awsm::kScanThreads), 0, s, *f, n_tiles);
}
extern "C" void awsm_launch_bin_fill(const awsm::FrameDev* f, hipStream_t s) {
    const uint32_t per = 256u * awsm::kBinBatches, nb = (f->total_tris - f->rank0 + per - 1u) / per;
    if (nb) hipLaunchKernelGGL(awsm::k_bin<true>, dim3(nb + awsm::kBinBigBlocks), dim3(256), 0, s, *f);
}
extern "C" void awsm_launch_raster(const awsm::FrameDev* f, hipStream_t s) {
    const uint32_t n_tiles = f->tiles_x * f->tiles_y;
    if (!n_tiles) return;
    const uint32_t nb = n_tiles + (f->raster_scratch ? f->raster_extra_cap : 0u);
    if (f->msaa == 4u) hipLaunchKernelGGL(awsm::k_raster_tile<4>, dim3(nb), dim3(256), awsm::kTile * awsm::kTile * 4 * sizeof(unsigned long long), s, *f);
    else hipLaunchKernelGGL(awsm::k_raster_tile<1>, dim3(nb), dim3(256), 0, s, *f);
}
```

Baseline: 3431 frames/s.

## Derive clip positions from world cache in binning and record bin masks for fill

Adds a per-draw decide kernel so unchanged draws skip the transform entirely. Their clip positions are no longer written; the binning kernel instead recomputes clip coordinates from the cached world positions. The count pass also packs each small triangle's tile window and coverage mask into an 8-byte record, which the fill pass reads instead of redoing setup and tile tests. A lazy clip materialize kernel fills the clip buffer before readback, at the cost of extra buffer space, an extra launch, and matrix math inside binning.

```diff
diff --git a/awsm-renderer_amd/csrc/awsm_hip.cpp b/awsm-renderer_amd/csrc/awsm_hip.cpp
--- a/awsm-renderer_amd/csrc/awsm_hip.cpp
+++ b/awsm-renderer_amd/csrc/awsm_hip.cpp
@@ -10,6 +10,7 @@
 #include <vector>
 
 #include "ctx.hpp"
+#include "bin_record.hpp"
 #include "launch.hpp"
 
 using namespace awsm;
@@ -371,6 +372,22 @@
     return AWSM_OK;
 }
 
+int materialize_clip(AwsmHipCtx* c) {
+    FrameBufs& b = FB(c);
+    if (!b.clip_in_bin_last) return AWSM_OK;
+    const uint32_t n = 3u * c->lists[kPassWorld].total_tris;
+    if (n && b.wcache.ptr && b.clip.ptr && b.camera.ptr) {
+        FrameDev f;
+        memset(&f, 0, sizeof f);
+        f.wcache = (float4*)b.wcache.ptr; f.clip = (float4*)b.clip.ptr; f.camera = (const uint8_t*)b.camera.ptr;
+        f.total_verts = n; f.clip_from_world = kClipReadBack;
+        awsm_launch_transform(c->scene_dev, &f, 0, c->stream);
+        HIPCHK(c, hipGetLastError());
+    }
+    b.clip_in_bin_last = false;
+    return AWSM_OK;
+}
+
 int enqueue_geometry(AwsmHipCtx* c, bool replay = false) {
     HostTrace ht(c->frame_serial);
     const PassList& world = c->lists[kPassWorld];
@@ -405,7 +422,10 @@
 #else
     const int knockout = 0;
 #endif
-    if (has_geometry && !(knockout & 1)) awsm_launch_transform(c->scene_dev, &f, world.n_blocks, c->stream);
+    f.clip_from_world = (c->clip_in_bin && f.wcache && FB(c).camera.ptr && c->bufs[AWSM_BUF_CAMERA].ptr && c->bufs[AWSM_BUF_CAMERA].size >= 192) ? 1u : 0u;
+    f.draw_hit_at = (f.clip_from_world && f.cache_on && f.block_draw && (size_t)FB(c).draw_hit_at + f.n_draws <= FB(c).block_map.size / 4) ? FB(c).draw_hit_at : 0u;
+    f.bin_rec_at = (c->clip_in_bin && bin_rec_fits(f.tiles_x, f.tiles_y) && ((size_t)FB(c).bin_rec_at + f.total_tris) * 8 <= FB(c).tri_rec.size) ? FB(c).bin_rec_at : 0u;
+    if (has_geometry && !(knockout & 1)) { awsm_launch_transform(c->scene_dev, &f, world.n_blocks, c->stream); FB(c).clip_in_bin_last = f.clip_from_world != 0u; }
     if ((rc = record(c, EV_TRANSFORM))) return rc;
     ht.mark("geometry: transform launch");
     if (n_tiles && !(knockout & 2)) enqueue_binning(f, world.total_tris != 0, c->stream);
@@ -695,7 +715,8 @@
         if ((rc = dev_reserve(c, b.draws_prev, nd * sizeof(DrawDev)))) return rc;
         if ((rc = dev_reserve(c, b.wcache, nv * 16))) return rc;
         const size_t blocks_bound = nv / 256 + nd + 1;
-        if ((rc = dev_reserve(c, b.block_map, blocks_bound * 4))) return rc;
+        b.draw_hit_at = (c->clip_in_bin && blocks_bound + nd < (1ull << 30)) ? (uint32_t)blocks_bound : 0u;
+        if ((rc = dev_reserve(c, b.block_map, (blocks_bound + (b.draw_hit_at ? nd : 0)) * 4))) return rc;
         b.block_map_valid = false;
         if (b.cache_mark.size < blocks_bound * 4) { if ((rc = dev_realloc(c, b.cache_mark, (blocks_bound + blocks_bound / 2) * 4, true))) return rc; }
     }
@@ -711,7 +732,8 @@
     if (!forward && !shadow && (rc = dev_reserve(c, b.tri_shade, nt * 32))) return rc;
     if (!forward && !shadow && (rc = dev_reserve(c, b.draw_lean, nd * sizeof(LeanDrawDev)))) return rc;
     if ((rc = dev_reserve(c, b.big_list, nt * 4))) return rc;
-    if ((rc = dev_reserve(c, b.tri_rec, nt * kTriRecBytes))) return rc;
+    b.bin_rec_at = (world_pass && c->clip_in_bin && nt * (kTriRecBytes / 8) <= 0xFFFFFFFFull) ? (uint32_t)(nt * (kTriRecBytes / 8)) : 0u;
+    if ((rc = dev_reserve(c, b.tri_rec, nt * kTriRecBytes + (b.bin_rec_at ? nt * 8 : 0)))) return rc;
     const uint32_t tiles_x = (dm.w + kTile - 1) / kTile, tiles_y_full = (dm.h + kTile - 1) / kTile;
     const size_t n_tiles_full = (size_t)tiles_x * tiles_y_full;
     if ((rc = dev_reserve(c, b.tile_count, n_tiles_full * 4))) return rc;
@@ -761,7 +783,7 @@
         if (!keep_prev || !b.block_map.ptr) return AWSM_OK;
         std::vector<uint32_t> map;
         for (size_t i = 0; i < draws_host.size(); i++) map.insert(map.end(), (3ull * draws_host[i].tri_count + 255) / 256, (uint32_t)i);
-        if (map.size() * 4 > b.block_map.size || map.size() * 4 > (1u << 20)) return AWSM_OK;
+        if (map.size() * 4 > b.block_map.size || map.size() * 4 > (1u << 20) || (b.draw_hit_at && map.size() > b.draw_hit_at)) return AWSM_OK;
         const int rc = upload_small(c, b.block_map.ptr, map.data(), map.size() * 4);
         if (!rc) b.block_map_valid = true;
         return rc;
@@ -836,6 +858,7 @@
     if (hipMalloc((void**)&c->scene_dev, sizeof(DevScene)) != hipSuccess) return bail(AWSM_ERR_OUT_OF_MEMORY);
     c->overlap = (cfg->flags & AWSM_CFG_OVERLAP_FRAMES) != 0;
     { const char* e = getenv("AWSM_GEOMETRY_CACHE"); c->geometry_cache = !(e && e[0] == '0'); }
+    { const char* e = getenv("AWSM_CLIP_IN_BIN"); c->clip_in_bin = !(e && e[0] == '0'); }
     {
         const char* e = getenv("AWSM_LEAN_WGS_PER_CU");
         const int per_cu = e ? atoi(e) : (c->overlap ? kLeanWgsPerCu : 0);
@@ -1547,8 +1570,9 @@
     c->shadow_px[c->slot] = shadow_on ? (size_t)c->width * c->height : 0;
     c->last_opaque = *p;
     if (!p->has_opaque && c->camera_written_since_snapshot && c->bufs[AWSM_BUF_CAMERA].ptr) {
-        int rcs = sync_all(c);
+        int rcs = materialize_clip(c);
         if (rcs) return rcs;
+        if ((rcs = sync_all(c))) return rcs;
         compose_pixel_to_view(c, FB(c));
         HIPCHK(c, hipMemcpy(FB(c).camera.ptr, c->bufs[AWSM_BUF_CAMERA].ptr, std::min<size_t>(512, c->bufs[AWSM_BUF_CAMERA].size), hipMemcpyDeviceToDevice));
         c->camera_written_since_snapshot = false;
@@ -2235,6 +2259,7 @@
 int awsm_hip_read_transformed(AwsmHipCtx* c, float* clip_out, float* nt_out, uint32_t max_vertices) {
     if (!c) return AWSM_ERR_INVALID_ARGUMENT;
     if (!c->geometry_done) return fail(c, AWSM_ERR_NOT_READY, "read_transformed before geometry_pass");
+    if (clip_out) { HIPCHK(c, hipSetDevice(c->device)); const int rc = materialize_clip(c); if (rc) return rc; }
     return read_pass_vertices(c, FB(c), std::min(max_vertices, 3u * c->lists[kPassWorld].total_tris), clip_out, nt_out, nullptr);
 }
 
diff --git a/awsm-renderer_amd/csrc/bin_record.hpp b/awsm-renderer_amd/csrc/bin_record.hpp
--- /dev/null
+++ b/awsm-renderer_amd/csrc/bin_record.hpp
@@ -0,0 +1,51 @@
+#pragma once
+#include <stdint.h>
+
+#if defined(__HIPCC__)
+#define AWSM_BINREC_FN __host__ __device__ inline
+#else
+#define AWSM_BINREC_FN inline
+#endif
+
+namespace awsm {
+
+constexpr uint32_t kBinRecTiles = 16;
+constexpr uint32_t kBinRecExtentBits = 4;
+constexpr uint32_t kBinRecTileBits = 10;
+constexpr uint32_t kBinRecMaxTileCols = 1u << kBinRecTileBits, kBinRecMaxTileRows = 1u << kBinRecTileBits;
+static_assert(kBinRecTiles <= 16, "the mask is 16 bits");
+static_assert((1u << kBinRecExtentBits) >= kBinRecTiles, "a window of kBinRecTiles tiles in one row or column must fit the extent fields");
+static_assert(2 + 2 * kBinRecExtentBits + 2 * kBinRecTileBits <= 32, "word 0");
+static_assert(((1u << 15) >> 5) <= kBinRecMaxTileCols && ((1u << 15) >> 5) <= kBinRecMaxTileRows, "tile coordinates of the largest frame");
+static_assert((3840 + 31) / 32 <= kBinRecMaxTileCols && (2160 + 31) / 32 <= kBinRecMaxTileRows, "the 4K frame");
+
+struct BinRecWords { uint32_t w0, w1; };
+struct BinRec {
+    bool ok, big;
+    uint32_t tx0, ty0;
+    uint32_t wm1, hm1;
+    uint32_t mask;
+};
+
+AWSM_BINREC_FN bool bin_rec_fits(uint32_t tiles_x, uint32_t tiles_y) { return tiles_x <= kBinRecMaxTileCols && tiles_y <= kBinRecMaxTileRows; }
+
+AWSM_BINREC_FN BinRecWords bin_rec_pack(const BinRec& r) {
+    BinRecWords w;
+    w.w0 = (r.ok ? 1u : 0u) | (r.big ? 2u : 0u) | ((r.wm1 & ((1u << kBinRecExtentBits) - 1u)) << 2) | ((r.hm1 & ((1u << kBinRecExtentBits) - 1u)) << (2 + kBinRecExtentBits)) |
+           ((r.tx0 & ((1u << kBinRecTileBits) - 1u)) << (2 + 2 * kBinRecExtentBits)) | ((r.ty0 & ((1u << kBinRecTileBits) - 1u)) << (2 + 2 * kBinRecExtentBits + kBinRecTileBits));
+    w.w1 = r.mask & 0xFFFFu;
+    return w;
+}
+
+AWSM_BINREC_FN BinRec bin_rec_unpack(BinRecWords w) {
+    BinRec r;
+    r.ok = (w.w0 & 1u) != 0u; r.big = (w.w0 & 2u) != 0u;
+    r.wm1 = (w.w0 >> 2) & ((1u << kBinRecExtentBits) - 1u);
+    r.hm1 = (w.w0 >> (2 + kBinRecExtentBits)) & ((1u << kBinRecExtentBits) - 1u);
+    r.tx0 = (w.w0 >> (2 + 2 * kBinRecExtentBits)) & ((1u << kBinRecTileBits) - 1u);
+    r.ty0 = (w.w0 >> (2 + 2 * kBinRecExtentBits + kBinRecTileBits)) & ((1u << kBinRecTileBits) - 1u);
+    r.mask = w.w1 & 0xFFFFu;
+    return r;
+}
+
+}
diff --git a/awsm-renderer_amd/csrc/ctx.hpp b/awsm-renderer_amd/csrc/ctx.hpp
--- a/awsm-renderer_amd/csrc/ctx.hpp
+++ b/awsm-renderer_amd/csrc/ctx.hpp
@@ -66,6 +66,8 @@
     uint32_t cache_serial = 0;
     PassKind kind = kPassWorld;
     uint8_t slot = 0;
+    uint32_t draw_hit_at = 0, bin_rec_at = 0;
+    bool clip_in_bin_last = false;
 };
 
 }
@@ -226,6 +228,8 @@
         PassList lists[AWSM_SHADOW_MAX_VIEWS];
     } shadow_views[kSlots];
     DevBuf shadow_view_ctr[kSlots], shadow_view_layers[kSlots];
+
+    bool clip_in_bin = true;
 };
 
 #define HIPCHK(c, call)                                                                            \
diff --git a/awsm-renderer_amd/csrc/frame_params.hpp b/awsm-renderer_amd/csrc/frame_params.hpp
--- a/awsm-renderer_amd/csrc/frame_params.hpp
+++ b/awsm-renderer_amd/csrc/frame_params.hpp
@@ -108,6 +108,8 @@
 constexpr uint32_t kMaxDirtyRanges = 12;
 
 enum CounterWord : uint32_t { kCtrBinned = 0, kCtrEntries, kCtrOverflow, kCtrCovered, kCtrBig, kCtrFragments, kCtrFragOverflow, kCtrExtraItems, kCtrWords };
+
+constexpr uint32_t kClipReadBack = 2u;
 
 struct FrameDev {
     uint32_t width, height;
@@ -148,13 +150,16 @@
     uint32_t prev_n_draws;
     uint32_t cache_on;
     uint32_t cache_serial;
+    uint32_t clip_from_world;
     uint32_t* cache_mark;
     uint32_t n_dirty;
     uint32_t dirty[12][3];
+    uint32_t draw_hit_at;
     TriRec* tri_rec;
     uint32_t* tri_info;
     uint4* tri_shade;
     uint32_t attr_data_bytes;
+    uint32_t bin_rec_at;
     LeanDrawDev* draw_lean;
     uint32_t* shade_todo;
     uint32_t shade_todo_cap;
diff --git a/awsm-renderer_amd/csrc/kernels_geometry.hip b/awsm-renderer_amd/csrc/kernels_geometry.hip
--- a/awsm-renderer_amd/csrc/kernels_geometry.hip
+++ b/awsm-renderer_amd/csrc/kernels_geometry.hip
@@ -1,5 +1,6 @@
 #include "frame_params.hpp"
 #include "raster_setup.hpp"
+#include "bin_record.hpp"
 #include "launch.hpp"
 
 #ifndef AWSM_GEOM_PRIO
@@ -41,6 +42,28 @@
     return true;
 }
 
+AWSM_DI f4 clip_from_world_pos(const m4& view_proj, float wx, float wy, float wz, float ww) { return mul(view_proj, {wx, wy, wz, ww}); }
+AWSM_DI m4 load_view_proj(const uint8_t* camera) {
+    const __attribute__((address_space(4))) float* p = (const __attribute__((address_space(4))) float*)(camera + 128);
+    m4 m;
+#pragma unroll
+    for (int i = 0; i < 4; i++) m.c[i] = {p[4 * i], p[4 * i + 1], p[4 * i + 2], p[4 * i + 3]};
+    return m;
+}
+
+__global__ __launch_bounds__(256) void k_draw_decide(const DevScene* __restrict__ sc, FrameDev f) {
+    if (frame_poisoned(f)) return;
+    uint32_t* const hit = const_cast<uint32_t*>(f.block_draw) + f.draw_hit_at;
+    const uint32_t i = blockIdx.x * 256u + threadIdx.x;
+    if (i >= f.n_draws) return;
+    bool same = false;
+    if (f.cache_on && i < f.prev_n_draws) {
+        const DrawDev d = f.draws[i];
+        same = draw_unchanged(sc, f, d, f.prev_draws[i], reinterpret_cast<const uint32_t*>(sc->buf[AWSM_BUF_GEOM_META] + d.geom_meta_off));
+    }
+    hit[i] = same ? 1u : 0u;
+}
+
 #ifndef AWSM_TRANSFORM_WAVES
 #define AWSM_TRANSFORM_WAVES 6
 #endif
@@ -68,19 +91,24 @@
         uint32_t mid = (lo + hi) >> 1;
         if (f.draws[mid].first_block <= b) lo = mid; else hi = mid;
     }
+    const bool decided = !FWD && f.draw_hit_at != 0u && f.block_draw != nullptr;
+    if (decided && f.block_draw[f.draw_hit_at + lo] != 0u) {
+        if (f.cache_mark && tid == 0u) f.cache_mark[blockIdx.x] = f.frame_serial;
+        return;
+    }
     const DrawDev d = f.draws[lo];
     const uint32_t nverts = 3u * d.tri_count;
     const uint32_t local0 = (b - d.first_block) * 256u;
     const uint32_t count = min(256u, nverts - local0);
 
     const uint32_t* gmp = reinterpret_cast<const uint32_t*>(sc->buf[AWSM_BUF_GEOM_META] + d.geom_meta_off);
-    if (!FWD && f.cache_on && lo < f.prev_n_draws && draw_unchanged(sc, f, d, f.prev_draws[lo], gmp)) {
+    if (!FWD && !decided && f.cache_on && lo < f.prev_n_draws && draw_unchanged(sc, f, d, f.prev_draws[lo], gmp)) {
         if (f.cache_mark && tid == 0u) f.cache_mark[blockIdx.x] = f.frame_serial;
-        if (tid < count) {
+        if (!f.clip_from_world && tid < count) {
             const size_t gv = (size_t)3u * d.first_tri + local0 + tid;
             const float4 w = f.wcache[gv];
             const m4 view_proj = load_m4(reinterpret_cast<const float*>(sc->buf[AWSM_BUF_CAMERA] + 128));
-            const f4 clip = mul(view_proj, {w.x, w.y, w.z, w.w});
+            const f4 clip = clip_from_world_pos(view_proj, w.x, w.y, w.z, w.w);
             f.clip[gv] = make_float4(clip.x, clip.y, clip.z, clip.w);
         }
         return;
@@ -175,7 +203,7 @@
     }
     const m4 view_proj = load_m4(reinterpret_cast<const float*>(sc->buf[AWSM_BUF_CAMERA] + 128));
     const f4 world_pos = mul(model, {pos.x, pos.y, pos.z, 1.0f});
-    const f4 clip = mul(view_proj, world_pos);
+    const f4 clip = clip_from_world_pos(view_proj, world_pos.x, world_pos.y, world_pos.z, world_pos.w);
 
     const m3 mm = upper3(model);
     const f3 c0 = mm.c[0], c1 = mm.c[1], c2 = mm.c[2];
@@ -199,7 +227,7 @@
 
     const uint32_t lv = local0 + tid;
     const size_t gv = (size_t)3u * d.first_tri + lv;
-    f.clip[gv] = make_float4(clip.x, clip.y, clip.z, clip.w);
+    if (FWD || !f.clip_from_world) f.clip[gv] = make_float4(clip.x, clip.y, clip.z, clip.w);
     if (!FWD && f.wcache) f.wcache[gv] = make_float4(world_pos.x, world_pos.y, world_pos.z, world_pos.w);
     f.nrm[gv] = make_float4(world_normal.x, world_normal.y, world_normal.z, 0.0f);
     f.tan[gv] = make_float4(tangent_ortho.x, tangent_ortho.y, tangent_ortho.z, tangent.w);
@@ -250,7 +278,13 @@
     b.ok = false;
     if (r < f.total_tris) {
         if (SETUP) {
-            const float4 v0 = f.clip[(size_t)r * 3], v1 = f.clip[(size_t)r * 3 + 1], v2 = f.clip[(size_t)r * 3 + 2];
+            float4 v0, v1, v2;
+            if (f.clip_from_world) {
+                const float4 w0 = f.wcache[(size_t)r * 3], w1 = f.wcache[(size_t)r * 3 + 1], w2 = f.wcache[(size_t)r * 3 + 2];
+                const m4 view_proj = load_view_proj(f.camera);
+                const f4 c0 = clip_from_world_pos(view_proj, w0.x, w0.y, w0.z, w0.w), c1 = clip_from_world_pos(view_proj, w1.x, w1.y, w1.z, w1.w), c2 = clip_from_world_pos(view_proj, w2.x, w2.y, w2.z, w2.w);
+                v0 = make_float4(c0.x, c0.y, c0.z, c0.w); v1 = make_float4(c1.x, c1.y, c1.z, c1.w); v2 = make_float4(c2.x, c2.y, c2.z, c2.w);
+            } else { v0 = f.clip[(size_t)r * 3]; v1 = f.clip[(size_t)r * 3 + 1]; v2 = f.clip[(size_t)r * 3 + 2]; }
             bool outside = false;
             if ((f.band_n > 1u || f.y0 > 0u || f.y1 < f.height) && v0.w > 0.0f && v1.w > 0.0f && v2.w > 0.0f) {
                 const float hh = 0.5f * (float)f.height;
@@ -285,7 +319,7 @@
     }
     b.wdt = b.tx1 - b.tx0 + 1;
     b.ntiles = b.ok ? b.wdt * (b.ty1 - b.ty0 + 1) : 0;
-    b.big = b.ntiles > 16;
+    b.big = b.ntiles > (int)kBinRecTiles;
     b.small = b.ok && !b.big;
 }
 AWSM_DI bool bin_tile_hit(const FrameDev& f, const TriSetup& t, int ntiles, int tx, int l) {
@@ -313,8 +347,18 @@
 }
 constexpr uint32_t kBinBigBlocks = 64;
 
-template <bool FILL>
+AWSM_DI uint32_t bin_rec_read(const uint2* bin_rec, const FrameDev& f, uint32_t r, BinTri& b) {
+    BinRec q = bin_rec_unpack({0u, 0u});
+    if (r < f.total_tris) { const uint2 w = bin_rec[r]; q = bin_rec_unpack({w.x, w.y}); }
+    b.ok = q.ok; b.big = q.ok && q.big; b.small = q.ok && !q.big;
+    b.tx0 = (int)q.tx0; b.tx1 = (int)(q.tx0 + q.wm1); b.ty0 = (int)q.ty0; b.ty1 = (int)(q.ty0 + q.hm1);
+    b.wdt = (int)q.wm1 + 1; b.ntiles = 0;
+    return q.mask;
+}
+
+template <bool FILL, bool REC>
 __global__ __launch_bounds__(256) void k_bin(FrameDev f) {
+    uint2* const bin_rec = reinterpret_cast<uint2*>(f.tri_rec) + f.bin_rec_at;
 #if AWSM_GEOM_PRIO
     __builtin_amdgcn_s_setprio(AWSM_GEOM_PRIO);
 #endif
@@ -334,10 +378,12 @@
 
     uint32_t my_ok = 0;
     BinTri keep;
+    uint32_t rec_mask = 0u;
     for (uint32_t j = 0; j < kBinBatches; j++) {
         const uint32_t r = r0 + j * 256u;
         BinTri& b = keep;
-        bin_tri_load<!FILL>(f, r, b);
+        if (FILL && REC) rec_mask = bin_rec_read(bin_rec, f, r, b);
+        else bin_tri_load<!FILL>(f, r, b);
         AWSM_STAMP_AT(f, FILL ? 2 : 0, 7);
         my_ok += b.ok ? 1u : 0u;
         {
@@ -383,13 +429,23 @@
         BinTri reload;
         if (kBinBatches > 1) bin_tri_load<false>(f, r, reload);
         const BinTri& b = kBinBatches > 1 ? reload : keep;
-        if (b.small)
+        if (b.small) {
+            uint32_t bit = 1u;
             for (int l = b.ty0; l <= b.ty1; l++)
-                for (int tx = b.tx0; tx <= b.tx1; tx++)
-                    if (bin_tile_hit(f, b.t, b.ntiles, tx, l)) {
+                for (int tx = b.tx0; tx <= b.tx1; tx++, bit <<= 1)
+                    if ((FILL && REC) ? (rec_mask & bit) != 0u : bin_tile_hit(f, b.t, b.ntiles, tx, l)) {
+                        if (!FILL && REC) rec_mask |= bit;
                         if (use_lds) atomicAdd(&lcount[(l - wy0) * ww + (tx - wx0)], 1u);
                         else bin_emit<FILL>(f, tx, l, r);
                     }
+        }
+        if (!FILL && REC && r < f.total_tris) {
+            BinRec q;
+            q.ok = b.ok; q.big = b.big; q.tx0 = (uint32_t)b.tx0; q.ty0 = (uint32_t)b.ty0; q.wm1 = (uint32_t)(b.tx1 - b.tx0); q.hm1 = (uint32_t)(b.ty1 - b.ty0); q.mask = rec_mask;
+            if (!b.small) { q.tx0 = 0u; q.ty0 = 0u; q.wm1 = 0u; q.hm1 = 0u; }
+            const BinRecWords w = bin_rec_pack(q);
+            bin_rec[r] = make_uint2(w.w0, w.w1);
+        }
     }
     if (!use_lds) return;
     __syncthreads();
@@ -411,14 +467,16 @@
         BinTri reload;
         if (kBinBatches > 1) bin_tri_load<false>(f, r, reload);
         const BinTri& b = kBinBatches > 1 ? reload : keep;
-        if (b.small)
+        if (b.small) {
+            uint32_t bit = 1u;
             for (int l = b.ty0; l <= b.ty1; l++)
-                for (int tx = b.tx0; tx <= b.tx1; tx++)
-                    if (bin_tile_hit(f, b.t, b.ntiles, tx, l)) {
+                for (int tx = b.tx0; tx <= b.tx1; tx++, bit <<= 1)
+                    if ((FILL && REC) ? (rec_mask & bit) != 0u : bin_tile_hit(f, b.t, b.ntiles, tx, l)) {
                         const uint32_t li = (uint32_t)((l - wy0) * ww + (tx - wx0));
                         const uint32_t pos = lbase[li] + atomicAdd(&lcount[li], 1u);
                         if (pos < f.bin_capacity) f.bin_list[pos] = r;
                     }
+        }
     }
     AWSM_STAMP_AT(f, 2, 6);
 }
@@ -931,6 +989,14 @@
     out[i] = h == ~0ull ? w : ((depth << 32) | (h & 0xFFFFFFFFull));
 }
 
+__global__ __launch_bounds__(256) void k_clip_from_world(FrameDev f, uint32_t n_verts) {
+    const uint32_t i = blockIdx.x * 256u + threadIdx.x;
+    if (i >= n_verts) return;
+    const float4 w = f.wcache[i];
+    const f4 clip = clip_from_world_pos(load_view_proj(f.camera), w.x, w.y, w.z, w.w);
+    f.clip[i] = make_float4(clip.x, clip.y, clip.z, clip.w);
+}
+
 __global__ __launch_bounds__(256) void k_upload_words(uint32_t* __restrict__ dst, const uint32_t* __restrict__ src_pinned, uint32_t n_words) {
     for (uint32_t i = blockIdx.x * 256u + threadIdx.x; i < n_words; i += gridDim.x * 256u) dst[i] = __builtin_nontemporal_load(src_pinned + i);
 }
@@ -973,14 +1039,22 @@
     if (n) hipLaunchKernelGGL(awsm::k_hud_merge, dim3((unsigned)((n + 255u) / 256u)), dim3(256), 0, s, world, hud, out, first, n);
 }
 extern "C" void awsm_launch_transform(const awsm::DevScene* sc, const awsm::FrameDev* f, uint32_t n_blocks, hipStream_t s) {
-    if (n_blocks) hipLaunchKernelGGL(awsm::k_deform_transform<false>, dim3(n_blocks), dim3(256), 0, s, sc, *f);
+    if (f->clip_from_world == awsm::kClipReadBack) {
+        if (f->total_verts) hipLaunchKernelGGL(awsm::k_clip_from_world, dim3((f->total_verts + 255u) / 256u), dim3(256), 0, s, *f, f->total_verts);
+        return;
+    }
+    if (!n_blocks) return;
+    if (f->draw_hit_at && f->block_draw && f->n_draws) hipLaunchKernelGGL(awsm::k_draw_decide, dim3((f->n_draws + 255u) / 256u), dim3(256), 0, s, sc, *f);
+    hipLaunchKernelGGL(awsm::k_deform_transform<false>, dim3(n_blocks), dim3(256), 0, s, sc, *f);
 }
 extern "C" void awsm_launch_transform_forward(const awsm::DevScene* sc, const awsm::FrameDev* f, uint32_t n_blocks, hipStream_t s) {
     if (n_blocks) hipLaunchKernelGGL(awsm::k_deform_transform<true>, dim3(n_blocks), dim3(256), 0, s, sc, *f);
 }
 extern "C" void awsm_launch_bin_count(const awsm::FrameDev* f, hipStream_t s) {
     const uint32_t per = 256u * awsm::kBinBatches, nb = (f->total_tris - f->rank0 + per - 1u) / per;
-    if (nb) hipLaunchKernelGGL(awsm::k_bin<false>, dim3(nb), dim3(256), 0, s, *f);
+    if (!nb) return;
+    if (f->bin_rec_at) hipLaunchKernelGGL((awsm::k_bin<false, true>), dim3(nb), dim3(256), 0, s, *f);
+    else hipLaunchKernelGGL((awsm::k_bin<false, false>), dim3(nb), dim3(256), 0, s, *f);
 }
 extern "C" void awsm_launch_bin_big(const awsm::FrameDev* f, int fill, hipStream_t s) {
     if (f->total_tris <= f->rank0) return;
@@ -1001,7 +1075,9 @@
 }
 extern "C" void awsm_launch_bin_fill(const awsm::FrameDev* f, hipStream_t s) {
     const uint32_t per = 256u * awsm::kBinBatches, nb = (f->total_tris - f->rank0 + per - 1u) / per;
-    if (nb) hipLaunchKernelGGL(awsm::k_bin<true>, dim3(nb + awsm::kBinBigBlocks), dim3(256), 0, s, *f);
+    if (!nb) return;
+    if (f->bin_rec_at) hipLaunchKernelGGL((awsm::k_bin<true, true>), dim3(nb + awsm::kBinBigBlocks), dim3(256), 0, s, *f);
+    else hipLaunchKernelGGL((awsm::k_bin<true, false>), dim3(nb + awsm::kBinBigBlocks), dim3(256), 0, s, *f);
 }
 extern "C" void awsm_launch_raster(const awsm::FrameDev* f, hipStream_t s) {
     const uint32_t n_tiles = f->tiles_x * f->tiles_y;
```

Measured after the change: 3511 frames/s (median of 6 runs). 2.3% higher.
